# tjtiger86/dl-swin-gan

Measured on AMD Instinct MI355X. Metric: cine slices/sec (fwd+bwd) at 10-iter unroll, 1/2/4/8 GPU; PSNR vs ref, higher is better.
Workload: dtype fp32

## Files before the change

### dl-swin-gan_amd/csrc/conv3d.hip

```cpp
#include "dlcs_common.h"

#include <cstdlib>
#include <map>
#include <mutex>
#include <tuple>
#include <type_traits>

namespace {

enum ScratchSlot { kScrColsum, kScrH3r, kScrSplit2, kScrH3Tail, kScrWgH3, kScrTwp, kScrV6Tail, kScrBiasPart,
                   kScrSlots };
std::mutex g_scr_mu;
std::map<std::tuple<int, int, hipStream_t>, std::pair<void*, size_t>> g_scr;

void* scratch(int slot, hipStream_t st, size_t bytes) {
    int dev = 0;
    if (hipGetDevice(&dev) != hipSuccess) return nullptr;
    std::lock_guard<std::mutex> lk(g_scr_mu);
    auto& e = g_scr[{slot, dev, st}];
    if (e.second < bytes) {
        if (e.first) {
            if (hipStreamSynchronize(st) != hipSuccess) return nullptr;
            (void)hipFree(e.first);
        }
        e.first = nullptr;
        e.second = 0;
        if (hipMalloc(&e.first, bytes) != hipSuccess) return nullptr;
        e.second = bytes;
    }
    return e.first;
}

constexpr int kHaloT = 6, kHaloY = 10, kHaloX = 10;
constexpr int kHalo = kHaloT * kHaloY * kHaloX;
constexpr int CK = 32;

template <typename T> struct ConvPad;
template <> struct ConvPad<bf16> { static constexpr int v = 8; };
template <> struct ConvPad<float> { static constexpr int v = 4; };

DLCS_DEV long brow(int b, int t, int y, int x, int nT, int nY, int nX) {
    const long patch = (((long)b * nT + (t >> 2)) * nY + (y >> 2)) * nX + (x >> 2);
    return patch * 64 + ((t & 3) << 4) + ((y & 3) << 2) + (x & 3);
}

struct ConvArgs {
    const void* in; const void* w; const float* bias; void* out;
    const void* mask; const void* res;
    int B, D, H, W, Cin, cin_ld, cin_pad, Cout, cout_pad, cout_ld;
    int mask_ld, res_ld, relu_in, out_f32, res_f32, accumulate, relu_out;
    float res_scale;
};

template <typename T>
DLCS_DEV Frag8<T> relu8(Frag8<T> f) {
#pragma unroll
    for (int i = 0; i < 8; ++i) f.v[i] = (to_f(f.v[i]) > 0.0f) ? f.v[i] : from_f<T>(0.0f);
    return f;
}

template <typename T, int NT>
__global__ void __launch_bounds__(256) conv3d_k3_kernel(ConvArgs a) {
    constexpr int LD = CK + ConvPad<T>::v;
    constexpr int COP = NT * 32;
    extern __shared__ __attribute__((aligned(16))) char smem_raw[];
    T* Hs = reinterpret_cast<T*>(smem_raw);
    T* Ws = Hs + kHalo * LD;

    const int nT = a.D >> 2, nY = a.H >> 2, nX = a.W >> 2;
    const int nYt = (nY + 1) >> 1, nXt = (nX + 1) >> 1;
    int bid = blockIdx.x;
    const int txx = bid % nXt; bid /= nXt;
    const int tyy = bid % nYt; bid /= nYt;
    const int pt = bid % nT;
    const int b = bid / nT;
    const int t0 = pt * 4, y0 = tyy * 8, x0 = txx * 8;
    const T* in = reinterpret_cast<const T*>(a.in);
    const T* wt = reinterpret_cast<const T*>(a.w);
    const int lane = threadIdx.x & 63, wave = threadIdx.x >> 6, hh = lane >> 5;
    const int ncc = a.cin_pad / CK;
    const int nsteps = ncc * 27;

    auto stage_halo = [&](int cc) {
        for (int i = threadIdx.x; i < kHalo * (CK / 8); i += 256) {
            const int hv = i >> 2, c8 = (i & 3) * 8;
            const int ht = hv / (kHaloY * kHaloX), hy = (hv / kHaloX) % kHaloY, hx = hv % kHaloX;
            const int t = t0 - 1 + ht, y = y0 - 1 + hy, x = x0 - 1 + hx;
            const int c = cc * CK + c8;
            Frag8<T> f = zero8<T>();
            if (t >= 0 && t < a.D && y >= 0 && y < a.H && x >= 0 && x < a.W && c < a.Cin) {
                f = load8<T>(in + brow(b, t, y, x, nT, nY, nX) * a.cin_ld + c);
                if (a.relu_in) f = relu8<T>(f);
            }
// ... 1677 lines not shown
                         dlcs_stream_t stream) {
    DLCS_CHECK_ARG(in && gout && dw_packed && B > 0);
    if (D % 4 || H % 4 || W % 4 || cin_pad % 32 || cout_pad % 32 || cout_pad > 160 || cin_ld % 8 || g_ld % 8)
        return DLCS_ERR_UNSUPPORTED_SIZE;
    WgradArgs a{};
    a.in = in; a.g = gout; a.dw = dw_packed;
    a.B = (int)B; a.D = (int)D; a.H = (int)H; a.W = (int)W; a.Cin = (int)cin; a.cin_ld = (int)cin_ld;
    a.cin_pad = (int)cin_pad; a.Cout = (int)cout; a.g_ld = (int)g_ld; a.cout_pad = (int)cout_pad;
    a.relu_in = relu_in; a.vox_per_block = vox_per_block > 0 ? ((vox_per_block + 31) / 32) * 32 : 16384;
    hipStream_t st = (hipStream_t)stream;
    a.dbias = dbias;
    bool done = false;
    const int rc = dtype == DLCS_F32 ? wgrad_launch<float>(a, st, &done) : wgrad_launch<bf16>(a, st, &done);
    if (rc || !dbias || done) return rc;
    const long rows = B * D * H * W;
    return dlcs_colsum(dtype, gout, rows, cout, g_ld, dbias, stream);
}

int dlcs_conv3d_pack_weights(int dtype, const float* w, void* packed, int64_t cout, int64_t cin,
                             int64_t rows_pad, int64_t cols_pad, int mode, dlcs_stream_t stream) {
    DLCS_CHECK_ARG(w && packed && cout > 0 && cin > 0 && mode >= 0 && mode <= 3);
    const long n = 27L * rows_pad * cols_pad;
    hipStream_t st = (hipStream_t)stream;
    if (mode >= 2) {
#ifdef DLCS_DIAG_BUILD
        if (cout != 160 || cin != 160) return DLCS_ERR_UNSUPPORTED_SIZE;
        bf16* wa = (bf16*)packed;
        hipLaunchKernelGGL(pack_weights_x6_kernel, dim3(grid_for(27L * 160 * 160)), dim3(256), 0, st, w, wa,
                           wa + 27L * 160 * 320, mode - 2);
        return dlcs_launch_status();
#else
        return DLCS_ERR_UNSUPPORTED_SIZE;
#endif
    }
    if (dtype == DLCS_F32)
        hipLaunchKernelGGL(pack_weights_kernel<float>, dim3(grid_for(n)), dim3(256), 0, st, w, (float*)packed, (int)cout, (int)cin, (int)rows_pad, (int)cols_pad, mode);
    else
        hipLaunchKernelGGL(pack_weights_kernel<bf16>, dim3(grid_for(n)), dim3(256), 0, st, w, (bf16*)packed, (int)cout, (int)cin, (int)rows_pad, (int)cols_pad, mode);
    return dlcs_launch_status();
}

#ifdef DLCS_DIAG_BUILD
int dlcs_split3_bf16(const float* x, int64_t rows, int64_t ld, void* xa, void* xb, dlcs_stream_t stream) {
    DLCS_CHECK_ARG(x && xa && xb && rows > 0 && ld >= 160);
    if (ld % 4 || ((uintptr_t)x & 15) || ((uintptr_t)xa & 15) || ((uintptr_t)xb & 15)) return DLCS_ERR_UNSUPPORTED_SIZE;
    hipLaunchKernelGGL(split3_kernel, dim3(grid_for(rows * 20)), dim3(256), 0, (hipStream_t)stream, x, (long)rows,
                       (int)ld, (bf16*)xa, (bf16*)xb);
    return dlcs_launch_status();
}

int dlcs_conv3d_k3_x6(const void* xa, const void* xb, const void* wpacked, const float* bias, float* out,
                      int64_t cout_ld, int64_t B, int64_t D, int64_t H, int64_t W, const float* mask, int64_t mask_ld,
                      const float* residual, int64_t res_ld, float res_scale, int accumulate, int relu_out,
                      dlcs_stream_t stream) {
    DLCS_CHECK_ARG(xa && xb && wpacked && out && B > 0);
    auto al16 = [](const void* p) { return ((uintptr_t)p & 15) == 0; };
    if (D % 4 || H % 4 || W % 4 || cout_ld % 4 || !al16(xa) || !al16(xb) || !al16(wpacked) || !al16(out) ||
        (mask && (mask_ld % 4 || !al16(mask))) || (residual && (res_ld % 4 || !al16(residual))) || (bias && !al16(bias)) ||
        B * D * H * W * 320 >= (1L << 31))
        return DLCS_ERR_UNSUPPORTED_SIZE;
    ConvX6Args v{};
    v.xa = (const bf16*)xa; v.xb = (const bf16*)xb; v.w = (const bf16*)wpacked; v.bias = bias; v.out = out;
    v.mask = mask; v.res = residual; v.B = (int)B; v.D = (int)D; v.H = (int)H; v.W = (int)W;
    v.cout_ld = (int)cout_ld; v.mask_ld = (int)mask_ld; v.res_ld = (int)res_ld; v.accumulate = accumulate;
    v.relu_out = relu_out; v.res_scale = res_scale;
    return conv_x6_launch(v, (hipStream_t)stream);
}

int dlcs_conv3d_k3_wgrad_x6(const void* xa, const void* xb, const void* ga, const void* gb, float* dw_packed,
                            int64_t B, int64_t D, int64_t H, int64_t W, dlcs_stream_t stream) {
    DLCS_CHECK_ARG(xa && xb && ga && gb && dw_packed && B > 0);
    auto al16 = [](const void* p) { return ((uintptr_t)p & 15) == 0; };
    if (D % 4 || H % 4 || W % 4 || !al16(xa) || !al16(xb) || !al16(ga) || !al16(gb) ||
        B * D * H * W * 320 >= (1L << 40))
        return DLCS_ERR_UNSUPPORTED_SIZE;
    WgradX6Args v{};
    v.xa = (const bf16*)xa; v.xb = (const bf16*)xb; v.ga = (const bf16*)ga; v.gb = (const bf16*)gb;
    v.dw = dw_packed; v.B = (int)B; v.D = (int)D; v.H = (int)H; v.W = (int)W;
    return wgrad_x6_launch(v, (hipStream_t)stream);
}
#endif

size_t dlcs_split2_f16_bytes(int64_t rows) { return (size_t)rows * 640 + 256 + 640; }

int dlcs_split2_f16(const float* x, int64_t rows, int64_t ld, void* planes, int have_max, float* colsum,
                    dlcs_stream_t stream) {
    DLCS_CHECK_ARG(x && planes && rows > 0 && ld >= 160);
    if (ld % 4 || ((uintptr_t)x & 15) || ((uintptr_t)planes & 15)) return DLCS_ERR_UNSUPPORTED_SIZE;
    hipStream_t st = (hipStream_t)stream;
    unsigned* mx = (unsigned*)((char*)planes + (size_t)rows * 640);
    if (!have_max) {
        if (hipMemsetAsync(mx, 0, 4, st) != hipSuccess) return dlcs_launch_status();
        hipLaunchKernelGGL(absmax_kernel, dim3(std::min(h3_grid(rows * 10), 2048u)), dim3(256), 0, st, x, (long)rows,
                           (int)ld, mx);
    }
    const unsigned g = (unsigned)std::min<long>(kSplit2Blocks, std::max<long>(5, (rows * 20 + 255) / 256 / 5 * 5));
    if (colsum) {
        float* cpart = split2_colsum_workspace(st);
        if (!cpart) return (int)hipErrorOutOfMemory;
        hipLaunchKernelGGL(split2_f16_kernel<true>, dim3(g), dim3(256), 0, st, x, (long)rows, (int)ld,
                           (const unsigned*)mx, (f16*)planes, cpart);
        hipLaunchKernelGGL(colsum_parts_kernel, dim3(160), dim3(256), 0, st, (const float*)cpart, (int)g, colsum);
    } else {
        hipLaunchKernelGGL(split2_f16_kernel<false>, dim3(g), dim3(256), 0, st, x, (long)rows, (int)ld,
                           (const unsigned*)mx, (f16*)planes, nullptr);
    }
    return dlcs_launch_status();
}

size_t dlcs_conv3d_pack_weights_f16x3_bytes(void) { return (size_t)5 * 27 * 160 * 64 * 2 + 256; }

int dlcs_conv3d_pack_weights_f16x3(const float* w, int mode, void* packed, dlcs_stream_t stream) {
    DLCS_CHECK_ARG(w && packed && (mode == 0 || mode == 1));
    if (((uintptr_t)w & 15) || ((uintptr_t)packed & 15)) return DLCS_ERR_UNSUPPORTED_SIZE;
    hipStream_t st = (hipStream_t)stream;
    unsigned* mx = (unsigned*)((char*)packed + (size_t)5 * 27 * 160 * 64 * 2);
    if (hipMemsetAsync(mx, 0, 4, st) != hipSuccess) return dlcs_launch_status();
    hipLaunchKernelGGL(absmax_kernel, dim3(h3_grid(4320L * 10)), dim3(256), 0, st, w, 4320L, 160, mx);
    hipLaunchKernelGGL(pack_weights_f16x3_kernel, dim3(h3_grid(27L * 160 * 160)), dim3(256), 0, st, w,
                       (const unsigned*)mx, (f16*)packed, mode);
    return dlcs_launch_status();
}

static float* colsum_part_workspace(hipStream_t st, long nwg) {
    return static_cast<float*>(scratch(kScrColsum, st, (size_t)nwg * 160 * sizeof(float)));
}

int dlcs_conv3d_k3_f16x3(const void* xplanes, const void* wpacked, const float* bias, float* out, int64_t cout_ld,
                         int64_t B, int64_t D, int64_t H, int64_t W, const float* mask, int64_t mask_ld,
                         const float* residual, int64_t res_ld, float res_scale, int accumulate, int relu_out,
                         unsigned* out_max, void* out_planes, float* colsum, const void* mask_planes,
                         dlcs_stream_t stream) {
    DLCS_CHECK_ARG(xplanes && wpacked && B > 0 && (out || (out_planes && !accumulate)) && !(mask && mask_planes));
    if (!out) cout_ld = 160;
    auto al16 = [](const void* p) { return ((uintptr_t)p & 15) == 0; };
    const long rows = (long)B * D * H * W;
    if (D % 4 || H % 4 || W % 4 || cout_ld % 4 || !al16(xplanes) || !al16(wpacked) || !al16(out) ||
        (mask && (mask_ld % 4 || !al16(mask))) || (residual && (res_ld % 4 || !al16(residual))) || (bias && !al16(bias)) ||
        rows * 320 >= (1L << 31))
        return DLCS_ERR_UNSUPPORTED_SIZE;
    ConvH3Args v{};
    v.xp = (const f16*)xplanes; v.wp = (const f16*)wpacked;
    v.xmax = (const unsigned*)((const char*)xplanes + rows * 640);
    v.wmax = (const unsigned*)((const char*)wpacked + (size_t)5 * 27 * 160 * 64 * 2);
    v.bias = bias; v.out = out; v.mask = mask; v.res = residual;
    v.B = (int)B; v.D = (int)D; v.H = (int)H; v.W = (int)W;
    v.cout_ld = (int)cout_ld; v.mask_ld = (int)mask_ld; v.res_ld = (int)res_ld; v.accumulate = accumulate;
    v.relu_out = relu_out; v.res_scale = res_scale; v.omax = out_max;
    if (mask_planes && !al16(mask_planes)) return DLCS_ERR_UNSUPPORTED_SIZE;
    v.mplanes = mask_planes;
    if (out_planes) {
        if (cout_ld != 160 || !al16(out_planes)) return DLCS_ERR_UNSUPPORTED_SIZE;
        v.oplanes = (f16*)out_planes;
        v.opmax = (const unsigned*)((const char*)out_planes + rows * 640);
    }
#ifdef DLCS_DIAG_BUILD
    v.stamp = conv_stamps_on() ? 1 : 0;
    static const int h3_exp = [] { const char* e = dlcs_knob("DLCS_H3_EXP"); return e ? atoi(e) : 0; }();
    v.exp = h3_exp;
#endif
    hipStream_t st = (hipStream_t)stream;
    const long ntile = (long)B * (D / 4) * ((H / 4 + 1) / 2) * ((W / 4 + 1) / 2);
    if (colsum) {
        v.cpart = colsum_part_workspace(st, ntile);
        if (!v.cpart) return (int)hipErrorOutOfMemory;
    }
    const int rc = conv_f16x3_launch(v, st);
    if (rc || !colsum) return rc;
    hipLaunchKernelGGL(colsum_parts_kernel, dim3(160), dim3(256), 0, st, (const float*)v.cpart, (int)ntile, colsum);
    return dlcs_launch_status();
}

int dlcs_conv3d_k3_wgrad_f16x3(const void* xplanes, const void* gplanes, float* dw_packed, int64_t B, int64_t D,
                               int64_t H, int64_t W, dlcs_stream_t stream) {
    DLCS_CHECK_ARG(xplanes && gplanes && dw_packed && B > 0);
    auto al16 = [](const void* p) { return ((uintptr_t)p & 15) == 0; };
    const long rows = (long)B * D * H * W;
    if (D % 4 || H % 4 || W % 4 || !al16(xplanes) || !al16(gplanes) || rows * 320 >= (1L << 40))
        return DLCS_ERR_UNSUPPORTED_SIZE;
    WgradH3Args v{};
    v.xp = (const f16*)xplanes; v.gp = (const f16*)gplanes;
    v.xmax = (const unsigned*)((const char*)xplanes + rows * 640);
    v.gmax = (const unsigned*)((const char*)gplanes + rows * 640);
    v.dw = dw_packed; v.B = (int)B; v.D = (int)D; v.H = (int)H; v.W = (int)W;
    return wgrad_f16x3_launch(v, (hipStream_t)stream);
}

int dlcs_gemm_k160_f16x3(const void* aplanes, int64_t M, const void* bplanes, int64_t N, float* C, int64_t ldc,
                         const float* bias, int act, float alpha, const float* residual, int64_t ldr, float res_scale,
                         const float* residual2, int64_t ldr2, float res2_scale, int accumulate, unsigned* out_max,
                         void* out_planes, float* colsum, const void* res_planes, const void* res2_planes,
                         dlcs_stream_t stream) {
    DLCS_CHECK_ARG(aplanes && bplanes && M > 0 && N > 0 && (act == 0 || act == 3) &&
                   (C || (out_planes && !accumulate)) && !(residual && res_planes) && !(residual2 && res2_planes));
    if (!C) ldc = N;
    auto al16 = [](const void* p) { return ((uintptr_t)p & 15) == 0; };
    if (N % 160 || ldc % 4 || !al16(aplanes) || !al16(bplanes) || !al16(C) || (bias && !al16(bias)) ||
        (residual && (ldr % 4 || !al16(residual))) || (residual2 && (ldr2 % 4 || !al16(residual2))) ||
        M * 320 >= (1L << 40))
        return DLCS_ERR_UNSUPPORTED_SIZE;
    GemmH3Args g{};
    g.ap = (const f16*)aplanes; g.bp = (const f16*)bplanes;
    g.amax = (const unsigned*)((const char*)aplanes + M * 640);
    g.bmax = (const unsigned*)((const char*)bplanes + N * 640);
    g.c = C; g.ldc = ldc; g.bias = bias; g.act = act; g.alpha = alpha;
    g.res = residual; g.ldr = ldr; g.res_scale = res_scale;
    g.res2 = residual2; g.ldr2 = ldr2; g.res2_scale = res2_scale;
    g.accumulate = accumulate; g.M = (int)M; g.N = (int)N; g.omax = out_max;
    const long prows = M * (N / 160);
    if (res_planes) {
        if (!al16(res_planes)) return DLCS_ERR_UNSUPPORTED_SIZE;
        g.rp = (const f16*)res_planes;
        g.rpmax = (const unsigned*)((const char*)res_planes + prows * 640);
    }
    if (res2_planes) {
        if (!al16(res2_planes)) return DLCS_ERR_UNSUPPORTED_SIZE;
        g.rp2 = (const f16*)res2_planes;
        g.rp2max = (const unsigned*)((const char*)res2_planes + prows * 640);
    }
    if (out_planes) {
        if (ldc != N || !al16(out_planes)) return DLCS_ERR_UNSUPPORTED_SIZE;
        g.oplanes = (f16*)out_planes;
        g.opmax = (const unsigned*)((const char*)out_planes + M * (N / 160) * 640);
    }
    hipStream_t st = (hipStream_t)stream;
    const long nwg = cdiv(M, 64) * (N / 160);
    if (colsum) {
        if (g.row_map || nwg > (1L << 24)) return DLCS_ERR_UNSUPPORTED_SIZE;
        g.cpart = colsum_part_workspace(st, nwg);
        if (!g.cpart) return (int)hipErrorOutOfMemory;
    }
    const int rc = gemm_k160_launch(g, st);
    if (rc || !colsum) return rc;
    hipLaunchKernelGGL(colsum_parts_kernel, dim3(160), dim3(256), 0, st, (const float*)g.cpart, (int)nwg, colsum);
    return dlcs_launch_status();
}

int dlcs_linear_k160_f16x3(const void* xplanes, int64_t M, const void* wplanes, int64_t N, float* C, int64_t ldc,
                           const float* bias, int act, const float* aux, float* aux_out, int64_t ldaux, float alpha,
                           const float* residual, int64_t ldr, const int32_t* row_map, int accumulate,
                           dlcs_stream_t stream) {
    DLCS_CHECK_ARG(xplanes && wplanes && C && M > 0 && N > 0 && act >= 0 && act <= 3 && (act != 2 || aux));
    auto al16 = [](const void* p) { return ((uintptr_t)p & 15) == 0; };
    if (N % 160 || ldc % 4 || !al16(xplanes) || !al16(wplanes) || !al16(C) || (bias && !al16(bias)) ||
        (residual && (ldr % 4 || !al16(residual))) || ((aux || aux_out) && ldaux % 4) || (aux && !al16(aux)) ||
        (aux_out && !al16(aux_out)) || M * 320 >= (1L << 40))
        return DLCS_ERR_UNSUPPORTED_SIZE;
    GemmH3Args g{};
    g.ap = (const f16*)xplanes; g.bp = (const f16*)wplanes;
    g.amax = (const unsigned*)((const char*)xplanes + M * 640);
    g.bmax = (const unsigned*)((const char*)wplanes + N * 640);
    g.c = C; g.ldc = ldc; g.bias = bias; g.act = act; g.alpha = alpha;
    g.res = residual; g.ldr = ldr; g.res_scale = 1.0f;
    g.accumulate = accumulate; g.M = (int)M; g.N = (int)N;
    g.aux = aux; g.aux_out = aux_out; g.ldaux = ldaux; g.row_map = row_map;
    return gemm_k160_launch(g, (hipStream_t)stream);
}

size_t dlcs_h3r_pack_bytes(int64_t rows, int64_t K) {
    return (size_t)rows * K * 4 + (size_t)rows * 4 + (size_t)rows * kH3rKSplit * 4 + 256;
}

int dlcs_h3r_pack_multi(int n, const float* const* src, const int64_t* ld, const int* trans, const int64_t* rows,
                        const int64_t* K, void* const* dst, dlcs_stream_t stream) {
    DLCS_CHECK_ARG(n >= 0 && (n == 0 || (src && ld && trans && rows && K && dst)));
    for (int i0 = 0; i0 < n; i0 += kH3rPackMax) {
        H3rPackBatch bt{};
        const int cnt = std::min(n - i0, kH3rPackMax);
        int64_t maxrows = 0;
        int maxks = 1;
        for (int j = 0; j < cnt; ++j) {
            const int i = i0 + j;
            DLCS_CHECK_ARG(src[i] && dst[i] && rows[i] > 0 && K[i] > 0 && K[i] % 32 == 0 && ld[i] > 0 &&
                           ((uintptr_t)dst[i] & 15) == 0 && (trans[i] || (ld[i] % 4 == 0 && ((uintptr_t)src[i] & 15) == 0)));
            if (rows[i] > (1 << 20) || K[i] > 16384 || rows[i] * K[i] * 4 >= (1L << 31)) return DLCS_ERR_UNSUPPORTED_SIZE;
            H3rPackJob& jb = bt.j[j];
            jb.src = src[i]; jb.dst = (f16*)dst[i]; jb.inv = (float*)((char*)dst[i] + rows[i] * K[i] * 4);
            jb.part = jb.inv + rows[i];
            jb.rows = (int)rows[i]; jb.K = (int)K[i]; jb.ld = (int)ld[i]; jb.trans = trans[i];
            jb.nks = (int)std::max<int64_t>(1, std::min<int64_t>(kH3rKSplit, K[i] / 128));
            maxrows = std::max(maxrows, rows[i]);
            maxks = std::max(maxks, jb.nks);
        }
        const dim3 grid((unsigned)cdiv(maxrows, 64), (unsigned)cnt, (unsigned)maxks);
        hipLaunchKernelGGL(h3r_rowmax_kernel, grid, dim3(256), 0, (hipStream_t)stream, bt);
        hipLaunchKernelGGL(h3r_pack_kernel, grid, dim3(256), 0, (hipStream_t)stream, bt);
        const int st = dlcs_launch_status();
        if (st) return st;
    }
    return 0;
}

static float* h3r_ksplit_workspace(hipStream_t st, size_t floats) {
    return static_cast<float*>(scratch(kScrH3r, st, floats * sizeof(float)));
}

int dlcs_gemm_h3r(const float* A, int64_t M, int64_t K, int64_t lda, const void* bpacked, int64_t N, float* C,
                  int64_t ldc, const float* bias, int act, const float* aux, float* aux_out, int64_t ldaux, float alpha,
                  const float* residual, int64_t ldr, const int32_t* row_map, int accumulate, dlcs_stream_t stream) {
    DLCS_CHECK_ARG(A && bpacked && C && M > 0 && N > 0 && K > 0 && act >= 0 && act <= 7 &&
                   ((act != 2 && act != 5 && act != 6) || aux) && lda >= K);
    auto al16 = [](const void* p) { return ((uintptr_t)p & 15) == 0; };
    int nj = 0, nch = 0;
    if (N % 160 == 0 && K % 160 == 0) { nj = 5; nch = 5; }
    else if (N % 64 == 0 && K % 64 == 0) { nj = N % 128 == 0 ? 4 : 2; nch = K % 192 == 0 ? 6 : K % 128 == 0 ? 4 : 2; }
    if (!nj || lda % 4 || ldc % 4 || !al16(A) || !al16(bpacked) || !al16(C) || (bias && !al16(bias)) ||
        (residual && (ldr % 4 || !al16(residual))) || ((aux || aux_out) && ldaux % 4) || (aux && !al16(aux)) ||
// ... 45 lines not shown
    if (K % 4 || ld % 4 || ((uintptr_t)x & 15) || ((uintptr_t)q & 3) || K > (1 << 20))
        return DLCS_ERR_UNSUPPORTED_SIZE;
    hipLaunchKernelGGL(quant_f8r_kernel, dim3(cdiv(rows, 4)), dim3(256), 0, (hipStream_t)stream, x, (long)rows, (int)K,
                       (long)ld, (unsigned*)q, inv);
    return dlcs_launch_status();
}

int dlcs_gemm_f8r(const void* aq, const float* ainv, int64_t M, int64_t K, const void* bq, const float* binv,
                  int64_t N, float* C, int64_t ldc, const float* bias, int act, float* aux_out, int64_t ldaux,
                  float alpha, const float* residual, int64_t ldr, const int32_t* row_map, dlcs_stream_t stream) {
    DLCS_CHECK_ARG(aq && ainv && bq && binv && C && M > 0 && N > 0 && K > 0 && (act == 0 || act == 1 || act == 4));
    if (K % 64 || N % 64 || ((uintptr_t)aq & 15) || ((uintptr_t)bq & 15) || M * K >= (1L << 40))
        return DLCS_ERR_UNSUPPORTED_SIZE;
    GemmF8rArgs g{};
    g.a = (const unsigned char*)aq; g.ainv = ainv; g.M = (int)M;
    g.b = (const unsigned char*)bq; g.binv = binv; g.N = (int)N; g.K = (int)K;
    g.c = C; g.ldc = ldc; g.bias = bias; g.act = act; g.alpha = alpha;
    g.res = residual; g.ldr = ldr; g.row_map = row_map; g.aux_out = aux_out; g.ldaux = ldaux;
    hipLaunchKernelGGL(gemm_f8r_kernel, dim3(cdiv(M, 64), (unsigned)(N / 64)), dim3(256), 0, (hipStream_t)stream, g);
    return dlcs_launch_status();
}

size_t dlcs_conv3d_thin_pack_f16x3_bytes(int kind) {
    return (size_t)(kind == 0 ? kThinInHalfs : kThinOutHalfs) * 2 + 256;
}

int dlcs_conv3d_thin_pack_f16x3(const float* wpacked, int64_t cout, int64_t cout_pad, int64_t cin, int64_t cin_pad,
                                int kind, void* out, dlcs_stream_t stream) {
    DLCS_CHECK_ARG(wpacked && out && (kind == 0 || kind == 1) && cout <= cout_pad && cin <= cin_pad);
    if (kind == 0 ? !(cout == 160 && cout_pad == 160 && cin >= 1 && cin <= 4)
                  : !(cin == 160 && cin_pad == 160 && cout >= 1 && cout <= 4))
        return DLCS_ERR_UNSUPPORTED_SIZE;
    if ((uintptr_t)out & 15) return DLCS_ERR_UNSUPPORTED_SIZE;
    hipStream_t st = (hipStream_t)stream;
    const int halfs = kind == 0 ? kThinInHalfs : kThinOutHalfs;
    unsigned* mx = reinterpret_cast<unsigned*>(reinterpret_cast<char*>(out) + (size_t)halfs * 2 + 16);
    if (hipMemsetAsync(mx, 0, 4, st) != hipSuccess) return dlcs_launch_status();
    const long n = 27L * cout_pad * cin_pad;
    hipLaunchKernelGGL(absmax_flat_kernel, dim3((unsigned)std::min<long>(64, (n / 4 + 255) / 256)), dim3(256), 0, st,
                       wpacked, n, mx);
    hipLaunchKernelGGL(pack_thin_f16x3_grid_kernel, dim3((unsigned)((halfs / 2 + 255) / 256)), dim3(256), 0, st,
                       wpacked, (int)cout, (int)cout_pad, (int)cin, (int)cin_pad, kind, (const unsigned*)mx, (f16*)out);
    return dlcs_launch_status();
}

int dlcs_abs_row_sum_max(const float* w, int64_t rows, int64_t row_stride, int64_t n_outer, int64_t outer_stride,
                         int64_t inner, unsigned* out, dlcs_stream_t stream) {
    DLCS_CHECK_ARG(w && out && rows > 0 && rows < (1L << 31) && n_outer > 0 && inner > 0 && n_outer * inner < (1L << 31));
    hipStream_t st = (hipStream_t)stream;
    if (hipMemsetAsync(out, 0, 4, st) != hipSuccess) return dlcs_launch_status();
    if (n_outer * inner > 2048)
        hipLaunchKernelGGL(absrow_max_kernel<true>, dim3((unsigned)rows), dim3(256), 0, st, w, (int)rows,
                           (long)row_stride, (int)n_outer, (long)outer_stride, (int)inner, out);
    else
        hipLaunchKernelGGL(absrow_max_kernel<false>, dim3((unsigned)std::min<int64_t>((rows + 3) / 4, 256)), dim3(256), 0, st,
                           w, (int)rows,
                           (long)row_stride, (int)n_outer, (long)outer_stride, (int)inner, out);
    return dlcs_launch_status();
}

int dlcs_planes_bound(void* planes, int64_t rows, const unsigned* m0, const unsigned* n0, float c0,
                      const unsigned* m1, const unsigned* n1, float c1, const float* vec, int64_t nvec, float cvec,
                      dlcs_stream_t stream) {
    DLCS_CHECK_ARG(planes && rows > 0 && nvec >= 0 && nvec < (1L << 31) && (vec || nvec == 0));
    if ((uintptr_t)planes & 15) return DLCS_ERR_UNSUPPORTED_SIZE;
    hipLaunchKernelGGL(planes_bound_kernel, dim3(1), dim3(256), 0, (hipStream_t)stream,
                       (unsigned*)((char*)planes + (size_t)rows * 640), m0, n0, c0, m1, n1, c1, vec, (int)nvec, cvec);
    return dlcs_launch_status();
}

int dlcs_absmax_f32(const float* x, int64_t n, unsigned* out, dlcs_stream_t stream) {
    DLCS_CHECK_ARG(x && out && n >= 0);
    if ((uintptr_t)x & 15) return DLCS_ERR_UNSUPPORTED_SIZE;
    if (n == 0) return 0;
    hipLaunchKernelGGL(absmax_flat_kernel, dim3(std::min(h3_grid(n / 4 + 1), 1024u)), dim3(256), 0,
                       (hipStream_t)stream, x, (long)n, out);
    return dlcs_launch_status();
}

int dlcs_conv3d_thin_f16x3(const float* in, int64_t cin, int64_t cin_ld, const unsigned* in_max, const void* wthin,
                           const float* bias, float* out, int64_t cout, int64_t cout_ld, int64_t B, int64_t D,
                           int64_t H, int64_t W, const float* mask, int64_t mask_ld, const float* residual,
                           int64_t res_ld, float res_scale, int accumulate, int relu_out, unsigned* out_max,
                           void* out_planes, float* colsum, const void* mask_planes, dlcs_stream_t stream) {
    DLCS_CHECK_ARG(in && in_max && wthin && B > 0 && (out || out_planes) && !(mask && mask_planes));
    if (!out) cout_ld = 160;
    auto al16 = [](const void* p) { return ((uintptr_t)p & 15) == 0; };
    const long rows = (long)B * D * H * W;
    if (D % 4 || H % 4 || W % 4 || cin_ld % 4 || cout_ld % 4 || !al16(in) || !al16(out) || !al16(wthin) ||
        (bias && !al16(bias)) || rows * std::max(cin_ld, cout_ld) >= (1L << 31) || rows / 64 >= (1L << 24))
        return DLCS_ERR_UNSUPPORTED_SIZE;
    const bool thin_in = cin >= 1 && cin <= 4 && cout == 160;
    const bool thin_out = cin == 160 && cout >= 1 && cout <= 4;
    if (!thin_in && !thin_out) return DLCS_ERR_UNSUPPORTED_SIZE;
    if (thin_in && ((mask && (mask_ld % 4 || !al16(mask))) || (residual && (res_ld % 4 || !al16(residual)))))
        return DLCS_ERR_UNSUPPORTED_SIZE;
    if (thin_out && (mask || residual || out_max || cout_ld < 4)) return DLCS_ERR_UNSUPPORTED_SIZE;
    ConvF32Args v{};
    v.in = in; v.bias = bias; v.out = out; v.mask = mask; v.res = residual;
    v.B = (int)B; v.D = (int)D; v.H = (int)H; v.W = (int)W; v.cin_ld = (int)cin_ld; v.cin_pad = (int)cin;
    v.cout_ld = (int)cout_ld; v.mask_ld = (int)mask_ld; v.res_ld = (int)res_ld; v.accumulate = accumulate;
    v.relu_out = relu_out; v.res_scale = res_scale; v.cout = (int)cout; v.cout_pad = (int)cout; v.omax = out_max;
    v.mplanes = mask_planes;
    hipStream_t st = (hipStream_t)stream;
    if (!thin_in && (out_planes || colsum || mask_planes || !out)) return DLCS_ERR_UNSUPPORTED_SIZE;
    if (mask_planes && !al16(mask_planes)) return DLCS_ERR_UNSUPPORTED_SIZE;
    if (out_planes && (!al16(out_planes) || cout_ld != 160)) return DLCS_ERR_UNSUPPORTED_SIZE;
    const unsigned* opmax = out_planes ? (const unsigned*)((const char*)out_planes + rows * 640) : nullptr;
    const long ntile = (long)B * (D / 4) * ((H / 4 + 1) / 2) * ((W / 4 + 1) / 2);
    float* cpart = nullptr;
    if (colsum) {
        cpart = colsum_part_workspace(st, ntile);
        if (!cpart) return (int)hipErrorOutOfMemory;
    }
    const int rc = conv_thin_f16x3_launch(v, (const f16*)wthin, in_max, (int)cin, thin_in, st, (f16*)out_planes, opmax,
                                          cpart);
    if (rc || !colsum) return rc;
    hipLaunchKernelGGL(colsum_parts_kernel, dim3(160), dim3(256), 0, st, (const float*)cpart, (int)ntile, colsum);
    return dlcs_launch_status();
}

int dlcs_conv3d_thin_wgrad_f16x3(const float* in, int64_t cin, int64_t cin_ld, const unsigned* in_max,
                                 const float* g, int64_t cout, int64_t g_ld, const unsigned* g_max, float* dw_packed,
                                 int64_t cout_pad, int64_t cin_pad, float* colsum, int64_t B, int64_t D, int64_t H,
                                 int64_t W, dlcs_stream_t stream) {
    DLCS_CHECK_ARG(in && in_max && g && g_max && dw_packed && B > 0 && cout <= cout_pad && cin <= cin_pad);
    auto al16 = [](const void* p) { return ((uintptr_t)p & 15) == 0; };
    const bool thin_sfe = cout == 160 && cin >= 1 && cin <= 4;
    const bool thin_fin = cin == 160 && cout >= 1 && cout <= 4;
    const long npatch = B * (D / 4) * (H / 4) * (W / 4);
    if ((!thin_sfe && !thin_fin) || (colsum && !thin_sfe) || D % 4 || H % 4 || W % 4 || cin_ld % 4 || g_ld % 4 ||
        !al16(in) || !al16(g) || npatch >= (1L << 24))
        return DLCS_ERR_UNSUPPORTED_SIZE;
    ThinWgH3Args t{};
    t.big = thin_sfe ? g : in;
    t.thin = thin_sfe ? in : g;
    t.big_max = thin_sfe ? g_max : in_max;
    t.thin_max = thin_sfe ? in_max : g_max;
    t.dw = dw_packed; t.colsum = colsum;
    t.big_ld = (int)(thin_sfe ? g_ld : cin_ld); t.thin_ld = (int)(thin_sfe ? cin_ld : g_ld);
    t.sgn = thin_sfe ? 1 : -1; t.big_is_co = thin_sfe; t.thin_ch = (int)(thin_sfe ? cin : cout);
    t.cout_pad = (int)cout_pad; t.cin_pad = (int)cin_pad;
    t.B = (int)B; t.D = (int)D; t.H = (int)H; t.W = (int)W;
    const int nr = (int)std::min<long>(256, npatch);
    const int pp = (int)((npatch + nr - 1) / nr);
    hipLaunchKernelGGL(conv3d_wgrad_thin_f16x3_kernel, dim3(nr), dim3(512), 0, (hipStream_t)stream, t, nr, pp);
    return dlcs_launch_status();
}

int dlcs_conv3d_thin_out_planes_f16x3(const void* xplanes, const void* wthin, const float* bias, float* out,
                                      int64_t cout, int64_t cout_ld, int64_t B, int64_t D, int64_t H, int64_t W,
                                      int accumulate, int relu_out, dlcs_stream_t stream) {
    DLCS_CHECK_ARG(xplanes && wthin && out && B > 0 && cout >= 1 && cout <= 4 && cout_ld >= 4);
    auto al16 = [](const void* p) { return ((uintptr_t)p & 15) == 0; };
    if (D % 4 || H % 4 || W % 4 || cout_ld % 4 || !al16(xplanes) || !al16(wthin) || !al16(out))
        return DLCS_ERR_UNSUPPORTED_SIZE;
    ConvF32Args v{};
    v.bias = bias; v.out = out;
    v.B = (int)B; v.D = (int)D; v.H = (int)H; v.W = (int)W;
    v.cout_ld = (int)cout_ld; v.accumulate = accumulate; v.relu_out = relu_out; v.cout = (int)cout;
    v.cout_pad = (int)cout;
    return conv_thin_out_p_launch(v, (const f16*)xplanes, (const f16*)wthin, (hipStream_t)stream);
}

int dlcs_conv3d_thin_wgrad_planes_f16x3(const void* bigplanes, const float* thin, int64_t thin_ch, int64_t thin_ld,
                                        const unsigned* thin_max, int big_is_co, float* dw_packed, int64_t cout_pad,
                                        int64_t cin_pad, int64_t B, int64_t D, int64_t H, int64_t W,
                                        dlcs_stream_t stream) {
    DLCS_CHECK_ARG(bigplanes && thin && thin_max && dw_packed && B > 0 && thin_ch >= 1 && thin_ch <= 4 &&
                   thin_ld >= 4);
    auto al16 = [](const void* p) { return ((uintptr_t)p & 15) == 0; };
    if (D % 4 || H % 4 || W % 4 || thin_ld % 4 || !al16(bigplanes) || !al16(thin) ||
        (big_is_co ? (cout_pad < 160 || cin_pad < thin_ch) : (cin_pad < 160 || cout_pad < thin_ch)))
        return DLCS_ERR_UNSUPPORTED_SIZE;
    ThinWgPArgs t{};
    t.bp = (const f16*)bigplanes; t.thin = thin; t.dw = dw_packed; t.thin_max = thin_max;
    t.rows = (long)B * D * H * W;
    t.thin_ld = (int)thin_ld; t.sgn = big_is_co ? 1 : -1; t.big_is_co = big_is_co ? 1 : 0; t.thin_ch = (int)thin_ch;
    t.cout_pad = (int)cout_pad; t.cin_pad = (int)cin_pad;
    t.B = (int)B; t.D = (int)D; t.H = (int)H; t.W = (int)W;
    return wgrad_thin_p_launch(t, (hipStream_t)stream);
}

int dlcs_conv3d_unpack_wgrad(const float* dw_packed, float* grad, int64_t cout, int64_t cin, int64_t cout_pad,
                             int64_t cin_pad, int accumulate, dlcs_stream_t stream) {
    DLCS_CHECK_ARG(dw_packed && grad && cout > 0 && cin > 0);
    hipLaunchKernelGGL(unpack_wgrad_kernel, dim3(grid_for(cout * cin * 27)), dim3(256), 0, (hipStream_t)stream,
                       dw_packed, grad, (int)cout, (int)cin, (int)cout_pad, (int)cin_pad, accumulate);
    return dlcs_launch_status();
// ... 4 lines not shown
```

### dl-swin-gan_amd/csrc/conv3d_f16x3.inc

```
typedef _Float16 f16;
typedef _Float16 f16x8_t __attribute__((ext_vector_type(8)));
typedef unsigned u32x4_h3 __attribute__((ext_vector_type(4)));

DLCS_DEV void mfma16h(f32x4_t& acc, const f16x8_t& a, const f16x8_t& b) {
    acc = __builtin_amdgcn_mfma_f32_16x16x32_f16(a, b, acc, 0, 0, 0);
}

DLCS_DEV float f16x3_scale(unsigned maxbits) {
    const float m = __uint_as_float(maxbits);
    if (!(m > 0.0f) || !(m < 3.0e38f)) return 1.0f;
    int e;
    const float f = frexpf(m, &e);
    int k = 14 - (f == 0.5f ? e - 1 : e);
    k = k < -100 ? -100 : (k > 100 ? 100 : k);
    return ldexpf(1.0f, k);
}

typedef _Float16 f16x4_h3 __attribute__((ext_vector_type(4)));
DLCS_DEV f16 plane_lo(float u, f16 h) {
    f16 l = (f16)(u - (float)h);
    if (u != 0.0f && h == (f16)0.0f && l == (f16)0.0f) l = u > 0.0f ? (f16)5.9604645e-8f : (f16)-5.9604645e-8f;
    return l;
}
DLCS_DEV void put_planes8(f16* xp, long r, int c, const f32x4_t& v0, const f32x4_t& v1, float s) {
    f16x8_t h, l;
#pragma unroll
    for (int e = 0; e < 8; ++e) {
        const float u = (e < 4 ? v0[e] : v1[e - 4]) * s;
        h[e] = (f16)u;
        l[e] = plane_lo(u, h[e]);
    }
    f16* d = xp + r * 320 + (c >> 5) * 64 + (c & 31);
    *reinterpret_cast<f16x8_t*>(d) = h;
    *reinterpret_cast<f16x8_t*>(d + 32) = l;
}
DLCS_DEV void put_planes4(f16* xp, long r, int c, const f32x4_t& v, float s) {
    f16x4_h3 h, l;
#pragma unroll
    for (int e = 0; e < 4; ++e) {
        const float u = v[e] * s;
        h[e] = (f16)u;
        l[e] = plane_lo(u, h[e]);
    }
    f16* d = xp + r * 320 + (c >> 5) * 64 + (c & 31);
    *reinterpret_cast<f16x4_h3*>(d) = h;
    *reinterpret_cast<f16x4_h3*>(d + 32) = l;
}

DLCS_DEV f32x4_t get_planes4(const f16* xp, long r, int c, float rinv) {
    const f16* d = xp + r * 320 + (c >> 5) * 64 + (c & 31);
    const f16x4_h3 h = *reinterpret_cast<const f16x4_h3*>(d), l = *reinterpret_cast<const f16x4_h3*>(d + 32);
    f32x4_t v;
#pragma unroll
    for (int e = 0; e < 4; ++e) v[e] = ((float)h[e] + (float)l[e]) * rinv;
    return v;
}

template <bool ROWBLK>
__global__ void __launch_bounds__(256) absrow_max_kernel(const float* w, int R, long rs, int no, long os, int ni,
                                                         unsigned* out) {
    const int n = no * ni;
    float best = 0.0f;
    if (ROWBLK) {
        const float* row = w + (long)blockIdx.x * rs;
        float acc = 0.0f;
        for (int k = threadIdx.x; k < n; k += 256) acc += fabsf(row[(long)(k / ni) * os + k % ni]);
#pragma unroll
        for (int m = 32; m > 0; m >>= 1) acc += __shfl_xor(acc, m, 64);
        __shared__ float red[4];
        if ((threadIdx.x & 63) == 0) red[threadIdx.x >> 6] = acc;
        __syncthreads();
        best = (red[0] + red[1]) + (red[2] + red[3]);
    } else {
        const int lane = threadIdx.x & 63;
        for (int r = blockIdx.x * 4 + (int)(threadIdx.x >> 6); r < R; r += gridDim.x * 4) {
            const float* row = w + (long)r * rs;
            float acc = 0.0f;
            for (int k = lane; k < n; k += 64) acc += fabsf(row[(long)(k / ni) * os + k % ni]);
#pragma unroll
            for (int m = 32; m > 0; m >>= 1) acc += __shfl_xor(acc, m, 64);
            best = fmaxf(best, acc);
        }
        __shared__ float redm[4];
        if (lane == 0) redm[threadIdx.x >> 6] = best;
        __syncthreads();
        best = fmaxf(fmaxf(redm[0], redm[1]), fmaxf(redm[2], redm[3]));
    }
    if (threadIdx.x == 0 && best > 0.0f) atomicMax(out, __float_as_uint(best));
}

__global__ void __launch_bounds__(256) planes_bound_kernel(unsigned* trailer, const unsigned* m0, const unsigned* n0,
                                                           float c0, const unsigned* m1, const unsigned* n1, float c1,
                                                           const float* vec, int nvec, float cv) {
    float vm = 0.0f;
    for (int i = threadIdx.x; i < nvec; i += 256) vm = fmaxf(vm, fabsf(vec[i]));
    __shared__ float red[256];
    red[threadIdx.x] = vm;
    __syncthreads();
    for (int h = 128; h > 0; h >>= 1) {
        if ((int)threadIdx.x < h) red[threadIdx.x] = fmaxf(red[threadIdx.x], red[threadIdx.x + h]);
        __syncthreads();
    }
    if (threadIdx.x < 40)
        *reinterpret_cast<u32x4_h3*>(reinterpret_cast<char*>(trailer) + 256 + threadIdx.x * 16) = (u32x4_h3)0u;
    if (threadIdx.x == 0) {
        auto f = [](const unsigned* p) { return p ? __uint_as_float(*p) : 1.0f; };
        float b = cv * red[0];
        if (m0) b += c0 * f(m0) * f(n0);
        if (m1) b += c1 * f(m1) * f(n1);
        b *= 1.0f + 0.0009765625f;
        *trailer = b > 0.0f ? __float_as_uint(b) : 0u;
    }
}

DLCS_DEV void block_max_to(unsigned* omax, float v, float* red) {
    v = wave_max(v);
    const int w = threadIdx.x >> 6, nw = blockDim.x >> 6;
    __syncthreads();
    if ((threadIdx.x & 63) == 0) red[w] = v;
    __syncthreads();
    if (threadIdx.x == 0) {
        float m = red[0];
        for (int i = 1; i < nw; ++i) m = fmaxf(m, red[i]);
        if (m > 0.0f && m > __uint_as_float(__atomic_load_n(omax, __ATOMIC_RELAXED)))
            atomicMax(omax, __float_as_uint(m));
    }
}

DLCS_DEV int f16x3_halo_swz(int hy, int hx) { return 2 * (hy & 3) + ((hx >> 1) & 1); }
// ... 52 lines not shown
        }
        f16* dst = xp + r * 320 + (c8 >> 5) * 64 + (c8 & 31);
        *reinterpret_cast<f16x8_t*>(dst) = h;
        *reinterpret_cast<f16x8_t*>(dst + 32) = l;
    };
    const long rs = stride / 20;
    long r = gt / 20;
    for (; r + 3 * rs < rows; r += 4 * rs) {
        f32x4_t v[4][2];
#pragma unroll
        for (int u = 0; u < 4; ++u) {
            const float* src = x + (r + u * rs) * ld + c8;
            v[u][0] = *reinterpret_cast<const f32x4_t*>(src);
            v[u][1] = *reinterpret_cast<const f32x4_t*>(src + 4);
        }
#pragma unroll
        for (int u = 0; u < 4; ++u) put(r + u * rs, v[u][0], v[u][1]);
    }
    for (; r < rows; r += rs)
        put(r, *reinterpret_cast<const f32x4_t*>(x + r * ld + c8), *reinterpret_cast<const f32x4_t*>(x + r * ld + c8 + 4));
    if (CS) {
        __shared__ float part[256 * 8];
#pragma unroll
        for (int e = 0; e < 8; ++e) part[threadIdx.x * 8 + e] = cs[e];
        __syncthreads();
        if (threadIdx.x < 160) {
            const int c = threadIdx.x, g = c >> 3;
            const int t0 = (int)((g - (long)blockIdx.x * 256 % 20 + 20) % 20);
            float sum = 0.0f;
            for (int t = t0; t < 256; t += 20) sum += part[t * 8 + (c & 7)];
            cpart[blockIdx.x * 160 + c] = sum;
        }
    }
}

__global__ void __launch_bounds__(256) colsum_parts_kernel(const float* cpart, int nblk, float* colsum) {
    const int c = blockIdx.x;
    float v = 0.0f;
    for (int b = threadIdx.x; b < nblk; b += 256) v += cpart[b * 160 + c];
    __shared__ float red[256];
    red[threadIdx.x] = v;
    __syncthreads();
    for (int w = 128; w > 0; w >>= 1) {
        if ((int)threadIdx.x < w) red[threadIdx.x] += red[threadIdx.x + w];
        __syncthreads();
    }
    if (threadIdx.x == 0) colsum[c] += red[0];
}

static float* split2_colsum_workspace(hipStream_t st) {
    return static_cast<float*>(scratch(kScrSplit2, st, (size_t)kSplit2Blocks * 160 * sizeof(float)));
}

__global__ void pack_weights_f16x3_kernel(const float* w, const unsigned* maxbits, f16* wp, int mode) {
    const float s = f16x3_scale(*maxbits);
    const long n = 27L * 160 * 160;
    for (long i = blockIdx.x * (long)blockDim.x + threadIdx.x; i < n; i += (long)gridDim.x * blockDim.x) {
        const int c = (int)(i % 160);
        const int r = (int)((i / 160) % 160);
        const int tap = (int)(i / (160L * 160));
        const float u = s * (mode == 0 ? w[((long)r * 160 + c) * 27 + tap] : w[((long)c * 160 + r) * 27 + (26 - tap)]);
        const f16 hv = (f16)u;
        const long base = (((long)(c >> 5) * 27 + tap) * 160 + r) * 64 + (c & 31);
        wp[base] = hv;
        wp[base + 32] = (f16)(u - (float)hv);
    }
}

constexpr int kH3Halo = kHalo * 64;
constexpr int kH3Tap = 160 * 64;
constexpr int kH3Slot = 2 * kH3Tap;
constexpr int kH3Steps = 5 * 14;

struct ConvH3Args {
    const f16* xp; const f16* wp; const unsigned* xmax; const unsigned* wmax;
    const float* bias; float* out; const float* mask; const float* res;
    int B, D, H, W;
    int cout_ld, mask_ld, res_ld, accumulate, relu_out;
    float res_scale;
    unsigned* omax;
    float* part; int tail_base;
    f16* oplanes; const unsigned* opmax;
    float* cpart;
    const void* mplanes;
    int stamp;
    int exp;
};

#ifdef DLCS_DIAG_BUILD
__device__ unsigned long long g_h3_stamps[4096 * 73];
#define H3_STAMP(k) do { if (!TAIL && a.stamp && threadIdx.x == 0 && blockIdx.x < 4096) \
    g_h3_stamps[blockIdx.x * 73 + (k)] = __builtin_readcyclecounter(); } while (0)
#else
#define H3_STAMP(k) do { } while (0)
#endif

template <int EPI, int NPASS, bool PREF = true>
DLCS_DEV void conv_epilogue_h3(const ConvF32Args& a, const f32x4_t (&acc)[4][5], float* Es, int pw, int cw0,
                               int lane, int b, int pt, int pyq, int pxq, int nT, int nY, int nX,
                               f16* op, const unsigned* opmax, float* cpart) {
    const float ps = op ? f16x3_scale(*opmax) : 1.0f;
    static_assert(EPI == kEpiRes || EPI == kEpiMask, "fused forms only");
    constexpr int PC = 160 / NPASS, EL = PC + 4, NCH = PC / 8, PER = 256 * NCH / 512;
    static_assert(PC % 8 == 0 && 256 * NCH % 512 == 0 && PC <= 512, "whole 8-channel chunks per thread");
    const float* src = EPI == kEpiRes ? a.res : a.mask;
    const int sld = EPI == kEpiRes ? a.res_ld : a.mask_ld;
    const f16* mp = EPI == kEpiMask ? reinterpret_cast<const f16*>(a.mplanes) : nullptr;
    f32x4_t pre[PREF ? NPASS : 1][PER][2];
    long orows[PER];
    bool oks[PER];
#pragma unroll
    for (int k = 0; k < PER; ++k) {
        const int c = threadIdx.x + k * 512;
        const int vl = c / NCH;
        const int pwv = vl >> 6;
        const int py = pyq + (pwv >> 1), px = pxq + (pwv & 1);
        oks[k] = py < nY && px < nX;
        orows[k] = ((((long)b * nT + pt) * nY + min(py, nY - 1)) * nX + min(px, nX - 1)) * 64 + (vl & 63);
    }
    auto load_pre = [&](int pass, int slot) {
#pragma unroll
        for (int k = 0; k < PER; ++k) {
            const int c = threadIdx.x + k * 512;
            const int co = pass * PC + (c % NCH) * 8;
            if (mp) {
                const f16* q = mp + orows[k] * 320 + (co >> 5) * 64 + (co & 31);
                pre[slot][k][0] = *reinterpret_cast<const f32x4_t*>(q);
                pre[slot][k][1] = *reinterpret_cast<const f32x4_t*>(q + 32);
            } else {
                const float* sp = src + orows[k] * sld + co;
                pre[slot][k][0] = *reinterpret_cast<const f32x4_t*>(sp);
                pre[slot][k][1] = *reinterpret_cast<const f32x4_t*>(sp + 4);
            }
        }
    };
    if constexpr (PREF) {
#pragma unroll
        for (int pass = 0; pass < NPASS; ++pass) load_pre(pass, pass);
    }
    float vmax = 0.0f;
#pragma unroll
    for (int pass = 0; pass < NPASS; ++pass) {
        const int ps_ = PREF ? pass : 0;
        if constexpr (!PREF) load_pre(pass, 0);
#pragma unroll
        for (int j = 0; j < 5; ++j) {
            const int c0 = cw0 + j * 16 - pass * PC;
            if (c0 + 16 <= 0 || c0 >= PC) continue;
#pragma unroll
            for (int i = 0; i < 4; ++i)
#pragma unroll
                for (int r = 0; r < 4; ++r) {
                    const int vl = pw * 64 + i * 16 + (lane >> 4) * 4 + r;
                    const int cl = c0 + (lane & 15);
                    if (cl >= 0 && cl < PC) Es[vl * EL + cl] = acc[i][j][r];
                }
        }
        __syncthreads();
#pragma unroll
        for (int k = 0; k < PER; ++k) {
            const int c = threadIdx.x + k * 512;
            const int vl = c / NCH, ch = (c % NCH) * 8;
            const int co = pass * PC + ch;
            if (!oks[k]) {
                if (cpart) {
                    *reinterpret_cast<f32x4_t*>(Es + vl * EL + ch) = (f32x4_t)0.0f;
                    *reinterpret_cast<f32x4_t*>(Es + vl * EL + ch + 4) = (f32x4_t)0.0f;
                }
                continue;
            }
            f32x4_t v0 = *reinterpret_cast<const f32x4_t*>(Es + vl * EL + ch);
            f32x4_t v1 = *reinterpret_cast<const f32x4_t*>(Es + vl * EL + ch + 4);
            if (a.bias) {
                v0 += *reinterpret_cast<const f32x4_t*>(a.bias + co);
                v1 += *reinterpret_cast<const f32x4_t*>(a.bias + co + 4);
            }
            if (EPI == kEpiMask && mp) {
                const u32x4_h3 hb = __builtin_bit_cast(u32x4_h3, pre[ps_][k][0]);
                const u32x4_h3 lb = __builtin_bit_cast(u32x4_h3, pre[ps_][k][1]);
#pragma unroll
                for (int e = 0; e < 8; ++e) {
                    const unsigned nz = ((hb[e >> 1] | lb[e >> 1]) >> (16 * (e & 1))) & 0x7fffu;
                    if (e < 4) v0[e] = nz ? v0[e] : 0.0f;
                    else v1[e - 4] = nz ? v1[e - 4] : 0.0f;
                }
            } else if (EPI == kEpiMask) {
#pragma unroll
                for (int e = 0; e < 4; ++e) {
                    v0[e] = pre[ps_][k][0][e] > 0.0f ? v0[e] : 0.0f;
                    v1[e] = pre[ps_][k][1][e] > 0.0f ? v1[e] : 0.0f;
                }
            } else {
                v0 += a.res_scale * pre[ps_][k][0];
                v1 += a.res_scale * pre[ps_][k][1];
            }
            if (a.relu_out) {
#pragma unroll
                for (int e = 0; e < 4; ++e) { v0[e] = fmaxf(v0[e], 0.0f); v1[e] = fmaxf(v1[e], 0.0f); }
            }
            if (a.out) {
                float* o = a.out + orows[k] * a.cout_ld + co;
                *reinterpret_cast<f32x4_t*>(o) = v0;
                *reinterpret_cast<f32x4_t*>(o + 4) = v1;
            }
            if (op) put_planes8(op, orows[k], co, v0, v1, ps);
            if (cpart) {
                *reinterpret_cast<f32x4_t*>(Es + vl * EL + ch) = v0;
                *reinterpret_cast<f32x4_t*>(Es + vl * EL + ch + 4) = v1;
            }
            if (a.omax) {
#pragma unroll
                for (int e = 0; e < 4; ++e) vmax = fmaxf(vmax, fmaxf(fabsf(v0[e]), fabsf(v1[e])));
            }
        }
        if (cpart) {
            constexpr int G = 512 / PC;
            __syncthreads();
            float* red = Es + 256 * EL;
            const int t = threadIdx.x;
            if (t < G * PC) {
                const int cc = t % PC, g = t / PC;
                float cs = 0.0f;
                for (int r = g; r < 256; r += G) cs += Es[r * EL + cc];
                red[g * PC + cc] = cs;
            }
            __syncthreads();
            if (t < PC) {
                float cs = 0.0f;
#pragma unroll
                for (int g = 0; g < G; ++g) cs += red[g * PC + t];
                cpart[pass * PC + t] = cs;
            }
        }
        __syncthreads();
    }
    if (a.omax) {
        vmax = wave_max(vmax);
        if ((threadIdx.x & 63) == 0 && vmax > 0.0f && vmax > __uint_as_float(__atomic_load_n(a.omax, __ATOMIC_RELAXED)))
            atomicMax(a.omax, __float_as_uint(vmax));
    }
}

template <int EPI, int FOLD, bool TAIL = false>
__global__ void __launch_bounds__(512) conv3d_k3_f16x3_kernel(ConvH3Args a) {
    __shared__ __attribute__((aligned(16))) f16 smem_h3[kH3Halo + 2 * kH3Slot];
    f16* X = smem_h3;
    f16* Ws = X + kH3Halo;

    const int nT = a.D >> 2, nY = a.H >> 2, nX = a.W >> 2;
    const int nYt = (nY + 1) >> 1, nXt = (nX + 1) >> 1;
    const int nblk = a.B * nT * nYt * nXt;
    const int cc0 = TAIL ? (int)blockIdx.x % 5 : 0;
    const int cc1 = TAIL ? cc0 + 1 : 5;
    const int q8 = nblk >> 3, r8 = nblk & 7;
    const int lane = threadIdx.x & 63;
    const int wave = __builtin_amdgcn_readfirstlane(threadIdx.x >> 6);
    int vb = 0, b = 0, pt = 0, tyy = 0, txx = 0, t0 = 0, y0 = 0, x0 = 0;
    unsigned rsgn = 0;
    auto set_tile = [&](int v) {
        vb = v;
        const int xcd = vb & 7;
        int bid = xcd * q8 + min(xcd, r8) + (vb >> 3);
        txx = bid % nXt; bid /= nXt;
        tyy = bid % nYt; bid /= nYt;
        pt = bid % nT;
        b = bid / nT;
        t0 = pt * 4; y0 = tyy * 8; x0 = txx * 8;
        rsgn = ((unsigned)(vb * 8 + wave) * 0x9E3779B1u) >> 16;
    };
    set_tile(TAIL ? a.tail_base + (int)blockIdx.x / 5 : (int)blockIdx.x);
    const int pw = wave & 3, nh = wave >> 2;
    const int send = cc1 * 14;
    H3_STAMP(0);

    constexpr int HP = 10, HD = 3, HR = HP - HD;
    f16x8_t hr[HR];
    auto halo_off = [&](int k) {
        const int i = threadIdx.x + k * 512;
        int off = -1;
        if (i < kHalo * 8) {
            const int hv = i >> 3, c = i & 7;
            const int ht = hv / (kHaloY * kHaloX), hy = (hv / kHaloX) % kHaloY, hx = hv % kHaloX;
            const int t = t0 - 1 + ht, y = y0 - 1 + hy, x = x0 - 1 + hx;
            if (t >= 0 && t < a.D && y >= 0 && y < a.H && x >= 0 && x < a.W)
                off = (int)(brow(b, t, y, x, nT, nY, nX) * 320 + (c ^ f16x3_halo_swz(hy, hx)) * 8);
        }
        return off;
    };
    const unsigned xbase = lds_offset(X);
    auto dma_halo = [&](int cc) {
        const f16* zrow = reinterpret_cast<const f16*>(g_wg_zero_row);
#pragma unroll
        for (int k = 0; k < HD; ++k) {
            const int off = halo_off(k);
            glds16(off >= 0 ? a.xp + cc * 64 + off : zrow, xbase + (unsigned)((k * 512 + wave * 64) * 16));
        }
    };
    auto load_halo = [&](int cc) {
#pragma unroll
        for (int k = 0; k < HR; ++k) {
            const int off = halo_off(HD + k);
            hr[k] = (f16x8_t)(f16)0.0f;
            if (off >= 0) hr[k] = *reinterpret_cast<const f16x8_t*>(a.xp + cc * 64 + off);
        }
    };
    auto store_halo = [&]() {
#pragma unroll
        for (int k = 0; k < HR; ++k) {
            const int i = threadIdx.x + (HD + k) * 512;
            if (i < kHalo * 8) *reinterpret_cast<f16x8_t*>(X + i * 8) = hr[k];
        }
    };
    const unsigned wbase = lds_offset(Ws);
    unsigned woff[5];
#pragma unroll
    for (int k = 0; k < 5; ++k) {
        const int wi = k * 8 + wave, pp = wi % 20;
// ... 141 lines not shown
#pragma unroll
                for (int i = 0; i < 4; ++i)
#pragma unroll
                    for (int j = 0; j < 5; ++j) acc[i][j] = -acc[i][j];
            };
            const unsigned nm = flip ? 0x80008000u : 0u;
            auto nega = [&](f16x8_t (&af)[4]) {
                if constexpr (FOLD == 2 || FOLD == 3) {
                    const unsigned m = FOLD == 2 ? nm : rowm;
#pragma unroll
                    for (int i = 0; i < 4; ++i)
                        af[i] = __builtin_bit_cast(f16x8_t, __builtin_bit_cast(u32x4_h3, af[i]) ^ m);
                }
            };
            if (flip) negate_acc();
#pragma unroll
            for (int ti = 0; ti < nt; ++ti) {
                read_a(tap_a(ti, 0), ah);
                nega(ah);
                read_b(ti, bofh, bh);
                read_b(ti, bofl, bl);
                if (xexp & 4) {
                    read_a(tap_a(ti, 1), al);
#pragma unroll
                    for (int i = 0; i < 4; ++i)
                        acc[i][0][0] += (float)ah[i][0] + (float)al[i][1] + (float)bh[i][2] + (float)bl[i][3] + (float)bh[4][i] + (float)bl[4][i];
                    continue;
                }
                mma(ah, bh);
                if (ti == 0 && s + 1 < send && !(xexp & 8)) issue_w(s + 1);
                read_a(tap_a(ti, 1), al);
                nega(al);
                mma(ah, bl);
                mma(al, bh);
            }
            if (flip) negate_acc();
        }
        if (seam) {
            __syncthreads();
            store_halo();
        }
        if (!(xexp & 2)) asm volatile("s_waitcnt vmcnt(0)" ::: "memory");
        if (seam || !(xexp & 1)) __syncthreads();
        H3_STAMP(2 + s);
    };
    dma_halo(cc0);
    load_halo(cc0);
    issue_w(cc0 * 14);
    store_halo();
    asm volatile("s_waitcnt vmcnt(0)" ::: "memory");
    __syncthreads();
    H3_STAMP(1);

#pragma unroll
    for (int i = 0; i < 4; ++i)
#pragma unroll
        for (int j = 0; j < 5; ++j) acc[i][j] = (f32x4_t)0.0f;
    for (int cc = cc0; cc < cc1; ++cc) {
        for (int tp = 0; tp < 13; ++tp) step(cc * 14 + tp, cc, tp, std::integral_constant<int, 2>{});
        step(cc * 14 + 13, cc, 13, std::integral_constant<int, 1>{});
    }
    const float inv = 1.0f / (f16x3_scale(*a.xmax) * f16x3_scale(*a.wmax));
#pragma unroll
    for (int i = 0; i < 4; ++i)
#pragma unroll
        for (int j = 0; j < 5; ++j)
#pragma unroll
            for (int r = 0; r < 4; ++r)
                acc[i][j][r] *= (FOLD == 3 && ((rsgn >> (4 * (lane >> 4) + r)) & 1)) ? -inv : inv;
    if constexpr (TAIL) {
        float* pp = a.part + (long)blockIdx.x * 256 * 160;
#pragma unroll
        for (int i = 0; i < 4; ++i)
#pragma unroll
            for (int j = 0; j < 5; ++j)
#pragma unroll
                for (int r = 0; r < 4; ++r)
                    pp[(pw * 64 + i * 16 + (lane >> 4) * 4 + r) * 160 + nh * 80 + j * 16 + (lane & 15)] = acc[i][j][r];
        return;
    }
    ConvF32Args ea{};
    ea.bias = a.bias; ea.out = a.out; ea.mask = a.mask; ea.res = a.res;
    ea.cout_ld = a.cout_ld; ea.mask_ld = a.mask_ld; ea.res_ld = a.res_ld; ea.accumulate = a.accumulate;
    ea.relu_out = a.relu_out; ea.res_scale = a.res_scale; ea.omax = a.omax; ea.mplanes = a.mplanes;
    if constexpr (EPI == kEpiRes || EPI == kEpiMask)
        conv_epilogue_h3<EPI, 2>(ea, acc, reinterpret_cast<float*>(smem_h3), pw, nh * 80, lane, b, pt, tyy * 2, txx * 2,
                                 nT, nY, nX, a.oplanes, a.opmax, a.cpart ? a.cpart + (long)vb * 160 : nullptr);
    else
        conv_epilogue_f32<EPI>(ea, acc, reinterpret_cast<float*>(smem_h3), pw, nh * 80, lane, b, pt, tyy * 2, txx * 2,
                               nT, nY, nX);
    H3_STAMP(72);
}

__global__ void __launch_bounds__(256) conv_f16x3_tail_reduce_kernel(ConvH3Args a, int ntail) {
    __shared__ float red[4];
    const int nT = a.D >> 2, nY = a.H >> 2, nX = a.W >> 2;
    const int nYt = (nY + 1) >> 1, nXt = (nX + 1) >> 1;
    const int nblk = a.B * nT * nYt * nXt;
    const long i = (long)blockIdx.x * 256 + threadIdx.x;
    float vmax = 0.0f;
    if (i < (long)ntail * 256 * 40) {
        const int t = (int)(i / (256 * 40)), rem = (int)(i % (256 * 40));
        const int vl = rem / 40, c = (rem % 40) * 4;
        f32x4_t v = (f32x4_t)0.0f;
#pragma unroll
        for (int w = 0; w < 5; ++w) v += *reinterpret_cast<const f32x4_t*>(a.part + ((long)(t * 5 + w) * 256 + vl) * 160 + c);
        const int vb = a.tail_base + t;
        const int q8 = nblk >> 3, r8 = nblk & 7, xcd = vb & 7;
        int bid = xcd * q8 + min(xcd, r8) + (vb >> 3);
        const int txx = bid % nXt; bid /= nXt;
        const int tyy = bid % nYt; bid /= nYt;
        const int pt = bid % nT;
        const int b = bid / nT;
        const int pwv = vl >> 6;
        const int py = tyy * 2 + (pwv >> 1), px = txx * 2 + (pwv & 1);
        if (py < nY && px < nX) {
            const long orow = ((((long)b * nT + pt) * nY + py) * nX + px) * 64 + (vl & 63);
            if (a.bias) v += *reinterpret_cast<const f32x4_t*>(a.bias + c);
            if (a.mask) {
                const f32x4_t m = *reinterpret_cast<const f32x4_t*>(a.mask + orow * a.mask_ld + c);
#pragma unroll
                for (int e = 0; e < 4; ++e) v[e] = m[e] > 0.0f ? v[e] : 0.0f;
            } else if (a.mplanes) {
                const f16* q = reinterpret_cast<const f16*>(a.mplanes) + orow * 320 + (c >> 5) * 64 + (c & 31);
                const f16x4_h3 h = *reinterpret_cast<const f16x4_h3*>(q), l = *reinterpret_cast<const f16x4_h3*>(q + 32);
#pragma unroll
                for (int e = 0; e < 4; ++e) v[e] = (h[e] != (f16)0.0f || l[e] != (f16)0.0f) ? v[e] : 0.0f;
            }
            if (a.res) v += a.res_scale * *reinterpret_cast<const f32x4_t*>(a.res + orow * a.res_ld + c);
            if (a.relu_out) {
#pragma unroll
                for (int e = 0; e < 4; ++e) v[e] = fmaxf(v[e], 0.0f);
            }
            if (a.out) {
                float* o = a.out + orow * a.cout_ld + c;
                if (a.accumulate) v += *reinterpret_cast<const f32x4_t*>(o);
                *reinterpret_cast<f32x4_t*>(o) = v;
            }
            if (a.oplanes) put_planes4(a.oplanes, orow, c, v, f16x3_scale(*a.opmax));
            vmax = fmaxf(fmaxf(fabsf(v[0]), fabsf(v[1])), fmaxf(fabsf(v[2]), fabsf(v[3])));
        } else {
            v = (f32x4_t)0.0f;
        }
        if (a.cpart) *reinterpret_cast<f32x4_t*>(a.part + ((long)(t * 5) * 256 + vl) * 160 + c) = v;
    }
    if (a.omax) block_max_to(a.omax, vmax, red);
}

__global__ void __launch_bounds__(160) tail_colsum_kernel(ConvH3Args a, int nparts) {
    const int t = blockIdx.x, c = threadIdx.x;
    const float* p = a.part + (long)(t * nparts) * 256 * 160 + c;
    float cs = 0.0f;
    for (int r = 0; r < 256; ++r) cs += p[(long)r * 160];
    a.cpart[(long)(a.tail_base + t) * 160 + c] = cs;
}

static float* h3_tail_workspace(hipStream_t st) {
    return static_cast<float*>(scratch(kScrH3Tail, st, (size_t)51 * 5 * 256 * 160 * sizeof(float)));
}

static int conv_f16x3_launch(const ConvH3Args& v0, hipStream_t st) {
    ConvH3Args v = v0;
    const int nT = v.D / 4, nY = v.H / 4, nX = v.W / 4;
    unsigned nblk = (unsigned)((long)v.B * nT * ((nY + 1) / 2) * ((nX + 1) / 2));
    const char* te = dlcs_test_hook("DLCS_H3_TAIL");
    const bool tail_split = !(te && te[0] == '0');
    const unsigned ntail = nblk % 256, nmain = nblk - ntail;
    const bool split = tail_split && nmain > 0 && ntail > 0 && ntail * 5 <= 256;
    float* ws = nullptr;
    if (split) {
        ws = h3_tail_workspace(st);
        if (!ws) return (int)hipErrorOutOfMemory;
        nblk = nmain;
    }
    int epi;
    if (!v.res && !v.mask && !v.mplanes && !v.accumulate) epi = 0;
    else if (v.res && !v.mask && !v.mplanes && !v.accumulate) epi = kEpiRes;
    else if (!v.res && (v.mask || v.mplanes) && !v.accumulate) epi = kEpiMask;
    else epi = kEpiGeneric;
    if ((v.oplanes || v.cpart || v.mplanes) && epi != kEpiRes && epi != kEpiMask)
        return DLCS_ERR_UNSUPPORTED_SIZE;
    static const int fold_mode = [] {
        const char* e = dlcs_knob("DLCS_H3_FOLD");
        return !e ? 4 : e[0] == '0' ? 0 : e[0] == 'm' ? 2 : e[0] == 'a' ? 3 : e[0] == 'r' ? 4 : e[0] == 'R' ? 5 : 1;
    }();
    const bool masked = v.mask || v.mplanes;
    const int pf = fold_mode == 1 || (fold_mode == 2 && masked) ? 1 : (fold_mode == 3 && masked) ? 2
                 : (fold_mode == 5 || (fold_mode == 4 && masked)) ? 3 : 0;
    auto launch = [&](auto F) {
        constexpr int f = decltype(F)::value;
        const dim3 g(nblk);
        if (epi == 0) hipLaunchKernelGGL((conv3d_k3_f16x3_kernel<0, f>), g, dim3(512), 0, st, v);
        else if (epi == kEpiRes) hipLaunchKernelGGL((conv3d_k3_f16x3_kernel<kEpiRes, f>), g, dim3(512), 0, st, v);
        else if (epi == kEpiMask) hipLaunchKernelGGL((conv3d_k3_f16x3_kernel<kEpiMask, f>), g, dim3(512), 0, st, v);
        else hipLaunchKernelGGL((conv3d_k3_f16x3_kernel<kEpiGeneric, f>), g, dim3(512), 0, st, v);
    };
#ifdef DLCS_DIAG_BUILD
    if (pf == 1) launch(std::integral_constant<int, 1>{});
    else if (pf == 2) launch(std::integral_constant<int, 2>{});
    else
#endif
    if (pf == 3) launch(std::integral_constant<int, 3>{});
    else launch(std::integral_constant<int, 0>{});
    if (split) {
        ConvH3Args t = v;
        t.part = ws;
        t.tail_base = (int)nmain;
#ifdef DLCS_DIAG_BUILD
        if (pf == 1) hipLaunchKernelGGL((conv3d_k3_f16x3_kernel<0, 1, true>), dim3(ntail * 5), dim3(512), 0, st, t);
        else if (pf == 2) hipLaunchKernelGGL((conv3d_k3_f16x3_kernel<0, 2, true>), dim3(ntail * 5), dim3(512), 0, st, t);
        else
#endif
        if (pf == 3) hipLaunchKernelGGL((conv3d_k3_f16x3_kernel<0, 3, true>), dim3(ntail * 5), dim3(512), 0, st, t);
        else hipLaunchKernelGGL((conv3d_k3_f16x3_kernel<0, 0, true>), dim3(ntail * 5), dim3(512), 0, st, t);
        hipLaunchKernelGGL(conv_f16x3_tail_reduce_kernel, dim3((unsigned)cdiv((long)ntail * 256 * 40, 256)), dim3(256),
                           0, st, t, (int)ntail);
        if (v.cpart) hipLaunchKernelGGL(tail_colsum_kernel, dim3(ntail), dim3(160), 0, st, t, 5);
    }
    return dlcs_launch_status();
}

constexpr int kWhRows = 32 + 48;
constexpr int kWhPlane = kWhRows * 160;
constexpr int kWhBuf = 2 * kWhPlane;

struct WgradH3Args {
    const f16* gp; const f16* xp;
    const unsigned* gmax; const unsigned* xmax;
    float* dw;
    float* part;
    int B, D, H, W;
};

DLCS_DEV f16x8_t tr_read16h(const f16* p0, const f16* p1) {
    return __builtin_bit_cast(f16x8_t, tr_read16(reinterpret_cast<const bf16*>(p0), reinterpret_cast<const bf16*>(p1)));
}

DLCS_DEV long h3_zero_row_byte(long rows) { return rows * 640 + 256; }

__global__ void __launch_bounds__(768) conv3d_wgrad_f16x3_kernel(WgradH3Args a, int nrange, int ppr) {
    __shared__ __attribute__((aligned(16))) f16 smem_wh[3 * kWhBuf];
    const int b = blockIdx.x;
    int range, grp;
    {
        const int xcd = b & 7, slot = b >> 3;
        const int q = nrange >> 3;
        if ((nrange & 7) == 0) { range = (slot / 9) * 8 + xcd; grp = slot % 9; }
        else if ((nrange & 7) == 4) {
            if (slot < 9 * q) { range = (slot / 9) * 8 + xcd; grp = slot % 9; }
            else { range = 8 * q + (xcd & 3); grp = (slot - 9 * q) + (xcd < 4 ? 0 : 5); }
        } else { range = b / 9; grp = b % 9; }
    }
    if (range >= nrange || grp >= 9) return;
    const int kd = grp / 3 - 1, kh = grp % 3 - 1;
    const int nT = a.D >> 2, nY = a.H >> 2, nX = a.W >> 2;
    const int nYX = nY * nX;
    const int npatch = a.B * nT * nYX;
    const int p0 = range * ppr, p1 = min(npatch, p0 + ppr);
    if (p0 >= p1) return;
    const int lane = threadIdx.x & 63, wave = __builtin_amdgcn_readfirstlane(threadIdx.x >> 6);
    const int kwi = wave >> 2, coh = (wave >> 1) & 1, cih = wave & 1;
    const int bias_rows = (nYX + nX + 1) * 64;
    const long rows = (long)npatch * 64;

    unsigned pk[5];
#pragma unroll
    for (int k = 0; k < 5; ++k) {
        const int wi = k * 12 + wave;
        const int pl = wi >= 25 ? 1 : 0, wl = wi - pl * 25;
// ... 130 lines not shown
                xl = tr_read16h(Xl + bcol(j + 1), Xl + 6 * 160 + bcol(j + 1));
            }
        }
        if (!ahead) asm volatile("s_waitcnt vmcnt(0)" ::: "memory");
        else if (wave < 2) asm volatile("s_waitcnt vmcnt(5)" ::: "memory");
        else asm volatile("s_waitcnt vmcnt(4)" ::: "memory");
        __syncthreads();
        cur = cur == 2 ? 0 : cur + 1;
    };
    for (int u = 2 * p0; u < 2 * p1; ++u) {
        const int th = u & 1;
        unit(th, (u >> 1) + 1 < p1);
        if (th) next_patch();
    }
    const int tap = (kd + 1) * 9 + (kh + 1) * 3 + kwi;
    float* pp = a.part + ((long)range * 27 + tap) * 160 * 160;
    float* st = reinterpret_cast<float*>(smem_wh) + wave * (16 * 84);
#pragma unroll
    for (int i = 0; i < 5; ++i) {
#pragma unroll
        for (int j = 0; j < 5; ++j)
#pragma unroll
            for (int r = 0; r < 4; ++r) st[(gq * 4 + r) * 84 + j * 16 + (lane & 15)] = acc[i][j][r];
#pragma unroll
        for (int s = 0; s < 5; ++s) {
            const int e = s * 64 + lane, r = e / 20, c4 = (e % 20) * 4;
            const f32x4_t v = *reinterpret_cast<const f32x4_t*>(st + r * 84 + c4);
            *reinterpret_cast<f32x4_t*>(pp + (coh * 80 + 16 * i + r) * 160 + cih * 80 + c4) = v;
        }
    }
}

__global__ void __launch_bounds__(256) wgrad_f16x3_reduce_kernel(WgradH3Args a, int nrange) {
    const long i = (long)blockIdx.x * 256 + threadIdx.x;
    if (i >= 27L * 160 * 40) return;
    const float inv = 1.0f / (f16x3_scale(*a.gmax) * f16x3_scale(*a.xmax));
    const f32x4_t* src = reinterpret_cast<const f32x4_t*>(a.part);
    f32x4_t s = src[i];
    for (int r = 1; r < nrange; ++r) s += src[(long)r * 27 * 160 * 40 + i];
    f32x4_t* d = reinterpret_cast<f32x4_t*>(a.dw) + i;
    *d = *d + s * inv;
}

constexpr int kWgH3MaxRanges = 32;

static float* wgh3_workspace(hipStream_t st) {
    return static_cast<float*>(scratch(kScrWgH3, st, (size_t)kWgH3MaxRanges * 27 * 160 * 160 * sizeof(float)));
}

static int wgrad_f16x3_launch(const WgradH3Args& a0, hipStream_t st) {
    WgradH3Args a = a0;
    const long npatch = (long)a.B * (a.D / 4) * (a.H / 4) * (a.W / 4);
    const long bias_rows = ((long)(a.H / 4) * (a.W / 4) + a.W / 4 + 1) * 64;
    if ((2 * bias_rows + 128) * 40 >= (1L << 25) || (npatch * 64 + bias_rows) * 640 + 1024 >= (1L << 32))
        return DLCS_ERR_UNSUPPORTED_SIZE;
    static const int env_nr = [] { const char* e = dlcs_knob("DLCS_WGH3_RANGES"); return e ? atoi(e) : 0; }();
    int nr = env_nr > 0 ? std::min(env_nr, kWgH3MaxRanges) : 28;
    nr = (int)std::min<long>(nr, npatch);
    const long pp = (npatch + nr - 1) / nr;
    nr = (int)((npatch + pp - 1) / pp);
    a.part = wgh3_workspace(st);
    if (!a.part) return (int)hipErrorOutOfMemory;
    hipLaunchKernelGGL(conv3d_wgrad_f16x3_kernel, dim3((unsigned)(9 * nr)), dim3(768), 0, st, a, nr, (int)pp);
    hipLaunchKernelGGL(wgrad_f16x3_reduce_kernel, dim3((unsigned)cdiv(27L * 160 * 40, 256)), dim3(256), 0, st, a, nr);
    return dlcs_launch_status();
}

struct GemmH3Args {
    const f16* ap; const f16* bp; const unsigned* amax; const unsigned* bmax;
    float* c; long ldc;
    const float* bias; int act; float alpha;
    const float* res; long ldr; float res_scale;
    const float* res2; long ldr2; float res2_scale;
    int accumulate;
    int M, N;
    unsigned* omax;
    const float* aux; float* aux_out; long ldaux;
    const int* row_map;
    int xcd_nt;
    f16* oplanes; const unsigned* opmax;
    float* cpart;
    const f16* rp; const f16* rp2;
    const unsigned* rpmax; const unsigned* rp2max;
};
constexpr int kG3A = 64 * 64, kG3B = 160 * 64;

__global__ void __launch_bounds__(512, 2) gemm_k160_f16x3_kernel(GemmH3Args g) {
    __shared__ __attribute__((aligned(16))) f16 smem_g3[5 * kG3A + 2 * kG3B];
    const int lane = threadIdx.x & 63, wave = __builtin_amdgcn_readfirstlane(threadIdx.x >> 6);
    const int wm = wave & 3, wn = wave >> 2;
    int mt = blockIdx.x, nt = blockIdx.y;
    if (g.xcd_nt) {
        const int k = blockIdx.x >> 3;
        nt = (blockIdx.x & 7) * g.xcd_nt + k % g.xcd_nt;
        mt = k / g.xcd_nt;
    }
    const int m0 = mt * 64, n0 = nt * 160;
    const unsigned sbase = lds_offset(smem_g3);
    auto issue_a = [&]() {
        for (int wi = wave; wi < 40; wi += 8) {
            const int cc = wi >> 3, rb = wi & 7;
            const int r = rb * 8 + (lane >> 3), pc = lane & 7;
            const int lc = pc ^ ((r >> 1) & 7);
            const f16* src = g.ap + (long)min(m0 + r, g.M - 1) * 320 + cc * 64 + lc * 8;
            glds16(src, sbase + (unsigned)(cc * kG3A * 2 + rb * 1024));
        }
    };
    auto issue_b = [&](int cc, int slot) {
        for (int rb = wave; rb < 20; rb += 8) {
            const int r = rb * 8 + (lane >> 3), pc = lane & 7;
            const int lc = pc ^ ((r >> 1) & 7);
            const f16* src = g.bp + (long)min(n0 + r, g.N - 1) * 320 + cc * 64 + lc * 8;
            glds16(src, sbase + (unsigned)((5 * kG3A + slot * kG3B) * 2 + rb * 1024));
        }
    };
    issue_a();
    issue_b(0, 0);
    f32x4_t acc[5];
#pragma unroll
    for (int j = 0; j < 5; ++j) acc[j] = (f32x4_t)0.0f;
    const int vq = lane & 15, cq = lane >> 4, sw = (vq >> 1) & 7;
    const int oh = (cq ^ sw) << 3, ol = ((4 + cq) ^ sw) << 3;
    asm volatile("s_waitcnt vmcnt(0)" ::: "memory");
    __syncthreads();
    for (int cc = 0; cc < 5; ++cc) {
        if (cc + 1 < 5) issue_b(cc + 1, (cc + 1) & 1);
        const f16* As = smem_g3 + cc * kG3A + (wm * 16 + vq) * 64;
        const f16* Bs = smem_g3 + 5 * kG3A + (cc & 1) * kG3B + (wn * 80 + vq) * 64;
        const f16x8_t ah = *reinterpret_cast<const f16x8_t*>(As + oh);
        const f16x8_t al = *reinterpret_cast<const f16x8_t*>(As + ol);
#pragma unroll
        for (int j = 0; j < 5; ++j) {
            const f16x8_t bh = *reinterpret_cast<const f16x8_t*>(Bs + j * 16 * 64 + oh);
            const f16x8_t bl = *reinterpret_cast<const f16x8_t*>(Bs + j * 16 * 64 + ol);
            mfma16h(acc[j], ah, bh);
            mfma16h(acc[j], ah, bl);
            mfma16h(acc[j], al, bh);
        }
        asm volatile("s_waitcnt vmcnt(0)" ::: "memory");
        __syncthreads();
    }
    const float inv = 1.0f / (f16x3_scale(*g.amax) * f16x3_scale(*g.bmax));
    __syncthreads();
    float* Es = reinterpret_cast<float*>(smem_g3);
    constexpr int EL = 164;
    const float ps = g.oplanes ? f16x3_scale(*g.opmax) : 1.0f;
    const float rinv = g.rp ? 1.0f / f16x3_scale(*g.rpmax) : 1.0f;
    const float rinv2 = g.rp2 ? 1.0f / f16x3_scale(*g.rp2max) : 1.0f;
    float vmax = 0.0f;
#pragma unroll
    for (int j = 0; j < 5; ++j)
#pragma unroll
        for (int r = 0; r < 4; ++r)
            Es[(wm * 16 + 4 * cq + r) * EL + wn * 80 + j * 16 + vq] = acc[j][r] * inv;
    __syncthreads();
#pragma unroll
    for (int k = 0; k < 5; ++k) {
        const int c = threadIdx.x + k * 512;
        const int ml = c / 40, ch = (c % 40) * 4;
        const long m = m0 + ml, n = n0 + ch;
        if (m >= g.M || n >= g.N) {
            if (g.cpart) *reinterpret_cast<f32x4_t*>(Es + ml * EL + ch) = (f32x4_t)0.0f;
            continue;
        }
        long orow = m;
        if (g.row_map) {
            orow = g.row_map[m];
            if (orow < 0) continue;
        }
        f32x4_t v = *reinterpret_cast<const f32x4_t*>(Es + ml * EL + ch);
        if (g.bias) v += *reinterpret_cast<const f32x4_t*>(g.bias + n);
        if (g.act == 3) {
#pragma unroll
            for (int e = 0; e < 4; ++e) v[e] = fmaxf(v[e], 0.0f);
        } else if (g.act == 1) {
            if (g.aux_out) *reinterpret_cast<f32x4_t*>(g.aux_out + m * g.ldaux + n) = v;
#pragma unroll
            for (int e = 0; e < 4; ++e) v[e] = gelu_erf(v[e]);
        } else if (g.act == 2) {
            const f32x4_t av = *reinterpret_cast<const f32x4_t*>(g.aux + m * g.ldaux + n);
#pragma unroll
            for (int e = 0; e < 4; ++e) v[e] *= gelu_erf_grad(av[e]);
        }
        v *= g.alpha;
        if (g.res) v += g.res_scale * *reinterpret_cast<const f32x4_t*>(g.res + orow * g.ldr + n);
        if (g.res2) v += g.res2_scale * *reinterpret_cast<const f32x4_t*>(g.res2 + orow * g.ldr2 + n);
        if (g.rp) v += g.res_scale * get_planes4(g.rp, orow * (g.N / 160) + nt, ch, rinv);
        if (g.rp2) v += g.res2_scale * get_planes4(g.rp2, orow * (g.N / 160) + nt, ch, rinv2);
        if (g.c) {
            float* cp = g.c + orow * g.ldc + n;
            if (g.accumulate) v += *reinterpret_cast<const f32x4_t*>(cp);
            *reinterpret_cast<f32x4_t*>(cp) = v;
        }
        if (g.oplanes) put_planes4(g.oplanes, orow * (g.N / 160) + nt, ch, v, ps);
        if (g.cpart) *reinterpret_cast<f32x4_t*>(Es + ml * EL + ch) = v;
        vmax = fmaxf(vmax, fmaxf(fmaxf(fabsf(v[0]), fabsf(v[1])), fmaxf(fabsf(v[2]), fabsf(v[3]))));
    }
    if (g.cpart) {
        __syncthreads();
        if (threadIdx.x < 160) {
            float cs = 0.0f;
            for (int r = 0; r < 64; ++r) cs += Es[r * EL + threadIdx.x];
            g.cpart[((long)mt * (g.N / 160) + nt) * 160 + threadIdx.x] = cs;
        }
    }
    if (g.omax) block_max_to(g.omax, vmax, Es + 64 * EL);
}

static int gemm_k160_launch(const GemmH3Args& g0, hipStream_t st) {
    GemmH3Args g = g0;
    const int ntiles = g.N / 160;
    if (g.xcd_nt >= 0 && ntiles % 8 == 0) {
        g.xcd_nt = ntiles / 8;
        hipLaunchKernelGGL(gemm_k160_f16x3_kernel, dim3(cdiv(g.M, 64) * (unsigned)ntiles), dim3(512), 0, st, g);
    } else {
        g.xcd_nt = 0;
        hipLaunchKernelGGL(gemm_k160_f16x3_kernel, dim3(cdiv(g.M, 64), (unsigned)ntiles), dim3(512), 0, st, g);
    }
    return dlcs_launch_status();
}
```

### dl-swin-gan_amd/csrc/conv3d_f32.inc

```

constexpr int kWfC = 160;
constexpr int kWfRows = 32 + 48;
constexpr int kWfBuf = kWfRows * kWfC;
constexpr int kWfChunks = kWfRows * kWfC / 4;

__device__ float4 g_wf_zero_row[kWfC / 4];

DLCS_DEV void mfma4f(f32x4_t& acc, float a, float b) {
    acc = __builtin_amdgcn_mfma_f32_16x16x4f32(a, b, acc, 0, 0, 0);
}

__global__ void __launch_bounds__(768) conv3d_wgrad_f32_kernel(WgradArgs a, int nrange, long ppr, int xcd_map) {
    __shared__ __attribute__((aligned(16))) float smem[3 * kWfBuf];
    const int b = blockIdx.x;
    int range, grp;
    if (xcd_map) {
        const int xcd = b & 7, slot = b >> 3;
        range = (slot / 9) * 8 + xcd;
        grp = slot % 9;
    } else {
        range = b / 9;
        grp = b % 9;
    }
    if (range >= nrange) return;
// ... 40 lines not shown
            }
            glds16(src, dst + wi * 1024);
        }
    };

    f32x4_t acc[5][5];
#pragma unroll
    for (int i = 0; i < 5; ++i)
#pragma unroll
        for (int j = 0; j < 5; ++j) acc[i][j] = (f32x4_t)0.0f;

    const int q = lane >> 4, m = lane & 15;
    const int gp = q & 1, hp = (q + kwi) & 1;
    int aoff[5], boff[5];
#pragma unroll
    for (int i = 0; i < 5; ++i) aoff[i] = q * kWfC + (((coh * 5 + i) ^ gp) << 4) + m;
#pragma unroll
    for (int j = 0; j < 5; ++j) boff[j] = (32 + q + kwi) * kWfC + (((cih * 5 + j) ^ hp) << 4) + m;

    const long u0 = 2 * p0, u1 = 2 * p1;
    issue(u0, 0);
    if (u0 + 1 < u1) issue(u0 + 1, 1);
    asm volatile("s_waitcnt vmcnt(0)" ::: "memory");
    __syncthreads();
    int cur = 0;
    for (long u = u0; u < u1; ++u) {
        if (u + 2 < u1) issue(u + 2, cur == 0 ? 2 : cur - 1);
        const float* S = smem + cur * kWfBuf;
#pragma unroll
        for (int s = 0; s < 8; ++s) {
            const int gro = 4 * s * kWfC, hro = ((s >> 2) * 4 + (s & 3)) * 6 * kWfC;
            float af[5], bfv[5];
#pragma unroll
            for (int i = 0; i < 5; ++i) af[i] = S[aoff[i] + gro];
#pragma unroll
            for (int j = 0; j < 5; ++j) bfv[j] = S[boff[j] + hro];
#pragma unroll
            for (int j = 0; j < 5; ++j)
#pragma unroll
                for (int i = 0; i < 5; ++i) mfma4f(acc[i][j], af[i], bfv[j]);
        }
        if (u + 2 < u1) {
            if (wave < 2) asm volatile("s_waitcnt vmcnt(5)" ::: "memory");
            else asm volatile("s_waitcnt vmcnt(4)" ::: "memory");
        } else {
            asm volatile("s_waitcnt vmcnt(0)" ::: "memory");
        }
        __syncthreads();
        cur = cur == 2 ? 0 : cur + 1;
    }
    const int tap = (kd + 1) * 9 + (kh + 1) * 3 + kwi;
    float* dw = a.dw + (long)tap * kWfC * kWfC;
#pragma unroll
    for (int i = 0; i < 5; ++i)
#pragma unroll
        for (int j = 0; j < 5; ++j)
#pragma unroll
            for (int r = 0; r < 4; ++r) {
                const int co = coh * 80 + 16 * i + q * 4 + r, ci = cih * 80 + 16 * j + m;
                atomicAdd(dw + co * kWfC + ci, acc[i][j][r]);
            }
}

static int wgrad_f32_c160_launch(const WgradArgs& a, hipStream_t st) {
    const long npatch = (long)a.B * (a.D / 4) * (a.H / 4) * (a.W / 4);
    static const int env_nr = [] { const char* e = dlcs_knob("DLCS_WGF32_RANGES"); return e ? atoi(e) : 0; }();
    int nr = env_nr > 0 ? env_nr : 28;
    nr = (int)std::min<long>(nr, npatch);
    const long pp = (npatch + nr - 1) / nr;
    nr = (int)((npatch + pp - 1) / pp);
    const int xcd_map = (nr % 8 == 0) ? 1 : 0;
    hipLaunchKernelGGL(conv3d_wgrad_f32_kernel, dim3((unsigned)(9 * nr)), dim3(768), 0, st, a, nr, pp, xcd_map);
    return dlcs_launch_status();
}

struct ConvF32Args {
    const float* in; const float* w; const float* bias; float* out;
    const float* mask; const float* res;
    int B, D, H, W, cin_ld, cin_pad;
    int cout_ld, mask_ld, res_ld, accumulate, relu_out;
    float res_scale;
    int cout, cout_pad;
    unsigned* omax;
    const void* mplanes;
};

template <int EPI, int NPASS = 2>
DLCS_DEV void conv_epilogue_f32(const ConvF32Args& a, const f32x4_t (&acc)[4][5], float* Es, int pw, int cw0,
                                int lane, int b, int pt, int pyq, int pxq, int nT, int nY, int nX) {
    constexpr int PC = 160 / NPASS, EL = PC + 4, NCH = PC / 8, PER = 256 * NCH / 512;
    static_assert(256 * NCH % 512 == 0, "whole 8-channel chunks per thread");
    const bool has_res = (EPI & kEpiGeneric) ? a.res != nullptr : (EPI & kEpiRes);
    const bool has_mask = (EPI & kEpiGeneric) ? a.mask != nullptr : (EPI & kEpiMask);
    const bool accum = (EPI & kEpiGeneric) ? a.accumulate != 0 : (EPI & kEpiAcc);
    float vmax = 0.0f;
#pragma unroll
    for (int pass = 0; pass < NPASS; ++pass) {
#pragma unroll
        for (int j = 0; j < 5; ++j) {
            const int c0 = cw0 + j * 16 - pass * PC;
            if (c0 + 16 <= 0 || c0 >= PC) continue;
#pragma unroll
            for (int i = 0; i < 4; ++i)
#pragma unroll
                for (int r = 0; r < 4; ++r) {
                    const int vl = pw * 64 + i * 16 + (lane >> 4) * 4 + r;
                    const int cl = c0 + (lane & 15);
                    if (cl >= 0 && cl < PC) Es[vl * EL + cl] = acc[i][j][r];
                }
        }
        __syncthreads();
#pragma unroll
        for (int k = 0; k < PER; ++k) {
            const int c = threadIdx.x + k * 512;
            const int vl = c / NCH, ch = (c % NCH) * 8;
            const int pwv = vl >> 6;
            const int py = pyq + (pwv >> 1), px = pxq + (pwv & 1);
            if (py >= nY || px >= nX) continue;
            const long orow = ((((long)b * nT + pt) * nY + py) * nX + px) * 64 + (vl & 63);
            const int co = pass * PC + ch;
            f32x4_t v0 = *reinterpret_cast<const f32x4_t*>(Es + vl * EL + ch);
            f32x4_t v1 = *reinterpret_cast<const f32x4_t*>(Es + vl * EL + ch + 4);
            if (a.bias) {
                v0 += *reinterpret_cast<const f32x4_t*>(a.bias + co);
                v1 += *reinterpret_cast<const f32x4_t*>(a.bias + co + 4);
            }
            if (has_mask) {
                const float* mp = a.mask + orow * a.mask_ld + co;
                const f32x4_t m0 = *reinterpret_cast<const f32x4_t*>(mp);
                const f32x4_t m1 = *reinterpret_cast<const f32x4_t*>(mp + 4);
#pragma unroll
                for (int e = 0; e < 4; ++e) {
                    v0[e] = m0[e] > 0.0f ? v0[e] : 0.0f;
                    v1[e] = m1[e] > 0.0f ? v1[e] : 0.0f;
                }
            }
            if (has_res) {
                const float* rp = a.res + orow * a.res_ld + co;
                v0 += a.res_scale * *reinterpret_cast<const f32x4_t*>(rp);
                v1 += a.res_scale * *reinterpret_cast<const f32x4_t*>(rp + 4);
            }
            if (a.relu_out) {
#pragma unroll
                for (int e = 0; e < 4; ++e) { v0[e] = fmaxf(v0[e], 0.0f); v1[e] = fmaxf(v1[e], 0.0f); }
            }
            float* o = a.out + orow * a.cout_ld + co;
            if (accum) {
                v0 += *reinterpret_cast<const f32x4_t*>(o);
                v1 += *reinterpret_cast<const f32x4_t*>(o + 4);
            }
            *reinterpret_cast<f32x4_t*>(o) = v0;
            *reinterpret_cast<f32x4_t*>(o + 4) = v1;
            if (a.omax) {
#pragma unroll
                for (int e = 0; e < 4; ++e) vmax = fmaxf(vmax, fmaxf(fabsf(v0[e]), fabsf(v1[e])));
            }
        }
        __syncthreads();
    }
    if (a.omax) {
        vmax = wave_max(vmax);
        if ((threadIdx.x & 63) == 0 && vmax > 0.0f && vmax > __uint_as_float(__atomic_load_n(a.omax, __ATOMIC_RELAXED)))
            atomicMax(a.omax, __float_as_uint(vmax));
    }
}

constexpr int kF5Slot = 3 * 160 * 16;
// ... 496 lines not shown
```

### dl-swin-gan_amd/csrc/conv3d_thin_f16x3.inc

```
typedef _Float16 f16x4_t __attribute__((ext_vector_type(4)));

DLCS_DEV void mfma32h(f32x16& acc, const f16x8_t& a, const f16x8_t& b) {
    acc = __builtin_amdgcn_mfma_f32_32x32x16_f16(a, b, acc, 0, 0, 0);
}

struct XcdWalk {
    int t, end, step;
    DLCS_DEV XcdWalk(int ntiles) {
        const int per = (ntiles + 7) >> 3, x = blockIdx.x & 7;
        t = x * per + (blockIdx.x >> 3);
        end = min(ntiles, (x + 1) * per);
        step = gridDim.x >> 3;
    }
};

DLCS_DEV f32x4_t ldz4f(const float* p, bool ok) {
    return *reinterpret_cast<const f32x4_t*>(ok ? static_cast<const void*>(p) : static_cast<const void*>(g_wg_zero_row));
}

DLCS_DEV void split_f16(float x, float s, f16& h, f16& l) {
    const float u = x * s;
    h = (f16)u;
    l = (f16)(u - (float)h);
}
// ... 121 lines not shown
    auto decode = [&](int tile, int& b, int& pt, int& tyy, int& txx) {
        int bid = tile;
        txx = bid % nXt; bid /= nXt;
        tyy = bid % nYt; bid /= nYt;
        pt = bid % nT;
        b = bid / nT;
    };
    constexpr int HPER = (kHalo + 511) / 512;
    f32x4_t hreg[HPER];
    auto load_halo = [&](int tile) {
        int b, pt, tyy, txx;
        decode(tile, b, pt, tyy, txx);
#pragma unroll
        for (int kk = 0; kk < HPER; ++kk) {
            const int hv = threadIdx.x + 512 * kk;
            const int ht = hv / (kHaloY * kHaloX), hy = (hv / kHaloX) % kHaloY, hx = hv % kHaloX;
            const int t = pt * 4 - 1 + ht, y = tyy * 8 - 1 + hy, x = txx * 8 - 1 + hx;
            const bool ok = hv < kHalo && t >= 0 && t < a.D && y >= 0 && y < a.H && x >= 0 && x < a.W;
            hreg[kk] = ldz4f(a.in + brow(b, t, y, x, nT, nY, nX) * a.cin_ld, ok);
        }
    };
    const XcdWalk wk(ntiles);
    int tile = wk.t;
    if (tile < wk.end) load_halo(tile);
    for (; tile < wk.end; tile += wk.step) {
        int b, pt, tyy, txx;
        decode(tile, b, pt, tyy, txx);
#pragma unroll
        for (int kk = 0; kk < HPER; ++kk) {
            const int hv = threadIdx.x + 512 * kk;
            if (hv < kHalo) {
                f16x8_t hl;
#pragma unroll
                for (int e = 0; e < 4; ++e) {
                    f16 h, l;
                    split_f16(e < cin ? hreg[kk][e] : 0.0f, sx, h, l);
                    hl[e] = h;
                    hl[4 + e] = l;
                }
                *reinterpret_cast<f16x8_t*>(Hs + hv * 8) = hl;
            }
        }
        __syncthreads();
        if (tile + wk.step < wk.end) load_halo(tile + wk.step);
        f32x4_t acc[4][5];
#pragma unroll
        for (int i = 0; i < 4; ++i)
#pragma unroll
            for (int j = 0; j < 5; ++j) acc[i][j] = (f32x4_t)0.0f;
        const unsigned rsgn = ((unsigned)(tile * 8 + wave) * 0x9E3779B1u) >> 16;
        const unsigned rowm = ((rsgn >> m) & 1) ? 0x80008000u : 0u;
#pragma unroll
        for (int ks = 0; ks < 4; ++ks) {
            f16x8_t ah[4], al[4];
#pragma unroll
            for (int i = 0; i < 4; ++i) {
                const f16x8_t ra = *reinterpret_cast<const f16x8_t*>(Hs + aoff[ks][0] + i * kHaloY * kHaloX * 8);
                const f16x8_t rb = *reinterpret_cast<const f16x8_t*>(Hs + aoff[ks][1] + i * kHaloY * kHaloX * 8);
                ah[i] = __builtin_shufflevector(ra, rb, 0, 1, 2, 3, 8, 9, 10, 11);
                al[i] = __builtin_shufflevector(ra, rb, 4, 5, 6, 7, 12, 13, 14, 15);
                ah[i] = __builtin_bit_cast(f16x8_t, __builtin_bit_cast(u32x4_h3, ah[i]) ^ rowm);
                al[i] = __builtin_bit_cast(f16x8_t, __builtin_bit_cast(u32x4_h3, al[i]) ^ rowm);
            }
#pragma unroll
            for (int j = 0; j < 5; ++j) {
                const f16* wb = Wt + ks * 4 * 160 * 8 + boff + j * 16 * 8;
                const f16x8_t bh = *reinterpret_cast<const f16x8_t*>(wb);
                const f16x8_t bl = *reinterpret_cast<const f16x8_t*>(wb + kThinInHalfs / 2);
#pragma unroll
                for (int i = 0; i < 4; ++i) {
                    mfma16h(acc[i][j], al[i], bh);
                    mfma16h(acc[i][j], ah[i], bl);
                    mfma16h(acc[i][j], ah[i], bh);
                }
            }
        }
#pragma unroll
        for (int i = 0; i < 4; ++i)
#pragma unroll
            for (int j = 0; j < 5; ++j)
#pragma unroll
                for (int r = 0; r < 4; ++r) acc[i][j][r] *= ((rsgn >> (4 * (lane >> 4) + r)) & 1) ? -inv : inv;
        if constexpr (EPI == kEpiMask)
            conv_epilogue_h3<kEpiMask, 5, false>(a, acc, Es, pw, nh * 80, lane, b, pt, tyy * 2, txx * 2, nT, nY, nX, op, opmax,
                                          cpart ? cpart + (long)tile * 160 : nullptr);
        else
            conv_epilogue_f32<EPI, 5>(a, acc, Es, pw, nh * 80, lane, b, pt, tyy * 2, txx * 2, nT, nY, nX);
    }
}

template <bool GW>
__global__ void __launch_bounds__(256, GW ? 2 : 1) conv3d_thin_out_f16x3_kernel(ConvF32Args a, const f16* wimg,
                                                                                const unsigned* xmax, int ntiles) {
    constexpr int WCH = 9 * 2 * 4 * 16 * 8;
    __shared__ __attribute__((aligned(16))) f16 smem_to3[kHalo * 64 + (GW ? 8 : WCH)];
    f16* Hs = smem_to3;
    f16* Wk = smem_to3 + kHalo * 64;
    float* Q = reinterpret_cast<float*>(smem_to3);
    const float sx = f16x3_scale(*xmax);
    const float inv = 1.0f / (sx * *reinterpret_cast<const float*>(wimg + kThinOutHalfs));
    const int nT = a.D >> 2, nY = a.H >> 2, nX = a.W >> 2;
    const int nYt = (nY + 1) >> 1, nXt = (nX + 1) >> 1;
    const int lane = threadIdx.x & 63, wave = __builtin_amdgcn_readfirstlane(threadIdx.x >> 6);
    const int m = lane & 15, kg = lane >> 4;
    int hb[5];
#pragma unroll
    for (int i = 0; i < 5; ++i) {
        const int r = 16 * (5 * wave + i) + m;
        const int xp = r % 10, y = (r / 10) % 8, t = r / 80;
        hb[i] = (t * kHaloY + y) * kHaloX + xp;
    }
    constexpr int NQ = kHalo * 8;
    constexpr int HPER = (NQ + 255) / 256;
    f32x4_t hr[HPER];
    auto load_halo = [&](int b, int pt, int tyy, int txx, int cc) {
#pragma unroll
        for (int k = 0; k < HPER; ++k) {
            const int i = threadIdx.x + k * 256;
            const int hv = i >> 3, q = i & 7;
            const int ht = hv / (kHaloY * kHaloX), hy = (hv / kHaloX) % kHaloY, hx = hv % kHaloX;
            const int t = pt * 4 - 1 + ht, y = tyy * 8 - 1 + hy, x = txx * 8 - 1 + hx;
            const bool ok = i < NQ && t >= 0 && t < a.D && y >= 0 && y < a.H && x >= 0 && x < a.W;
            hr[k] = ldz4f(a.in + brow(b, ok ? t : 0, ok ? y : 0, ok ? x : 0, nT, nY, nX) * a.cin_ld + cc * 32 + q * 4, ok);
        }
    };
    auto store_halo = [&]() {
#pragma unroll
        for (int k = 0; k < HPER; ++k) {
            const int i = threadIdx.x + k * 256;
            if (i < NQ) {
                const int hv = i >> 3, q = i & 7;
                const int swz = ((hv >> 1) & 3) << 1;
                f16x4_t h, l;
#pragma unroll
                for (int e = 0; e < 4; ++e) {
                    f16 hh, ll;
                    split_f16(hr[k][e], sx, hh, ll);
                    h[e] = hh;
                    l[e] = ll;
                }
                f16* row = Hs + hv * 64 + (q & 1) * 4;
                *reinterpret_cast<f16x4_t*>(row + (((q >> 1) ^ swz) << 3)) = h;
                *reinterpret_cast<f16x4_t*>(row + (((4 + (q >> 1)) ^ swz) << 3)) = l;
            }
        }
    };
    auto store_w = [&](int cc) {
        const uint4* src = reinterpret_cast<const uint4*>(wimg + cc * WCH);
        for (int it = threadIdx.x; it < WCH / 8; it += 256) reinterpret_cast<uint4*>(Wk)[it] = src[it];
    };
    const XcdWalk wk(ntiles);
    for (int tile = wk.t; tile < wk.end; tile += wk.step) {
        int bid = tile;
        const int txx = bid % nXt; bid /= nXt;
        const int tyy = bid % nYt; bid /= nYt;
        const int pt = bid % nT;
        const int b = bid / nT;
        f32x4_t acc[5];
#pragma unroll
        for (int i = 0; i < 5; ++i) acc[i] = (f32x4_t)0.0f;
        load_halo(b, pt, tyy, txx, 0);
        for (int cc = 0; cc < 5; ++cc) {
            __syncthreads();
            store_halo();
            if (!GW) store_w(cc);
            __syncthreads();
            if (cc + 1 < 5) load_halo(b, pt, tyy, txx, cc + 1);
// ... 279 lines not shown
                *reinterpret_cast<f16x8_t*>(ThinC + 8192 + n * 64 + c * 8) = lv;
            }
        }
    };

    f32x16 acc[5];
#pragma unroll
    for (int i = 0; i < 5; ++i) acc[i] = (f32x16)0.0f;
    const int r = lane & 31, h = lane >> 5;
    const int nt = wave & 3, kh2 = wave >> 2;
    const int nrow = 32 * nt + r;
    load(p0);
    store(0);
    if (p0 + 1 < p1) load(p0 + 1);
    __syncthreads();
    for (int patch = p0; patch < p1; ++patch) {
        const int cur = (patch - p0) & 1;
        const f16* BigT = smem_tw + cur * kTwgBuf;
        const f16* ThinC = BigT + kTwgBig;
#pragma unroll
        for (int kk = 0; kk < 2; ++kk) {
            const int c = 2 * (2 * kh2 + kk) + h;
            const f16* bp = ThinC + nrow * 64 + ((c ^ ((nrow >> 1) & 7)) << 3);
            const f16x8_t bh = *reinterpret_cast<const f16x8_t*>(bp);
            const f16x8_t bl = *reinterpret_cast<const f16x8_t*>(bp + 8192);
#pragma unroll
            for (int mt = 0; mt < 5; ++mt) {
                const int brw = 32 * mt + r;
                const f16* ap = BigT + brw * 64 + ((c ^ ((brw >> 1) & 7)) << 3);
                const f16x8_t ah = *reinterpret_cast<const f16x8_t*>(ap);
                const f16x8_t al = *reinterpret_cast<const f16x8_t*>(ap + 10240);
                mfma32h(acc[mt], al, bh);
                mfma32h(acc[mt], ah, bl);
                mfma32h(acc[mt], ah, bh);
            }
        }
        if (patch + 1 < p1) {
            store(cur ^ 1);
            if (patch + 2 < p1) load(patch + 2);
        }
        __syncthreads();
    }
    float* X = reinterpret_cast<float*>(smem_tw);
    if (kh2 == 1) {
#pragma unroll
        for (int mt = 0; mt < 5; ++mt)
#pragma unroll
            for (int q = 0; q < 16; ++q) X[((nt * 5 + mt) * 16 + q) * 64 + lane] = acc[mt][q];
    }
    __syncthreads();
    if (kh2 == 0) {
        const int n = 32 * nt + r, tap = n >> 2, sc = n & 3;
        if (tap < 27 && sc < a.thin_ch) {
#pragma unroll
            for (int mt = 0; mt < 5; ++mt)
#pragma unroll
                for (int q = 0; q < 16; ++q) {
                    const int bch = 32 * mt + (q & 3) + 8 * (q >> 2) + 4 * h;
                    const int co = a.big_is_co ? bch : sc, ci = a.big_is_co ? sc : bch;
                    const float v = acc[mt][q] + X[((nt * 5 + mt) * 16 + q) * 64 + lane];
                    atomicAdd(a.dw + ((long)tap * a.cout_pad + co) * a.cin_pad + ci, v * inv);
                }
        }
    }
    if (a.colsum && big_task) {
#pragma unroll
        for (int e = 0; e < 4; ++e) atomicAdd(a.colsum + 4 * cq + e, csum[e]);
    }
}

static bool thin_out_v1() {
    static const bool v = [] { const char* e = dlcs_knob("DLCS_THIN_OUT_V2"); return !(e && e[0] == '1'); }();
    return v;
}

static int conv_thin_f16x3_launch(const ConvF32Args& v, const f16* wimg, const unsigned* xmax, int cin, bool thin_in,
                                  hipStream_t st, f16* op = nullptr, const unsigned* opmax = nullptr,
                                  float* cpart = nullptr) {
    const int nT = v.D / 4, nY = v.H / 4, nX = v.W / 4;
    const int ntiles = (int)((long)v.B * nT * ((nY + 1) / 2) * ((nX + 1) / 2));
    const dim3 g(256);
    if (thin_in) {
        int epi;
        if (!v.res && !v.mask && !v.mplanes && !v.accumulate) epi = 0;
        else if (!v.res && (v.mask || v.mplanes) && !v.accumulate) epi = kEpiMask;
        else epi = kEpiGeneric;
        if ((op || cpart || v.mplanes) && epi != kEpiMask) return DLCS_ERR_UNSUPPORTED_SIZE;
        if (epi == 0)
            hipLaunchKernelGGL(conv3d_thin_in_f16x3_kernel<0>, g, dim3(512), 0, st, v, wimg, xmax, cin, ntiles, op, opmax,
                               cpart);
        else if (epi == kEpiMask)
            hipLaunchKernelGGL(conv3d_thin_in_f16x3_kernel<kEpiMask>, g, dim3(512), 0, st, v, wimg, xmax, cin, ntiles, op,
                               opmax, cpart);
        else
            hipLaunchKernelGGL(conv3d_thin_in_f16x3_kernel<kEpiGeneric>, g, dim3(512), 0, st, v, wimg, xmax, cin, ntiles,
                               op, opmax, cpart);
    } else if (thin_out_v1()) {
        static const bool gw = [] { const char* e = dlcs_knob("DLCS_THIN_OUT_GW"); return !(e && e[0] == '0'); }();
        if (gw) hipLaunchKernelGGL(conv3d_thin_out_f16x3_kernel<true>, dim3(512), dim3(256), 0, st, v, wimg, xmax, ntiles);
        else hipLaunchKernelGGL(conv3d_thin_out_f16x3_kernel<false>, g, dim3(256), 0, st, v, wimg, xmax, ntiles);
    } else {
        hipLaunchKernelGGL(conv3d_thin_out_f16x3_v2_kernel, g, dim3(256), 0, st, v, wimg, xmax, ntiles);
    }
    return dlcs_launch_status();
}
```

### dl-swin-gan_amd/dl_cs/_lib.py

```python
import ctypes
import os

import torch

_HERE = os.path.dirname(os.path.abspath(__file__))
LIB_PATH = os.environ.get("DLCS_HIP_LIB", os.path.join(_HERE, "libdlcs_hip.so"))

F32, BF16 = 0, 1
_LIB = None

_P = ctypes.c_void_p
_I64 = ctypes.c_int64
_INT = ctypes.c_int
_F = ctypes.c_float
_SZ = ctypes.c_size_t

SIGNATURES = {
    "dlcs_version": [],
    "dlcs_status_string": [_INT],
    "dlcs_scratch_bytes": [],
    "dlcs_release_scratch": [],
    "dlcs_sense_workspace_bytes": [_I64, _I64, _I64, _I64, _I64],
    "dlcs_sense_fwd": [_P, _P, _P, _I64, _P, _I64, _I64, _I64, _I64, _I64, _I64, _P, _SZ, _P],
    "dlcs_sense_adj": [_P, _P, _P, _I64, _P, _P, _P, _F, _I64, _I64, _I64, _I64, _I64, _I64, _P, _SZ, _P],
    "dlcs_sense_normal": [_P, _P, _P, _I64, _P, _P, _F, _F, _I64, _I64, _I64, _I64, _I64, _I64, _P, _SZ, _P],
    "dlcs_sense_cg_workspace_bytes": [_I64] * 6,
    "dlcs_sense_cg": [_P, _P, _P, _P, _I64, _F, _INT, _I64, _I64, _I64, _I64, _I64, _I64, _P, _SZ, _P],
    "dlcs_sense_rowtab_bytes": [_I64] * 4,
    "dlcs_sense_rowtab": [_P, _I64, _I64, _I64, _I64, _I64, _P, _SZ, _P],
    "dlcs_sense_rows_workspace_bytes": [_I64] * 5,
    "dlcs_sense_adj_rows": [_P, _P, _P, _I64, _P, _I64, _P, _P, _P, _F, _I64, _I64, _I64, _I64, _I64, _I64, _P,
                            _SZ, _P],
    "dlcs_sense_normal_rows": [_P, _P, _P, _I64, _P, _I64, _P, _P, _F, _F, _I64, _I64, _I64, _I64, _I64, _I64, _P,
                               _SZ, _P],
    "dlcs_sense_cg_rows": [_P, _P, _P, _P, _I64, _P, _I64, _F, _INT, _I64, _I64, _I64, _I64, _I64, _I64, _P, _SZ, _P],
    "dlcs_fft2": [_P, _P, _I64, _I64, _I64, _INT, _P, _SZ, _P],
    "dlcs_fft_plan": [_I64, _P, _P],
    "dlcs_window_index": [_I64] * 10 + [_P, _P, _P, _P],
    "dlcs_gather_rows": [_INT, _INT, _P, _P, _P, _I64, _I64, _I64, _I64, _P],
    "dlcs_layernorm_fwd": [_INT, _P, _P, _P, _P, _F, _P, _P, _P, _I64, _I64, _P],
    "dlcs_layernorm_bwd_workspace_bytes": [_I64, _I64],
    "dlcs_layernorm_bwd": [_P, _P, _P, _P, _P, _P, _P, _P, _P, _P, _I64, _I64, _P, _SZ, _P],
    "dlcs_colsum": [_INT, _P, _I64, _I64, _I64, _P, _P],
    "dlcs_gemm": [_INT, _I64, _I64, _I64, _P, _I64, _INT, _P, _I64, _INT, _P, _I64, _INT,
                  _P, _INT, _P, _P, _I64, _F, _P, _I64, _INT, _F, _P, _I64, _INT, _F, _P, _INT, _INT, _P],
    "dlcs_gemm_dw_workspace_bytes": [_INT, _P, _P, _I64],
    "dlcs_gemm_dw_grouped": [_INT, _P, _P, _P, _P, _P, _P, _P, _P, _P, _I64, _P, _SZ, _P],
    "dlcs_gemm_dw_grouped_f32": [_INT, _P, _P, _P, _P, _P, _P, _P, _P, _P, _I64, _P, _SZ, _P],
    "dlcs_window_attn_fwd": [_INT, _P, _P, _P, _P, _P, _P, _I64, _I64, _I64, _I64, _I64,
                             _I64, _I64, _I64, _F, _P],
    "dlcs_window_attn_bwd": [_INT, _P, _P, _P, _P, _P, _P, _P, _I64, _P, _P, _I64, _I64, _I64, _I64,
                             _I64, _I64, _I64, _F, _P],
    "dlcs_conv3d_k3": [_INT, _P, _I64, _I64, _P, _I64, _P, _P, _INT, _I64, _I64, _I64, _I64, _I64, _I64,
                       _I64, _INT, _P, _I64, _P, _INT, _I64, _F, _INT, _INT, _P],
    "dlcs_conv3d_k3_wgrad": [_INT, _P, _I64, _I64, _I64, _INT, _P, _I64, _I64, _I64, _P, _P, _I64, _I64, _I64,
                             _I64, _I64, _P],
    "dlcs_conv3d_pack_weights": [_INT, _P, _P, _I64, _I64, _I64, _I64, _INT, _P],
    "dlcs_conv3d_unpack_wgrad": [_P, _P, _I64, _I64, _I64, _I64, _INT, _P],
    "dlcs_split2_f16_bytes": [_I64],
    "dlcs_split2_f16": [_P, _I64, _I64, _P, _INT, _P, _P],
    "dlcs_conv3d_pack_weights_f16x3_bytes": [],
    "dlcs_conv3d_pack_weights_f16x3": [_P, _INT, _P, _P],
    "dlcs_gemm_k160_f16x3": [_P, _I64, _P, _I64, _P, _I64, _P, _INT, _F, _P, _I64, _F, _P, _I64, _F, _INT, _P, _P, _P,
                             _P, _P, _P],
    "dlcs_planes_bound": [_P, _I64, _P, _P, _F, _P, _P, _F, _P, _I64, _F, _P],
    "dlcs_abs_row_sum_max": [_P, _I64, _I64, _I64, _I64, _I64, _P, _P],
    "dlcs_h3r_pack_bytes": [_I64, _I64],
    "dlcs_h3r_pack_multi": [_INT, _P, _P, _P, _P, _P, _P, _P],
    "dlcs_gemm_h3r": [_P, _I64, _I64, _I64, _P, _I64, _P, _I64, _P, _INT, _P, _P, _I64, _F, _P, _I64, _P, _INT, _P],
    "dlcs_f8r_quant": [_P, _I64, _I64, _I64, _P, _P, _P],
    "dlcs_gemm_f8r": [_P, _P, _I64, _I64, _P, _P, _I64, _P, _I64, _P, _INT, _P, _I64, _F, _P, _I64, _P, _P],
    "dlcs_linear_k160_f16x3": [_P, _I64, _P, _I64, _P, _I64, _P, _INT, _P, _P, _I64, _F, _P, _I64, _P, _INT, _P],
    "dlcs_gemm_f32_splitk_det": [_P, _I64, _P, _I64, _I64, _I64, _I64, _P, _P, _SZ, _P],
    "dlcs_gemm_f32_splitk_det_workspace_bytes": [_I64, _I64],
    "dlcs_conv3d_k3_wgrad_f16x3": [_P, _P, _P, _I64, _I64, _I64, _I64, _P],
    "dlcs_conv3d_k3_f16x3": [_P, _P, _P, _P, _I64, _I64, _I64, _I64, _I64, _P, _I64, _P, _I64, _F, _INT, _INT, _P, _P, _P,
                             _P, _P],
    "dlcs_conv3d_thin_pack_f16x3_bytes": [_INT],
    "dlcs_conv3d_thin_pack_f16x3": [_P, _I64, _I64, _I64, _I64, _INT, _P, _P],
    "dlcs_absmax_f32": [_P, _I64, _P, _P],
    "dlcs_conv3d_thin_f16x3": [_P, _I64, _I64, _P, _P, _P, _P, _I64, _I64, _I64, _I64, _I64, _I64, _P, _I64, _P,
                               _I64, _F, _INT, _INT, _P, _P, _P, _P, _P],
    "dlcs_conv3d_thin_out_planes_f16x3": [_P, _P, _P, _P, _I64, _I64, _I64, _I64, _I64, _I64, _INT, _INT, _P],
    "dlcs_conv3d_thin_wgrad_planes_f16x3": [_P, _P, _I64, _I64, _P, _INT, _P, _I64, _I64, _I64, _I64, _I64, _I64,
                                            _P],
    "dlcs_conv3d_thin_wgrad_f16x3": [_P, _I64, _I64, _P, _P, _I64, _I64, _P, _P, _I64, _I64, _P, _I64, _I64, _I64,
                                     _I64, _P],
    "dlcs_swin_pre": [_INT, _P, _P, _I64, _I64, _I64, _I64, _I64, _I64, _I64, _P],
    "dlcs_swin_pre_bwd": [_INT, _P, _P, _I64, _I64, _I64, _I64, _I64, _I64, _I64, _P],
    "dlcs_swin_post": [_INT, _P, _P, _I64, _I64, _I64, _I64, _I64, _I64, _I64, _P],
    "dlcs_swin_post_bwd": [_INT, _P, _P, _I64, _I64, _I64, _I64, _I64, _I64, _I64, _P],
    "dlcs_axpby": [_INT, _INT, _P, _P, _I64, _F, _F, _P],
    "dlcs_relu_grad": [_INT, _P, _INT, _P, _I64, _P],
    "dlcs_permute": [_INT, _INT, _P, _P, _I64, _P, _P, _INT, _P],
    "dlcs_fill_bias": [_P, _P, _I64, _I64, _I64, _P],
    "dlcs_block_layout": [_INT, _INT, _P, _P, _I64, _I64, _I64, _I64, _I64, _I64, _INT, _P],
    "dlcs_cast_multi_bf16": [_I64, _P, _P, _P, _P],
    "dlcs_kt_window_average": [_P, _P, _I64, _I64, _I64, _I64, _INT, _P],
    "dlcs_kth_largest_abs": [_P, _I64, _I64, _P, _P],
    "dlcs_cplx_mask_scale": [_P, _P, _P, _I64, _I64, _I64, _P, _INT, _P],
    "dlcs_crop_flip": [_P, _P, _I64, _I64, _I64, _I64, _I64, _I64, _I64, _I64, _INT, _INT, _INT, _P],
    "dlcs_mhsa_fwd": [_INT, _P, _P, _P, _I64, _I64, _I64, _I64, _F, _P],
    "dlcs_mhsa_bwd_workspace_bytes": [_I64, _I64, _I64],
    "dlcs_mhsa_bwd": [_INT, _P, _P, _P, _P, _P, _I64, _I64, _I64, _I64, _F, _P, _SZ, _P],
    "dlcs_conv3d_thin_im2col": [_P, _I64, _I64, _P, _I64, _INT, _I64, _I64, _I64, _I64, _P],
    "dlcs_conv3d_thin_col2im": [_P, _I64, _I64, _P, _I64, _P, _INT, _INT, _I64, _I64, _I64, _I64, _P],
    "dlcs_dit_vec": [_INT, _P, _P, _P, _I64, _P],
    "dlcs_timestep_embedding": [_P, _I64, _I64, _F, _P, _P],
    "dlcs_scale_rows": [_P, _P, _P, _P, _P, _I64, _I64, _P],
    "dlcs_gated_linear_grad": [_P, _P, _P, _P, _P, _P, _P, _P, _I64, _I64, _P],
    "dlcs_rows_add": [_P, _P, _P, _I64, _I64, _P],
}
DIAG_SIGNATURES = {
    "dlcs_conv3d_k3_x6": [_P, _P, _P, _P, _P, _I64, _I64, _I64, _I64, _I64, _P, _I64, _P, _I64, _F, _INT,
                          _INT, _P],
    "dlcs_split3_bf16": [_P, _I64, _I64, _P, _P, _P],
    "dlcs_conv3d_k3_wgrad_x6": [_P, _P, _P, _P, _P, _I64, _I64, _I64, _I64, _P],
    "dlcs_gemm_nt_x6": [_P, _I64, _P, _I64, _I64, _I64, _I64, _P, _P, _SZ, _P],
    "dlcs_gemm_nt_x6_workspace_bytes": [_I64, _I64, _I64],
    "dlcs_debug_conv_stamps": [_P, _I64],
    "dlcs_debug_h3_stamps": [_P, _I64],
}
_RESTYPE = {"dlcs_status_string": ctypes.c_char_p, "dlcs_scratch_bytes": _SZ, "dlcs_sense_workspace_bytes": _SZ,
            "dlcs_sense_cg_workspace_bytes": _SZ, "dlcs_sense_rowtab_bytes": _SZ,
            "dlcs_sense_rows_workspace_bytes": _SZ, "dlcs_split2_f16_bytes": _SZ,
            "dlcs_conv3d_pack_weights_f16x3_bytes": _SZ, "dlcs_conv3d_thin_pack_f16x3_bytes": _SZ,
            "dlcs_gemm_dw_workspace_bytes": _SZ, "dlcs_layernorm_bwd_workspace_bytes": _SZ,
            "dlcs_gemm_f32_splitk_det_workspace_bytes": _SZ, "dlcs_gemm_nt_x6_workspace_bytes": _SZ,
            "dlcs_h3r_pack_bytes": _SZ, "dlcs_mhsa_bwd_workspace_bytes": _SZ}


class DlcsError(RuntimeError):
    pass


def lib():
    global _LIB
    if _LIB is None:
        if not os.path.exists(LIB_PATH):
            raise DlcsError(f"libdlcs_hip.so not found at {LIB_PATH}; build it with "
                            "`make -C dl-swin-gan_amd/csrc` (or __graft_entry__.build())")
        L = ctypes.CDLL(LIB_PATH)
        for name, args in SIGNATURES.items():
            fn = getattr(L, name)
            fn.argtypes = args
            fn.restype = _RESTYPE.get(name, _INT)
        for name, args in DIAG_SIGNATURES.items():
            if hasattr(L, name):
                fn = getattr(L, name)
                fn.argtypes = args
                fn.restype = _RESTYPE.get(name, _INT)
        _LIB = L
    return _LIB


def exported_symbols():
    return sorted(SIGNATURES.keys())


def scratch_bytes():
    return int(lib().dlcs_scratch_bytes())


def release_scratch():
    check(lib().dlcs_release_scratch(), "dlcs_release_scratch")


def has_symbol(name):
    return hasattr(lib(), name)


def check(status, name):
    if status != 0:
        msg = lib().dlcs_status_string(int(status))
        raise DlcsError(f"{name} failed with status {status}: {msg.decode() if msg else '?'}")


def call(name, *args):
    check(getattr(lib(), name)(*args), name)


_RAW_STREAM = getattr(torch._C, "_cuda_getCurrentRawStream", None)
_GET_DEVICE = getattr(torch._C, "_cuda_getDevice", None)


def stream():
    if _RAW_STREAM is not None and _GET_DEVICE is not None:
        return ctypes.c_void_p(_RAW_STREAM(_GET_DEVICE()))
    return ctypes.c_void_p(torch.cuda.current_stream().cuda_stream)


def ptr(t):
    return None if t is None else ctypes.c_void_p(t.data_ptr())


def require_gpu(*tensors):
    for t in tensors:
        if t is not None and not t.is_cuda:
            raise DlcsError("dl_cs HIP ops need GPU tensors (no CPU fallback in the product path)")


def dtype_code(dt):
    if dt == torch.float32:
        return F32
    if dt == torch.bfloat16:
        return BF16
    raise DlcsError(f"unsupported dtype {dt}")
```

### dl-swin-gan_amd/dl_cs/models/_ops.py

```python
import ctypes

import torch

from .. import _lib
from .. import diag as _diag

F32, BF16 = _lib.F32, _lib.BF16
_I64P = ctypes.POINTER(ctypes.c_int64)


def code(t_or_dtype):
    dt = t_or_dtype.dtype if torch.is_tensor(t_or_dtype) else t_or_dtype
    return _lib.dtype_code(dt)


p = _lib.ptr
S = _lib.stream
call = _lib.call


def empty(shape, dtype, device):
    return torch.empty(shape, dtype=dtype, device=device)


# ... 262 lines not shown

def attn_bwd(qkv, out, dout, lse, table, labels, dtable, nwin, N, heads, hd, window0, scale,
             mask=None, mask_nw=0):
    dqkv = empty(qkv.shape, torch.float32, qkv.device)
    call("dlcs_window_attn_bwd", code(qkv), p(qkv), p(out), p(dout), p(lse), p(table), p(labels),
         p(mask), int(mask_nw), p(dqkv), p(dtable), nwin, N, heads, hd, window0[0], window0[1],
         window0[2], float(scale), S())
    return dqkv


def pad32(n):
    return (n + 31) // 32 * 32


def conv_pack(w, dtype, mode):
    cout, cin = w.shape[0], w.shape[1]
    rows, cols = (pad32(cout), pad32(cin)) if mode == 0 else (pad32(cin), pad32(cout))
    out = empty((27, rows, cols), dtype, w.device)
    call("dlcs_conv3d_pack_weights", code(out), p(w.contiguous()), p(out), cout, cin, rows, cols, mode, S())
    return out


def conv3d(x, cin, packed, cout, out_ld, grid, bias=None, out=None, out_dtype=None, relu_in=0,
           mask=None, res=None, res_scale=1.0, accumulate=0, relu_out=0):
    B, D, H, W = grid
    rows = B * D * H * W
    if out is None:
        out = empty((rows, out_ld), out_dtype or x.dtype, x.device)
    call("dlcs_conv3d_k3", code(x), p(x), cin, x.shape[-1], p(packed), packed.shape[2], p(bias),
         p(out), code(out), cout, packed.shape[1], out.shape[-1], B, D, H, W, int(relu_in),
         p(mask), mask.shape[-1] if mask is not None else 0, p(res),
         code(res) if res is not None else F32, res.shape[-1] if res is not None else 0,
         float(res_scale), int(accumulate), int(relu_out), S())
    return out


def split3(x, out=None):
    rows = x.shape[0]
    if out is None:
        out = (empty((rows, 320), torch.bfloat16, x.device), empty((rows, 160), torch.bfloat16, x.device))
    call("dlcs_split3_bf16", p(x), rows, x.shape[-1], p(out[0]), p(out[1]), S())
    return out


def conv_pack_x6(w, mode):
    packed = empty((27 * 160 * 480,), torch.bfloat16, w.device)
    call("dlcs_conv3d_pack_weights", F32, p(w.contiguous()), p(packed), 160, 160, 0, 0, 2 + mode, S())
    return packed


def conv3d_x6(planes, packed, grid, bias=None, out=None, mask=None, res=None, res_scale=1.0, accumulate=0,
              relu_out=0):
    B, D, H, W = grid
    xa, xb = planes
    if out is None:
        out = empty((xa.shape[0], 160), torch.float32, xa.device)
    call("dlcs_conv3d_k3_x6", p(xa), p(xb), p(packed), p(bias), p(out), out.shape[-1], B, D, H, W, p(mask),
         mask.shape[-1] if mask is not None else 0, p(res), res.shape[-1] if res is not None else 0,
         float(res_scale), int(accumulate), int(relu_out), S())
    return out


def conv3d_wgrad_x6(x_planes, g_planes, grid, dw_packed):
    B, D, H, W = grid
    call("dlcs_conv3d_k3_wgrad_x6", p(x_planes[0]), p(x_planes[1]), p(g_planes[0]), p(g_planes[1]), p(dw_packed),
         B, D, H, W, S())
    return dw_packed


def split2(x, out=None, have_max=False, colsum=None):
    rows = x.shape[0]
    if out is None:
        out = empty((int(_lib.lib().dlcs_split2_f16_bytes(rows)),), torch.uint8, x.device)
    call("dlcs_split2_f16", p(x), rows, x.shape[-1], p(out), int(bool(have_max)), p(colsum), S())
    return out


def planes_alloc(rows, device):
    out = empty((int(_lib.lib().dlcs_split2_f16_bytes(rows)),), torch.uint8, device)
    out[rows * 640:rows * 640 + 4].zero_()
    return out


def planes_max(planes, rows):
    return ctypes.c_void_p(planes.data_ptr() + rows * 640)


def conv_pack_f16x3(w, mode):
    packed = empty((int(_lib.lib().dlcs_conv3d_pack_weights_f16x3_bytes()),), torch.uint8, w.device)
    call("dlcs_conv3d_pack_weights_f16x3", p(w.contiguous()), int(mode), p(packed), S())
    return packed


def conv3d_f16x3(planes, packed, grid, bias=None, out=None, mask=None, res=None, res_scale=1.0, accumulate=0,
                 relu_out=0, out_max=None, out_planes=None, colsum=None, planes_only=False, mask_planes=None):
    B, D, H, W = grid
    rows = B * D * H * W
    if out is None and not planes_only:
        out = empty((rows, 160), torch.float32, planes.device)
    call("dlcs_conv3d_k3_f16x3", p(planes), p(packed), p(bias), p(out), out.shape[-1] if out is not None else 160,
         B, D, H, W, p(mask), mask.shape[-1] if mask is not None else 0, p(res), res.shape[-1] if res is not None else 0,
         float(res_scale), int(accumulate), int(relu_out), out_max, p(out_planes), p(colsum), p(mask_planes), S())
    return out


def gemm_k160_f16x3(a_planes, M, b_planes, N, C, bias=None, act=0, alpha=1.0, res=None, res_scale=1.0,
                    res2=None, res2_scale=1.0, accumulate=0, out_max=None, out_planes=None, colsum=None,
                    res_planes=None, res2_planes=None):
    call("dlcs_gemm_k160_f16x3", p(a_planes), M, p(b_planes), N, p(C), C.shape[-1] if C is not None else N,
         p(bias), int(act), float(alpha), p(res), res.shape[-1] if res is not None else 0, float(res_scale),
         p(res2), res2.shape[-1] if res2 is not None else 0, float(res2_scale), int(accumulate), out_max,
         p(out_planes), p(colsum), p(res_planes), p(res2_planes), S())
    return C


def _w(m):
    if m is None or isinstance(m, ctypes.c_void_p):
        return m
    return p(m)


def planes_bound(planes, rows, m0=None, n0=None, c0=1.0, m1=None, n1=None, c1=1.0, vec=None, cvec=1.0):
    call("dlcs_planes_bound", p(planes), rows, _w(m0), _w(n0), float(c0), _w(m1), _w(n1), float(c1), p(vec),
         vec.numel() if vec is not None else 0, float(cvec), S())
    return planes


def abs_row_sum_max(w, rows, row_stride, inner, n_outer=1, outer_stride=0, out=None):
    if out is None:
        out = empty((1,), torch.int32, w.device)
    call("dlcs_abs_row_sum_max", p(w), rows, row_stride, n_outer, outer_stride, inner, p(out), S())
    return out


def linear_k160_f16x3(x_planes, M, w_planes, N, out, bias=None, act=0, aux=None, aux_out=None, alpha=1.0,
                      res=None, row_map=None, accumulate=0):
    ldaux = (aux if aux is not None else aux_out).shape[-1] if (aux is not None or aux_out is not None) else 0
    call("dlcs_linear_k160_f16x3", p(x_planes), M, p(w_planes), N, p(out), out.shape[-1], p(bias), int(act),
         p(aux), p(aux_out), ldaux, float(alpha), p(res), res.shape[-1] if res is not None else 0, p(row_map),
         int(accumulate), S())
    return out


def conv3d_wgrad_f16x3(x_planes, g_planes, grid, dw_packed):
    B, D, H, W = grid
    call("dlcs_conv3d_k3_wgrad_f16x3", p(x_planes), p(g_planes), p(dw_packed), B, D, H, W, S())
    return dw_packed


def absmax(x, out=None):
    if out is None:
        out = zeros((1,), torch.int32, x.device)
    call("dlcs_absmax_f32", p(x), x.numel(), p(out), S())
    return out


def _word(m):
    return m if isinstance(m, ctypes.c_void_p) else p(m)


def thin_pack_f16x3(packed, cout, cin, kind):
    out = empty((int(_lib.lib().dlcs_conv3d_thin_pack_f16x3_bytes(kind)),), torch.uint8, packed.device)
    call("dlcs_conv3d_thin_pack_f16x3", p(packed), cout, packed.shape[1], cin, packed.shape[2], int(kind), p(out), S())
    return out


def conv3d_thin_f16x3(x, cin, x_max, wthin, cout, out_ld, grid, bias=None, out=None, mask=None, res=None,
                      res_scale=1.0, accumulate=0, relu_out=0, out_max=None, out_planes=None, colsum=None,
                      planes_only=False, mask_planes=None):
    B, D, H, W = grid
    rows = B * D * H * W
    if out is None and not planes_only:
        out = empty((rows, out_ld), torch.float32, x.device)
    call("dlcs_conv3d_thin_f16x3", p(x), cin, x.shape[-1], _word(x_max), p(wthin), p(bias), p(out), cout,
         out.shape[-1] if out is not None else 160, B, D, H, W, p(mask), mask.shape[-1] if mask is not None else 0,
         p(res), res.shape[-1] if res is not None else 0, float(res_scale), int(accumulate), int(relu_out),
         _word(out_max) if out_max is not None else None, p(out_planes), p(colsum), p(mask_planes), S())
    return out


def conv3d_thin_wgrad_f16x3(x, cin, x_max, g, cout, g_max, grid, dw_packed, colsum=None):
    B, D, H, W = grid
    call("dlcs_conv3d_thin_wgrad_f16x3", p(x), cin, x.shape[-1], _word(x_max), p(g), cout, g.shape[-1],
         _word(g_max), p(dw_packed), dw_packed.shape[1], dw_packed.shape[2], p(colsum), B, D, H, W, S())
    return dw_packed


def conv3d_thin_out_planes(planes, wthin, cout, out_ld, grid, bias=None, out=None, accumulate=0, relu_out=0):
    B, D, H, W = grid
    rows = B * D * H * W
    if out is None:
        out = empty((rows, out_ld), torch.float32, planes.device)
    call("dlcs_conv3d_thin_out_planes_f16x3", p(planes), p(wthin), p(bias), p(out), cout, out.shape[-1], B, D, H, W,
         int(accumulate), int(relu_out), S())
    return out


def conv3d_thin_wgrad_planes(big_planes, thin, thin_ch, thin_max, big_is_co, grid, dw_packed):
    B, D, H, W = grid
    call("dlcs_conv3d_thin_wgrad_planes_f16x3", p(big_planes), p(thin), thin_ch, thin.shape[-1], _word(thin_max),
         int(big_is_co), p(dw_packed), dw_packed.shape[1], dw_packed.shape[2], B, D, H, W, S())
    return dw_packed


def conv3d_wgrad(x, cin, relu_in, g, cout, grid, dw_packed, vox_per_block=16384, dbias=None):
    B, D, H, W = grid
    call("dlcs_conv3d_k3_wgrad", code(x), p(x), cin, x.shape[-1], dw_packed.shape[2], int(relu_in),
         p(g), cout, g.shape[-1], dw_packed.shape[1], p(dw_packed), p(dbias), B, D, H, W, vox_per_block, S())
    return dw_packed


def conv_unpack_grad(dw_packed, grad, cout, cin, accumulate=1):
    call("dlcs_conv3d_unpack_wgrad", p(dw_packed), p(grad), cout, cin, dw_packed.shape[1],
         dw_packed.shape[2], int(accumulate), S())
    return grad


def swin_pre(x, dtype, pad, ldc):
    B, E, T, Y, X = x.shape
    u = empty((B * (T + 2 * pad) * Y * X, ldc), dtype, x.device)
    call("dlcs_swin_pre", code(dtype), p(x), p(u), B, E, T, Y, X, pad, ldc, S())
    return u


def swin_pre_bwd(gu, shape, pad):
    B, E, T, Y, X = shape
    gx = empty(shape, torch.complex64, gu.device)
    call("dlcs_swin_pre_bwd", code(gu), p(gu), p(gx), B, E, T, Y, X, pad, gu.shape[-1], S())
    return gx


def swin_post(o, shape, pad):
    B, E, T, Y, X = shape
    out = empty(shape, torch.complex64, o.device)
    call("dlcs_swin_post", code(o), p(o), p(out), B, E, T, Y, X, pad, o.shape[-1], S())
    return out


def swin_post_bwd(gout, dtype, pad, ldc):
    B, E, T, Y, X = gout.shape
    go = empty((B * (T + 2 * pad) * Y * X, ldc), dtype, gout.device)
    call("dlcs_swin_post_bwd", code(dtype), p(gout), p(go), B, E, T, Y, X, pad, ldc, S())
    return go


def relu_grad(g, a):
    assert g.numel() == a.numel()
    call("dlcs_relu_grad", code(g), p(g), code(a), p(a), g.numel(), S())
    return g
```

### dl-swin-gan_amd/dl_cs/models/engine.py

```python
import ctypes
import math
import weakref


import torch

from .. import diag as _diag
from . import _ops as K
from ._window import get_window_size as get_window_size_tuple


class BlockWeights:

    NAMES = ("norm1.weight", "norm1.bias", "attn.relative_position_bias_table", "attn.qkv.weight",
             "attn.qkv.bias", "attn.proj.weight", "attn.proj.bias", "norm2.weight", "norm2.bias",
             "mlp.fc1.weight", "mlp.fc1.bias", "mlp.fc2.weight", "mlp.fc2.bias")

    LINEARS = ("attn.qkv.weight", "attn.proj.weight", "mlp.fc1.weight", "mlp.fc2.weight")

    def __init__(self, params, dtype, cast=None, hr=None):
        self.p = params
        w = cast if cast is not None else [K.cast(params[n], dtype) for n in self.LINEARS]
        self.wqkv, self.wproj, self.wfc1, self.wfc2 = w
        self.hr = None
# ... 250 lines not shown
        if depth and h3r_ok(dtype, *[bp[0][n] for n in BlockWeights.LINEARS]):
            flat = K.h3r_pack([(b[n], t) for b in bp for t in (False, True) for n in BlockWeights.LINEARS])
            hrs = [flat[8 * i:8 * i + 8] for i in range(depth)]
        if dtype == torch.bfloat16:
            flat = K.cast_multi_bf16([b[n] for b in bp for n in BlockWeights.LINEARS])
            casts = [flat[4 * i:4 * i + 4] for i in range(depth)]
        self.blocks = [BlockWeights(bp[i], dtype, casts[i], hrs[i]) for i in range(depth)]


class NetWeights:

    def __init__(self, params, dtype, depth, nstages=1):
        self.p = params
        self.dtype = dtype
        C = params["SFE.layers.2.conv.bias"].shape[0]
        self.split = _use_split(dtype, C)
        self.x6 = self.h3_patch = self.split
        self.sfe = K.conv_pack(params["SFE.layers.2.conv.weight"], dtype, 0)
        self.fin = K.conv_pack(params["final_layer.layers.2.conv.weight"], dtype, 0)
        dfe = params["dfe_tail.weight"]
        self.dfe = K.conv_pack_f16x3(dfe, 0) if self.split else K.conv_pack(dfe, dtype, 0)
        self.dfe_norm = _conv_norm(dfe, C) if self.split else None
        self.thin_h3 = self.split and not THIN_F32
        if self.thin_h3:
            cin = params["SFE.layers.2.conv.weight"].shape[1]
            self.sfe_h3 = K.thin_pack_f16x3(self.sfe, C, cin, 0)
            self.fin_h3 = K.thin_pack_f16x3(self.fin, cin, C, 1)
        self.stages = [StageWeights(params, f"rs{k}.", dtype, depth, self.split) for k in range(nstages)]


def _stage_swin_forward(W, st, inp, geos, ntok, heads, drops):
    dtype, P = W.dtype, W.p
    C = st.emb.shape[0]
    if dtype == torch.float32 and st.emb_h3r is not None:
        tok = K.linear_h3r(inp.view(ntok, 64 * C), st.emb_h3r, C, bias=P[st.pre + "patch_embed.proj.bias"])
    else:
        tok = K.fill_bias(K.empty((ntok, C), torch.float32, inp.device), P[st.pre + "patch_embed.proj.bias"],
                          ntok, C, C)
        if dtype == torch.float32 and W.split and EMBED_X6:
            K.gemm_nt_x6(inp, st.emb, tok, ntok, C, 64 * C, 64 * C, 64 * C)
        elif dtype == torch.float32:
            K.gemm_f32_splitk_det(inp, st.emb, tok, ntok, C, 64 * C, 64 * C, 64 * C)
        else:
            K.gemm(inp, st.emb, tok, ntok, C, 64 * C, 64 * C, 64 * C, C, accumulate=1, splitk=1)
    bsaved = []
    for i, bw in enumerate(st.blocks):
        ds = drops[i] if drops is not None else (1.0, 1.0)
        tok, sv = block_forward(bw, geos[i], tok, dtype, heads, drop_scale=ds)
        bsaved.append(sv)
    return K.cast(tok, dtype), bsaved


def swinnet_forward(W, x, heads=8, window=(7, 8, 8), pad=4, drop_scales=None):
    dtype = W.dtype
    P = W.p
    B, E, T, Y, X = x.shape
    Tp = T + 2 * pad
    if Tp % 4 or Y % 4 or X % 4:
        raise NotImplementedError("dl_cs HIP path: T+2*pad, Y and X must be multiples of 4")
    grid = (B, Tp, Y, X)
    C = P["SFE.layers.2.conv.bias"].shape[0]
    cin = 2 * E
    dev = x.device
    rows = B * Tp * Y * X
    flops = _conv_flops(grid, C, C)
    u = K.swin_pre(x.contiguous(), dtype, pad, PAD_CIN)
    mx = K.zeros((2 * len(W.stages) + 2,), torch.int32, dev) if W.split else None
    word = (lambda i: ctypes.c_void_p(mx.data_ptr() + 4 * i)) if W.split else None
    if W.thin_h3:
        umax = K.absmax(u)
        s = K.conv3d_thin_f16x3(u, cin, umax, W.sfe_h3, C, C, grid, bias=P["SFE.layers.2.conv.bias"],
                                out_max=word(0) if W.split else None)
    else:
        umax = None
        s = K.conv3d(u, cin, W.sfe, C, C, grid, bias=P["SFE.layers.2.conv.bias"])
        if W.split:
            K.absmax(s, out=mx[0:1])
    nT, nY, nX = Tp // 4, Y // 4, X // 4
    ntok = B * nT * nY * nX
    depth = len(W.stages[0].blocks)
    geos = [SwinGeometry(B, nT, nY, nX, window, i % 2 == 1, dev) for i in range(depth)]
    nst = len(W.stages)
    stages = []
    inp, pout = s, None
    inp_max = word(0) if W.split else None
    fwd_po = (W.split and not K160_F32 and W.thin_h3 and THIN_PLANES and CAPTURE is None and
              DGRAD_CAPTURE is None and FWD_PLANES_ONLY)
    for k, st in enumerate(W.stages):
        last = k == nst - 1
        tok_t, bsaved = _stage_swin_forward(W, st, inp, geos, ntok, heads,
                                            drop_scales[k] if drop_scales is not None else None)
        a = None if fwd_po else K.empty((rows, C), dtype, dev)
        ss = dict(inp=inp, tok_t=tok_t, bsaved=bsaved, a=a)
        tb = P[st.pre + "swin_tail.bias"]
        if W.split:
            pa = K.planes_alloc(rows, dev)
            amax, omax = word(1 + 2 * k), word(2 + 2 * k)
            if K160_F32:
                K.gemm(tok_t, st.unemb, a, ntok, 64 * C, C, C, C, 64 * C, bias=st.unemb_bias, act=3)
                K.split2(a, out=pa)
                K.absmax(a, out=mx[1 + 2 * k:2 + 2 * k])
            else:
                tp = K.split2(tok_t)
                K.planes_bound(pa, rows, m0=K.planes_max(tp, ntok), n0=st.unemb_norm, vec=st.unemb_bias)
                K.gemm_k160_f16x3(tp, ntok, st.unemb_h3, 64 * C, a.view(ntok, 64 * C) if a is not None else None,
                                  bias=st.unemb_bias, act=3, out_max=amax, out_planes=pa)
            ss["planes"] = pa
            if last:
                pb = K.planes_alloc(rows, dev)
                K.planes_bound(pb, rows, m0=amax, n0=st.tail_norm, m1=inp_max, vec=tb)
                out = _timed("conv_fwd", flops, K.conv3d_f16x3, ss["planes"], st.tail, grid, bias=tb, res=inp,
                             relu_out=1, out_max=omax, out_planes=pb, planes_only=fwd_po)
                pout = pb
            else:
                out = _timed("conv_fwd", flops, K.conv3d_f16x3, ss["planes"], st.tail, grid, bias=tb, res=inp,
                             out_max=omax)
            inp_max = omax
        else:
            K.gemm(tok_t, st.unemb, a, ntok, 64 * C, C, C, C, 64 * C, bias=st.unemb_bias, act=3)
            out = _timed_conv(a, C, st.tail, C, C, grid, bias=tb, res=inp, relu_out=int(last))
        ss["out"] = out
        stages.append(ss)
        inp = out
    b = inp
    ph = None
    if W.split:
        hmax = mx[-1:]
        if W.thin_h3 and THIN_PLANES:
            ph = K.planes_alloc(rows, dev)
            K.planes_bound(ph, rows, m0=inp_max, n0=W.dfe_norm, m1=word(0), c1=2.0, vec=P["dfe_tail.bias"])
        h = _timed("conv_fwd", flops, K.conv3d_f16x3, pout, W.dfe, grid, bias=P["dfe_tail.bias"], res=s,
                   res_scale=2.0, relu_out=1, out_max=K.p(hmax), out_planes=ph, planes_only=fwd_po)
        if ph is not None:
            o = K.conv3d_thin_out_planes(ph, W.fin_h3, cin, PAD_CIN, grid, bias=P["final_layer.layers.2.conv.bias"])
        elif W.thin_h3:
            o = K.conv3d_thin_f16x3(h, C, hmax, W.fin_h3, cin, PAD_CIN, grid,
                                    bias=P["final_layer.layers.2.conv.bias"])
        else:
            o = K.conv3d(h, C, W.fin, cin, PAD_CIN, grid, bias=P["final_layer.layers.2.conv.bias"],
                         out_dtype=torch.float32)
    else:
        hmax = None
        h = _timed_conv(b, C, W.dfe, C, C, grid, bias=P["dfe_tail.bias"], res=s, res_scale=2.0, relu_out=1)
        o = K.conv3d(h, C, W.fin, cin, PAD_CIN, grid, bias=P["final_layer.layers.2.conv.bias"],
                     out_dtype=torch.float32)
    out = K.swin_post(o, (B, E, T, Y, X), pad)
    saved = dict(u=u, s=s, b=b, pout=pout, h=h, ph=ph, stages=stages, geos=geos, shape=(B, E, T, Y, X), grid=grid,
                 pad=pad, heads=heads, cin=cin, C=C, ntok=ntok, umax=umax, hmax=hmax)
    if CAPTURE is not None:
        CAPTURE.append(dict(relu_inputs=[ss["a"] for ss in stages] + [b, h], grid=grid, C=C))
    return out, saved


def swinnet_backward(W, sv, gout, grads):
    dtype = W.dtype
    P = W.p
    grid, pad, C, cin, ntok = sv["grid"], sv["pad"], sv["C"], sv["cin"], sv["ntok"]
    dev = gout.device
    rows = grid[0] * grid[1] * grid[2] * grid[3]
    flops = _conv_flops(grid, C, C)
    go = K.swin_post_bwd(gout.contiguous(), dtype, pad, PAD_CIN)
    gout_planes = W.split and not K160_F32 and DGRAD_CAPTURE is None

    def conv_grads(x_in, cin_, g, cout, wname, bname):
        dwp = torch.zeros((27, K.pad32(cout), K.pad32(cin_)), dtype=torch.float32, device=dev)
        if cin_ == C and cout == C:
            _timed("conv_wgrad", flops, K.conv3d_wgrad, x_in, cin_, 0, g, cout, grid, dwp, dbias=grads[bname])
        else:
            K.conv3d_wgrad(x_in, cin_, 0, g, cout, grid, dwp, dbias=grads[bname])
        K.conv_unpack_grad(dwp, grads[wname], cout, cin_)

    def split_wgrad(x_planes, g_planes, wname):
        dwp = torch.zeros((27, C, C), dtype=torch.float32, device=dev)
        _timed("conv_wgrad", flops, K.conv3d_wgrad_f16x3, x_planes, g_planes, grid, dwp)
        K.conv_unpack_grad(dwp, grads[wname], C, C)

    wf = K.conv_pack(P["final_layer.layers.2.conv.weight"], dtype, 1)
    if W.split:
        pg = K.planes_alloc(rows, dev)
        if W.thin_h3:
            gomax = K.absmax(go)
            if gout_planes:
                ghm = K.zeros((1,), torch.int32, dev)
                K.planes_bound(pg, rows, m0=gomax, n0=_conv_norm(P["final_layer.layers.2.conv.weight"], C, dgrad=True))
                K.conv3d_thin_f16x3(go, cin, gomax, K.thin_pack_f16x3(wf, C, cin, 0), C, C, grid, mask=sv["h"],
                                    mask_planes=sv["ph"] if sv["h"] is None else None, out_max=K.p(ghm),
                                    out_planes=pg, planes_only=True, colsum=grads["dfe_tail.bias"])
                g_h = None
            else:
                g_h = K.conv3d_thin_f16x3(go, cin, gomax, K.thin_pack_f16x3(wf, C, cin, 0), C, C, grid, mask=sv["h"],
                                          out_max=K.planes_max(pg, rows))
            dwp = torch.zeros((27, K.pad32(cin), C), dtype=torch.float32, device=dev)
            if sv["ph"] is not None:
                K.conv3d_thin_wgrad_planes(sv["ph"], go, cin, gomax, 0, grid, dwp)
            else:
                K.conv3d_thin_wgrad_f16x3(sv["h"], C, sv["hmax"], go, cin, gomax, grid, dwp)
            K.conv_unpack_grad(dwp, grads["final_layer.layers.2.conv.weight"], cin, C)
            K.colsum(go, grads["final_layer.layers.2.conv.bias"], rows=rows, C=cin, ld=go.shape[-1])
        else:
            g_h = K.conv3d(go, cin, wf, C, C, grid, relu_in=0, mask=sv["h"])
            conv_grads(sv["h"], C, go, cin, "final_layer.layers.2.conv.weight", "final_layer.layers.2.conv.bias")
        if g_h is None:
            gp = gh_pl = pg
            ghmax = ghm
        else:
            gh_pl = None
            gp = K.split2(g_h, out=pg, have_max=W.thin_h3, colsum=grads["dfe_tail.bias"])
            ghmax = gp[rows * 640:rows * 640 + 4].view(torch.int32).clone()
        pg = K.planes_alloc(rows, dev)
        if gout_planes:
            gom = K.zeros((1,), torch.int32, dev)
            K.planes_bound(pg, rows, m0=ghmax, n0=_conv_norm(P["dfe_tail.weight"], C, dgrad=True))
            _timed("conv_dgrad", flops, K.conv3d_f16x3, gp, K.conv_pack_f16x3(P["dfe_tail.weight"], 1), grid,
                   mask=sv["b"], mask_planes=sv["pout"] if sv["b"] is None else None, out_max=K.p(gom),
                   out_planes=pg, planes_only=True,
                   colsum=grads[W.stages[-1].pre + "swin_tail.bias"])
            g_out = None
        else:
            g_out = _timed("conv_dgrad", flops, K.conv3d_f16x3, gp, K.conv_pack_f16x3(P["dfe_tail.weight"], 1), grid,
                           mask=sv["b"], out_max=K.planes_max(pg, rows))
        split_wgrad(sv["pout"], gp, "dfe_tail.weight")
        del gp
        if DGRAD_CAPTURE is not None:
            DGRAD_CAPTURE.append(("dfe_tail", g_h, sv["b"], P["dfe_tail.weight"], g_out))
    else:
        g_h = K.conv3d(go, cin, wf, C, C, grid, relu_in=0, mask=sv["h"])
        conv_grads(sv["h"], C, go, cin, "final_layer.layers.2.conv.weight", "final_layer.layers.2.conv.bias")
        w2 = K.conv_pack(P["dfe_tail.weight"], dtype, 1)
        g_out = _timed("conv_dgrad", flops, K.conv3d, g_h, C, w2, C, C, grid, mask=sv["b"])
        conv_grads(sv["b"], C, g_h, C, "dfe_tail.weight", "dfe_tail.bias")
    gsmax = None
    pgs = None
    gout_pl = None
    for k in reversed(range(len(W.stages))):
        st, ss = W.stages[k], sv["stages"][k]
        pre = st.pre
        if W.split:
            if g_out is None:
                gp = gout_pl = pg
                gomax = gom
            else:
                gout_pl = None
                gp = K.split2(g_out, out=pg, have_max=True, colsum=grads[pre + "swin_tail.bias"])
                gomax = gp[rows * 640:rows * 640 + 4].view(torch.int32).clone()
            g_a = _timed("conv_dgrad", flops, K.conv3d_f16x3, gp, K.conv_pack_f16x3(P[pre + "swin_tail.weight"], 1),
                         grid, mask=ss["a"], mask_planes=ss["planes"] if ss["a"] is None else None)
            split_wgrad(ss["planes"], gp, pre + "swin_tail.weight")
            del gp
            if DGRAD_CAPTURE is not None:
                DGRAD_CAPTURE.append((pre + "swin_tail", g_out, ss["a"], P[pre + "swin_tail.weight"], g_a))
        else:
            w1 = K.conv_pack(P[pre + "swin_tail.weight"], dtype, 1)
            g_a = _timed("conv_dgrad", flops, K.conv3d, g_out, C, w1, C, C, grid, mask=ss["a"])
            conv_grads(ss["a"], C, g_out, C, pre + "swin_tail.weight", pre + "swin_tail.bias")
        d_tok = (K.empty if st.unemb_dx is not None else K.zeros)((ntok, C), torch.float32, dev)
        if st.unemb_dx is not None:
            K.linear_h3r(g_a.view(ntok, 64 * C), st.unemb_dx, C, out=d_tok)
        elif st.unembT is not None:
            K.gemm_nt_x6(g_a, st.unembT, d_tok, ntok, C, 64 * C, 64 * C, 64 * C)
        else:
            K.gemm(g_a, st.unemb, d_tok, ntok, C, 64 * C, 64 * C, C, C, b_trans=1, accumulate=1, splitk=16)
        if DGRAD_CAPTURE is not None:
            DGRAD_CAPTURE.append((pre + "unembed_dx", g_a, None, st.unemb, d_tok))
        g_a_tok = g_a.view(ntok, 64 * C)
        if K.dw_grouped_ok(ntok, [(g_a_tok, ss["tok_t"])]):
            K.gemm_dw_grouped(ntok, [(g_a_tok, ss["tok_t"], grads[pre + "unemb_packed"],
                                      grads[pre + "patch_unembed.proj.bias"], C)])
        else:
            K.gemm(g_a, ss["tok_t"], grads[pre + "unemb_packed"], 64 * C, C, ntok, 64 * C, C, C, a_trans=1,
                   b_trans=1, accumulate=1, splitk=max(1, min(16, ntok // 256)))
            K.colsum(g_a, grads[pre + "patch_unembed.proj.bias"], rows=rows, C=C, ld=C)
        del g_a, g_a_tok
        for i in reversed(range(len(st.blocks))):
            bg = {n: grads[f"{pre}blocks.{i}.{n}"] for n in BlockWeights.NAMES}
            d_tok = block_backward(st.blocks[i], sv["geos"][i], ss["bsaved"][i], d_tok, bg, dtype, sv["heads"])
        d_tok_t = K.cast(d_tok, dtype)
        first = k == 0
        planes_only = W.split and not K160_F32 and first and W.thin_h3 and THIN_PLANES
        g_in = None if planes_only else K.empty((rows, C), dtype, dev)
        if W.split and K160_F32:
            pg = K.planes_alloc(rows, dev)
            if first:
                K.gemm(d_tok_t, st.emb, g_in, ntok, 64 * C, C, C, 64 * C, 64 * C, b_trans=1,
                       res=g_h, ldr=64 * C, res_scale=2.0, res2=g_out, ldr2=64 * C)
                gsmax = K.absmax(g_in)
            else:
                K.gemm(d_tok_t, st.emb, g_in, ntok, 64 * C, C, C, 64 * C, 64 * C, b_trans=1, res=g_out, ldr=64 * C)
                K.absmax(g_in, out=pg[rows * 640:rows * 640 + 4].view(torch.int32))
        elif W.split:
            if first:
                dtp = K.split2(d_tok_t)
                if planes_only:
                    pgs = K.planes_alloc(rows, dev)
                    gsmax = None
                    K.planes_bound(pgs, rows, m0=K.planes_max(dtp, ntok), n0=st.embT_norm, m1=ghmax, c1=2.0,
                                   vec=gomax.view(torch.float32))
                    K.gemm_k160_f16x3(dtp, ntok, st.embT_h3, 64 * C, None,
                                      res=g_h.view(ntok, 64 * C) if g_h is not None else None, res_planes=gh_pl,
                                      res_scale=2.0, res2=g_out.view(ntok, 64 * C) if g_out is not None else None,
                                      res2_planes=gout_pl, out_planes=pgs, colsum=grads["SFE.layers.2.conv.bias"])
                else:
                    gsmax = K.zeros((1,), torch.int32, dev)
                    K.gemm_k160_f16x3(dtp, ntok, st.embT_h3, 64 * C, g_in.view(ntok, 64 * C),
                                      res=g_h.view(ntok, 64 * C) if g_h is not None else None, res_planes=gh_pl,
                                      res_scale=2.0, res2=g_out.view(ntok, 64 * C) if g_out is not None else None,
                                      res2_planes=gout_pl, out_max=K.p(gsmax))
            else:
                pg = K.planes_alloc(rows, dev)
                K.gemm_k160_f16x3(K.split2(d_tok_t), ntok, st.embT_h3, 64 * C, g_in.view(ntok, 64 * C),
                                  res=g_out.view(ntok, 64 * C) if g_out is not None else None, res_planes=gout_pl,
                                  out_max=K.planes_max(pg, rows))
        elif first:
            K.gemm(d_tok_t, st.emb, g_in, ntok, 64 * C, C, C, 64 * C, 64 * C, b_trans=1,
                   res=g_h, ldr=64 * C, res_scale=2.0, res2=g_out, ldr2=64 * C)
        else:
            K.gemm(d_tok_t, st.emb, g_in, ntok, 64 * C, C, C, 64 * C, 64 * C, b_trans=1, res=g_out, ldr=64 * C)
        in_tok = ss["inp"].view(ntok, 64 * C)
        if K.dw_grouped_ok(ntok, [(d_tok_t, in_tok)]):
            K.gemm_dw_grouped(ntok, [(d_tok_t, in_tok, grads[pre + "emb_packed"], grads[pre + "patch_embed.proj.bias"],
                                      0)])
        else:
            K.gemm(d_tok_t, ss["inp"], grads[pre + "emb_packed"], C, 64 * C, ntok, C, 64 * C, 64 * C, a_trans=1,
                   b_trans=1, accumulate=1, splitk=max(1, min(16, ntok // 256)))
            K.colsum(d_tok, grads[pre + "patch_embed.proj.bias"])
        g_out = g_in
    g_s_t = g_out
    wsfe = K.conv_pack(P["SFE.layers.2.conv.weight"], dtype, 1)
    if pgs is not None:
        if g_s_t is not None:
# ... 25 lines not shown
```

### include/dlcs.h

```cpp
#ifndef DLCS_H
#define DLCS_H

#include <stddef.h>
#include <stdint.h>

#ifdef __cplusplus
extern "C" {
#endif

#define DLCS_VERSION 1

enum dlcs_dtype { DLCS_F32 = 0, DLCS_BF16 = 1 };

enum dlcs_status {
    DLCS_OK = 0,
    DLCS_ERR_INVALID_ARG = 100001,
    DLCS_ERR_UNSUPPORTED_SIZE = 100002,
    DLCS_ERR_WORKSPACE = 100003
};

typedef void* dlcs_stream_t;

int dlcs_version(void);
const char* dlcs_status_string(int status);
// ... 35 lines not shown
                        void* workspace, size_t workspace_bytes, dlcs_stream_t stream);
int dlcs_sense_cg_rows(void* x, const void* b, const void* maps, const float* weights, int64_t weights_coils,
                       const void* table, int64_t jcap, float lamda, int num_iter,
                       int64_t B, int64_t E, int64_t C, int64_t T, int64_t Y, int64_t X,
                       void* workspace, size_t workspace_bytes, dlcs_stream_t stream);

int dlcs_fft2(const void* in, void* out, int64_t nplanes, int64_t Y, int64_t X, int inverse,
              void* workspace, size_t workspace_bytes, dlcs_stream_t stream);

int dlcs_fft_plan(int64_t n, int* kind, int* padded_len);


int dlcs_window_index(int64_t B, int64_t D, int64_t H, int64_t W, int64_t wd, int64_t wh, int64_t ww,
                      int64_t sd, int64_t sh, int64_t sw, int32_t* part_src, int32_t* rev_dst,
                      int32_t* labels, dlcs_stream_t stream);

int dlcs_gather_rows(int src_dtype, int dst_dtype, const void* src, const int32_t* idx, void* dst,
                     int64_t nrows, int64_t C, int64_t ld_src, int64_t ld_dst, dlcs_stream_t stream);

int dlcs_layernorm_fwd(int out_dtype, const float* x, const int32_t* src_map, const float* gamma,
                       const float* beta, float eps, void* out, float* mean, float* rstd,
                       int64_t rows, int64_t C, dlcs_stream_t stream);
size_t dlcs_layernorm_bwd_workspace_bytes(int64_t rows, int64_t C);
int dlcs_layernorm_bwd(const float* dy, const float* x, const int32_t* src_map, const float* gamma,
                       const float* mean, const float* rstd, const float* dx_in, float* dx, float* dgamma, float* dbeta,
                       int64_t rows, int64_t C, void* workspace, size_t workspace_bytes,
                       dlcs_stream_t stream);

int dlcs_colsum(int dtype, const void* x, int64_t rows, int64_t C, int64_t ld, float* out, dlcs_stream_t stream);

int dlcs_gemm(int dtype, int64_t M, int64_t N, int64_t K,
              const void* A, int64_t lda, int a_trans,
              const void* B, int64_t ldb, int b_trans,
              void* C, int64_t ldc, int c_dtype,
              const float* bias, int act, const void* aux, void* aux_out, int64_t ldaux, float alpha,
              const void* residual, int64_t ldr, int r_dtype, float res_scale,
              const void* residual2, int64_t ldr2, int r2_dtype, float res2_scale,
              const int32_t* row_map, int accumulate, int splitk, dlcs_stream_t stream);

size_t dlcs_gemm_dw_workspace_bytes(int ngroups, const int64_t* M, const int64_t* N, int64_t T);
int dlcs_gemm_dw_grouped(int ngroups, const void* const* A, const int64_t* lda, const void* const* B,
                         const int64_t* ldb, const int64_t* M, const int64_t* N, float* const* dW,
                         float* const* db, const int64_t* db_period, int64_t T, void* workspace,
                         size_t workspace_bytes, dlcs_stream_t stream);
int dlcs_gemm_dw_grouped_f32(int ngroups, const void* const* A, const int64_t* lda, const void* const* B,
                             const int64_t* ldb, const int64_t* M, const int64_t* N, float* const* dW,
                             float* const* db, const int64_t* db_period, int64_t T, void* workspace,
                             size_t workspace_bytes, dlcs_stream_t stream);

int dlcs_window_attn_fwd(int dtype, const void* qkv, void* out, float* lse, const float* table,
                         const int32_t* labels, const float* mask, int64_t mask_nw, int64_t nwin,
                         int64_t N, int64_t heads, int64_t head_dim,
                         int64_t wd0, int64_t wh0, int64_t ww0, float scale, dlcs_stream_t stream);
int dlcs_window_attn_bwd(int dtype, const void* qkv, const void* out, const void* dout, const float* lse,
                         const float* table, const int32_t* labels, const float* mask, int64_t mask_nw,
                         float* dqkv, float* dtable,
                         int64_t nwin, int64_t N, int64_t heads, int64_t head_dim,
                         int64_t wd0, int64_t wh0, int64_t ww0, float scale, dlcs_stream_t stream);

int dlcs_conv3d_k3(int dtype, const void* in, int64_t cin, int64_t cin_ld, const void* wpacked,
                   int64_t cin_pad, const float* bias, void* out, int out_dtype, int64_t cout,
                   int64_t cout_pad, int64_t cout_ld, int64_t B, int64_t D, int64_t H, int64_t W,
                   int relu_in, const void* mask, int64_t mask_ld, const void* residual, int res_dtype,
                   int64_t res_ld, float res_scale, int accumulate, int relu_out, dlcs_stream_t stream);
int dlcs_conv3d_k3_wgrad(int dtype, const void* in, int64_t cin, int64_t cin_ld, int64_t cin_pad, int relu_in,
                         const void* gout, int64_t cout, int64_t g_ld, int64_t cout_pad, float* dw_packed,
                         float* dbias, int64_t B, int64_t D, int64_t H, int64_t W, int64_t vox_per_block,
                         dlcs_stream_t stream);
int dlcs_conv3d_pack_weights(int dtype, const float* w, void* packed, int64_t cout, int64_t cin,
                             int64_t rows_pad, int64_t cols_pad, int mode, dlcs_stream_t stream);
#ifdef DLCS_DIAG_BUILD
int dlcs_conv3d_k3_x6(const void* xa, const void* xb, const void* wpacked, const float* bias, float* out,
                      int64_t cout_ld, int64_t B, int64_t D, int64_t H, int64_t W, const float* mask, int64_t mask_ld,
                      const float* residual, int64_t res_ld, float res_scale, int accumulate, int relu_out,
                      dlcs_stream_t stream);
int dlcs_conv3d_k3_wgrad_x6(const void* xa, const void* xb, const void* ga, const void* gb, float* dw_packed,
                            int64_t B, int64_t D, int64_t H, int64_t W, dlcs_stream_t stream);
int dlcs_split3_bf16(const float* x, int64_t rows, int64_t ld, void* xa, void* xb, dlcs_stream_t stream);
int dlcs_debug_conv_stamps(void* host, int64_t n);
int dlcs_debug_h3_stamps(void* host, int64_t n);
#endif

size_t dlcs_split2_f16_bytes(int64_t rows);
int dlcs_split2_f16(const float* x, int64_t rows, int64_t ld, void* planes, int have_max, float* colsum,
                    dlcs_stream_t stream);
size_t dlcs_conv3d_pack_weights_f16x3_bytes(void);
int dlcs_conv3d_pack_weights_f16x3(const float* w, int mode, void* packed, dlcs_stream_t stream);
int dlcs_conv3d_k3_f16x3(const void* xplanes, const void* wpacked, const float* bias, float* out, int64_t cout_ld,
                         int64_t B, int64_t D, int64_t H, int64_t W, const float* mask, int64_t mask_ld,
                         const float* residual, int64_t res_ld, float res_scale, int accumulate, int relu_out,
                         unsigned* out_max, void* out_planes, float* colsum, const void* mask_planes,
                         dlcs_stream_t stream);
int dlcs_gemm_k160_f16x3(const void* aplanes, int64_t M, const void* bplanes, int64_t N, float* C, int64_t ldc,
                         const float* bias, int act, float alpha, const float* residual, int64_t ldr, float res_scale,
                         const float* residual2, int64_t ldr2, float res2_scale, int accumulate, unsigned* out_max,
                         void* out_planes, float* colsum, const void* res_planes, const void* res2_planes,
                         dlcs_stream_t stream);
int dlcs_planes_bound(void* planes, int64_t rows, const unsigned* m0, const unsigned* n0, float c0,
                      const unsigned* m1, const unsigned* n1, float c1, const float* vec, int64_t nvec, float cvec,
                      dlcs_stream_t stream);
int dlcs_abs_row_sum_max(const float* w, int64_t rows, int64_t row_stride, int64_t n_outer, int64_t outer_stride,
                         int64_t inner, unsigned* out, dlcs_stream_t stream);

int dlcs_linear_k160_f16x3(const void* xplanes, int64_t M, const void* wplanes, int64_t N, float* C, int64_t ldc,
                           const float* bias, int act, const float* aux, float* aux_out, int64_t ldaux, float alpha,
                           const float* residual, int64_t ldr, const int32_t* row_map, int accumulate,
                           dlcs_stream_t stream);

size_t dlcs_h3r_pack_bytes(int64_t rows, int64_t K);
int dlcs_h3r_pack_multi(int n, const float* const* src, const int64_t* ld, const int* trans, const int64_t* rows,
                        const int64_t* K, void* const* dst, dlcs_stream_t stream);
int dlcs_gemm_h3r(const float* A, int64_t M, int64_t K, int64_t lda, const void* bpacked, int64_t N, float* C,
                  int64_t ldc, const float* bias, int act, const float* aux, float* aux_out, int64_t ldaux, float alpha,
                  const float* residual, int64_t ldr, const int32_t* row_map, int accumulate, dlcs_stream_t stream);

int dlcs_f8r_quant(const float* x, int64_t rows, int64_t K, int64_t ld, void* q, float* inv, dlcs_stream_t stream);
int dlcs_gemm_f8r(const void* aq, const float* ainv, int64_t M, int64_t K, const void* bq, const float* binv,
                  int64_t N, float* C, int64_t ldc, const float* bias, int act, float* aux_out, int64_t ldaux,
                  float alpha, const float* residual, int64_t ldr, const int32_t* row_map, dlcs_stream_t stream);

size_t dlcs_gemm_f32_splitk_det_workspace_bytes(int64_t M, int64_t N);
int dlcs_gemm_f32_splitk_det(const float* A, int64_t lda, const float* B, int64_t ldb, int64_t M, int64_t N,
                             int64_t K, float* C, void* workspace, size_t workspace_bytes, dlcs_stream_t stream);
#ifdef DLCS_DIAG_BUILD
size_t dlcs_gemm_nt_x6_workspace_bytes(int64_t M, int64_t N, int64_t K);
int dlcs_gemm_nt_x6(const float* A, int64_t lda, const float* B, int64_t ldb, int64_t M, int64_t N, int64_t K,
                    float* C, void* workspace, size_t workspace_bytes, dlcs_stream_t stream);
#endif
int dlcs_conv3d_k3_wgrad_f16x3(const void* xplanes, const void* gplanes, float* dw_packed, int64_t B, int64_t D,
                               int64_t H, int64_t W, dlcs_stream_t stream);
int dlcs_absmax_f32(const float* x, int64_t n, unsigned* out, dlcs_stream_t stream);
size_t dlcs_conv3d_thin_pack_f16x3_bytes(int kind);
int dlcs_conv3d_thin_pack_f16x3(const float* wpacked, int64_t cout, int64_t cout_pad, int64_t cin, int64_t cin_pad,
                                int kind, void* out, dlcs_stream_t stream);
int dlcs_conv3d_thin_f16x3(const float* in, int64_t cin, int64_t cin_ld, const unsigned* in_max, const void* wthin,
                           const float* bias, float* out, int64_t cout, int64_t cout_ld, int64_t B, int64_t D,
                           int64_t H, int64_t W, const float* mask, int64_t mask_ld, const float* residual,
                           int64_t res_ld, float res_scale, int accumulate, int relu_out, unsigned* out_max,
                           void* out_planes, float* colsum, const void* mask_planes, dlcs_stream_t stream);
int dlcs_conv3d_thin_wgrad_f16x3(const float* in, int64_t cin, int64_t cin_ld, const unsigned* in_max,
                                 const float* g, int64_t cout, int64_t g_ld, const unsigned* g_max, float* dw_packed,
                                 int64_t cout_pad, int64_t cin_pad, float* colsum, int64_t B, int64_t D, int64_t H,
                                 int64_t W, dlcs_stream_t stream);
int dlcs_conv3d_thin_out_planes_f16x3(const void* xplanes, const void* wthin, const float* bias, float* out,
                                      int64_t cout, int64_t cout_ld, int64_t B, int64_t D, int64_t H, int64_t W,
                                      int accumulate, int relu_out, dlcs_stream_t stream);
int dlcs_conv3d_thin_wgrad_planes_f16x3(const void* bigplanes, const float* thin, int64_t thin_ch, int64_t thin_ld,
                                        const unsigned* thin_max, int big_is_co, float* dw_packed, int64_t cout_pad,
                                        int64_t cin_pad, int64_t B, int64_t D, int64_t H, int64_t W,
                                        dlcs_stream_t stream);
int dlcs_conv3d_unpack_wgrad(const float* dw_packed, float* grad, int64_t cout, int64_t cin, int64_t cout_pad,
                             int64_t cin_pad, int accumulate, dlcs_stream_t stream);

int dlcs_swin_pre(int dtype, const void* x, void* u, int64_t B, int64_t E, int64_t T, int64_t Y, int64_t X,
                  int64_t pad, int64_t ldc, dlcs_stream_t stream);
int dlcs_swin_pre_bwd(int dtype, const void* gu, void* gx, int64_t B, int64_t E, int64_t T, int64_t Y, int64_t X,
                      int64_t pad, int64_t ldc, dlcs_stream_t stream);
int dlcs_swin_post(int dtype, const void* o, void* out, int64_t B, int64_t E, int64_t T, int64_t Y, int64_t X,
                   int64_t pad, int64_t ldc, dlcs_stream_t stream);
int dlcs_swin_post_bwd(int dtype, const void* gout, void* go, int64_t B, int64_t E, int64_t T, int64_t Y, int64_t X,
                       int64_t pad, int64_t ldc, dlcs_stream_t stream);

int dlcs_relu_grad(int g_dtype, void* g, int a_dtype, const void* a, int64_t n, dlcs_stream_t stream);
int dlcs_axpby(int x_dtype, int y_dtype, const void* x, void* y, int64_t n, float a, float b, dlcs_stream_t stream);
int dlcs_permute(int src_dtype, int dst_dtype, const void* src, void* dst, int64_t ndim,
                 const int64_t* dst_shape, const int64_t* src_strides, int accumulate, dlcs_stream_t stream);
int dlcs_fill_bias(float* out, const float* bias, int64_t rows, int64_t C, int64_t period, dlcs_stream_t stream);
int dlcs_block_layout(int src_dtype, int dst_dtype, const void* src, void* dst, int64_t B, int64_t C, int64_t D,
                      int64_t H, int64_t W, int64_t ld, int inverse, dlcs_stream_t stream);

#define DLCS_CAST_MULTI_MAX 64
int dlcs_cast_multi_bf16(int64_t count, const float* const* src, void* const* dst, const int64_t* n,
                         dlcs_stream_t stream);

int dlcs_kt_window_average(const void* k, void* out, int64_t P, int64_t T, int64_t YX, int64_t window,
                           int full, dlcs_stream_t stream);
int dlcs_kth_largest_abs(const void* x, int64_t n, int64_t k, float* out, dlcs_stream_t stream);
int dlcs_cplx_mask_scale(const void* x, const float* mask, void* y, int64_t P, int64_t TYX, int64_t mask_planes,
                         const float* scale, int divide, dlcs_stream_t stream);
int dlcs_crop_flip(const void* in, void* out, int64_t P, int64_t T, int64_t Y, int64_t X, int64_t y0, int64_t ny,
                   int64_t x0, int64_t nx, int flip_t, int flip_y, int flip_x, dlcs_stream_t stream);

int dlcs_mhsa_fwd(int dtype, const void* qkv, void* out, float* lse, int64_t nseq, int64_t N, int64_t heads,
                  int64_t head_dim, float scale, dlcs_stream_t stream);
size_t dlcs_mhsa_bwd_workspace_bytes(int64_t nseq, int64_t N, int64_t heads);
int dlcs_mhsa_bwd(int dtype, const void* qkv, const void* out, const void* dout, const float* lse, float* dqkv,
                  int64_t nseq, int64_t N, int64_t heads, int64_t head_dim, float scale, void* workspace,
                  size_t workspace_bytes, dlcs_stream_t stream);

int dlcs_conv3d_thin_im2col(const float* src, int64_t ld_src, int64_t C, float* dst, int64_t ld_dst, int sign,
                            int64_t B, int64_t D, int64_t H, int64_t W, dlcs_stream_t stream);
int dlcs_conv3d_thin_col2im(const float* P, int64_t ld_p, int64_t C, float* out, int64_t ld_out, const float* bias,
                            int sign, int accumulate, int64_t B, int64_t D, int64_t H, int64_t W,
                            dlcs_stream_t stream);

int dlcs_dit_vec(int op, const float* a, const float* b, float* y, int64_t n, dlcs_stream_t stream);
int dlcs_timestep_embedding(const float* t, int64_t B, int64_t dim, float max_period, float* out,
                            dlcs_stream_t stream);
int dlcs_scale_rows(const float* W, const float* b, const float* gate, float* Wo, float* bo, int64_t N, int64_t K,
                    dlcs_stream_t stream);
int dlcs_gated_linear_grad(const float* W, const float* b, const float* G, const float* colsum, const float* gate,
                           float* dW, float* db, float* dgate, int64_t N, int64_t K, dlcs_stream_t stream);
int dlcs_rows_add(float* dst, const int32_t* idx, const float* src, int64_t nrows, int64_t C, dlcs_stream_t stream);

#ifdef __cplusplus
}
#endif
#endif
```

Before: 4.568.

## Store ReLU masks as packed bits in forward for backward masking

Forward conv and GEMM epilogues now also emit a one-bit-per-channel ReLU mask (20 bytes per row), staged through shared memory and written coalesced. Backward dgrad epilogues read these bits instead of loading both f16 planes (640 bytes per row) to recover the mask. This cuts epilogue memory traffic in the backward pass. The cost is extra forward stores, some extra shared-memory use, and a conversion kernel kept as a fallback when only planes are supplied.

Result: no change. 4.565 (-0.1%).

```diff
diff --git a/dl-swin-gan_amd/csrc/conv3d.hip b/dl-swin-gan_amd/csrc/conv3d.hip
--- a/dl-swin-gan_amd/csrc/conv3d.hip
+++ b/dl-swin-gan_amd/csrc/conv3d.hip
@@ -9,6 +9,7 @@
 namespace {
 
 enum ScratchSlot { kScrColsum, kScrH3r, kScrSplit2, kScrH3Tail, kScrWgH3, kScrTwp, kScrV6Tail, kScrBiasPart,
+                   kScrMaskBits,
                    kScrSlots };
 std::mutex g_scr_mu;
 std::map<std::tuple<int, int, hipStream_t>, std::pair<void*, size_t>> g_scr;
@@ -1852,6 +1853,7 @@
 #endif
 
 size_t dlcs_split2_f16_bytes(int64_t rows) { return (size_t)rows * 640 + 256 + 640; }
+size_t dlcs_relu_bits_bytes(int64_t rows) { return (size_t)rows * 20; }
 
 int dlcs_split2_f16(const float* x, int64_t rows, int64_t ld, void* planes, int have_max, float* colsum,
                     dlcs_stream_t stream) {
@@ -1892,6 +1894,14 @@
     return dlcs_launch_status();
 }
 
+static const unsigned char* mask_bits_of_planes(const void* mask_planes, long rows, hipStream_t st) {
+    unsigned char* bits = static_cast<unsigned char*>(scratch(kScrMaskBits, st, (size_t)rows * 20));
+    if (!bits) return nullptr;
+    hipLaunchKernelGGL(relu_bits_from_planes_kernel, dim3((unsigned)cdiv(rows * 20, 256)), dim3(256), 0, st,
+                       (const f16*)mask_planes, rows, bits);
+    return bits;
+}
+
 static float* colsum_part_workspace(hipStream_t st, long nwg) {
     return static_cast<float*>(scratch(kScrColsum, st, (size_t)nwg * 160 * sizeof(float)));
 }
@@ -1900,8 +1910,9 @@
                          int64_t B, int64_t D, int64_t H, int64_t W, const float* mask, int64_t mask_ld,
                          const float* residual, int64_t res_ld, float res_scale, int accumulate, int relu_out,
                          unsigned* out_max, void* out_planes, float* colsum, const void* mask_planes,
-                         dlcs_stream_t stream) {
-    DLCS_CHECK_ARG(xplanes && wpacked && B > 0 && (out || (out_planes && !accumulate)) && !(mask && mask_planes));
+                         void* out_bits, const void* mask_bits, dlcs_stream_t stream) {
+    DLCS_CHECK_ARG(xplanes && wpacked && B > 0 && (out || (out_planes && !accumulate)) &&
+                   (mask != nullptr) + (mask_planes != nullptr) + (mask_bits != nullptr) <= 1);
     if (!out) cout_ld = 160;
     auto al16 = [](const void* p) { return ((uintptr_t)p & 15) == 0; };
     const long rows = (long)B * D * H * W;
@@ -1918,7 +1929,9 @@
     v.cout_ld = (int)cout_ld; v.mask_ld = (int)mask_ld; v.res_ld = (int)res_ld; v.accumulate = accumulate;
     v.relu_out = relu_out; v.res_scale = res_scale; v.omax = out_max;
     if (mask_planes && !al16(mask_planes)) return DLCS_ERR_UNSUPPORTED_SIZE;
-    v.mplanes = mask_planes;
+    if (out_bits && !al16(out_bits)) return DLCS_ERR_UNSUPPORTED_SIZE;
+    v.mbits = (const unsigned char*)mask_bits;
+    v.obits = (unsigned char*)out_bits;
     if (out_planes) {
         if (cout_ld != 160 || !al16(out_planes)) return DLCS_ERR_UNSUPPORTED_SIZE;
         v.oplanes = (f16*)out_planes;
@@ -1930,6 +1943,7 @@
     v.exp = h3_exp;
 #endif
     hipStream_t st = (hipStream_t)stream;
+    if (mask_planes && !(v.mbits = mask_bits_of_planes(mask_planes, rows, st))) return (int)hipErrorOutOfMemory;
     const long ntile = (long)B * (D / 4) * ((H / 4 + 1) / 2) * ((W / 4 + 1) / 2);
     if (colsum) {
         v.cpart = colsum_part_workspace(st, ntile);
@@ -1960,7 +1974,7 @@
                          const float* bias, int act, float alpha, const float* residual, int64_t ldr, float res_scale,
                          const float* residual2, int64_t ldr2, float res2_scale, int accumulate, unsigned* out_max,
                          void* out_planes, float* colsum, const void* res_planes, const void* res2_planes,
-                         dlcs_stream_t stream) {
+                         void* out_bits, dlcs_stream_t stream) {
     DLCS_CHECK_ARG(aplanes && bplanes && M > 0 && N > 0 && (act == 0 || act == 3) &&
                    (C || (out_planes && !accumulate)) && !(residual && res_planes) && !(residual2 && res2_planes));
     if (!C) ldc = N;
@@ -1993,6 +2007,8 @@
         g.oplanes = (f16*)out_planes;
         g.opmax = (const unsigned*)((const char*)out_planes + M * (N / 160) * 640);
     }
+    if (out_bits && ldc != N) return DLCS_ERR_UNSUPPORTED_SIZE;
+    g.obits = (unsigned char*)out_bits;
     hipStream_t st = (hipStream_t)stream;
     const long nwg = cdiv(M, 64) * (N / 160);
     if (colsum) {
@@ -2204,8 +2220,10 @@
                            const float* bias, float* out, int64_t cout, int64_t cout_ld, int64_t B, int64_t D,
                            int64_t H, int64_t W, const float* mask, int64_t mask_ld, const float* residual,
                            int64_t res_ld, float res_scale, int accumulate, int relu_out, unsigned* out_max,
-                           void* out_planes, float* colsum, const void* mask_planes, dlcs_stream_t stream) {
-    DLCS_CHECK_ARG(in && in_max && wthin && B > 0 && (out || out_planes) && !(mask && mask_planes));
+                           void* out_planes, float* colsum, const void* mask_planes, const void* mask_bits,
+                           dlcs_stream_t stream) {
+    DLCS_CHECK_ARG(in && in_max && wthin && B > 0 && (out || out_planes) &&
+                   (mask != nullptr) + (mask_planes != nullptr) + (mask_bits != nullptr) <= 1);
     if (!out) cout_ld = 160;
     auto al16 = [](const void* p) { return ((uintptr_t)p & 15) == 0; };
     const long rows = (long)B * D * H * W;
@@ -2223,10 +2241,11 @@
     v.B = (int)B; v.D = (int)D; v.H = (int)H; v.W = (int)W; v.cin_ld = (int)cin_ld; v.cin_pad = (int)cin;
     v.cout_ld = (int)cout_ld; v.mask_ld = (int)mask_ld; v.res_ld = (int)res_ld; v.accumulate = accumulate;
     v.relu_out = relu_out; v.res_scale = res_scale; v.cout = (int)cout; v.cout_pad = (int)cout; v.omax = out_max;
-    v.mplanes = mask_planes;
+    v.mbits = (const unsigned char*)mask_bits;
     hipStream_t st = (hipStream_t)stream;
-    if (!thin_in && (out_planes || colsum || mask_planes || !out)) return DLCS_ERR_UNSUPPORTED_SIZE;
+    if (!thin_in && (out_planes || colsum || mask_planes || mask_bits || !out)) return DLCS_ERR_UNSUPPORTED_SIZE;
     if (mask_planes && !al16(mask_planes)) return DLCS_ERR_UNSUPPORTED_SIZE;
+    if (mask_planes && !(v.mbits = mask_bits_of_planes(mask_planes, rows, st))) return (int)hipErrorOutOfMemory;
     if (out_planes && (!al16(out_planes) || cout_ld != 160)) return DLCS_ERR_UNSUPPORTED_SIZE;
     const unsigned* opmax = out_planes ? (const unsigned*)((const char*)out_planes + rows * 640) : nullptr;
     const long ntile = (long)B * (D / 4) * ((H / 4 + 1) / 2) * ((W / 4 + 1) / 2);
diff --git a/dl-swin-gan_amd/csrc/conv3d_f16x3.inc b/dl-swin-gan_amd/csrc/conv3d_f16x3.inc
--- a/dl-swin-gan_amd/csrc/conv3d_f16x3.inc
+++ b/dl-swin-gan_amd/csrc/conv3d_f16x3.inc
@@ -45,6 +45,23 @@
     f16* d = xp + r * 320 + (c >> 5) * 64 + (c & 31);
     *reinterpret_cast<f16x4_h3*>(d) = h;
     *reinterpret_cast<f16x4_h3*>(d + 32) = l;
+}
+
+DLCS_DEV unsigned relu_bits4(const f32x4_t& v) {
+    return (v[0] > 0.0f ? 1u : 0u) | (v[1] > 0.0f ? 2u : 0u) | (v[2] > 0.0f ? 4u : 0u) | (v[3] > 0.0f ? 8u : 0u);
+}
+DLCS_DEV unsigned relu_bits8(const f32x4_t& v0, const f32x4_t& v1) { return relu_bits4(v0) | (relu_bits4(v1) << 4); }
+__global__ void __launch_bounds__(256) relu_bits_from_planes_kernel(const f16* xp, long rows, unsigned char* bits) {
+    const long i = (long)blockIdx.x * 256 + threadIdx.x;
+    if (i >= rows * 20) return;
+    const long r = i / 20;
+    const int c = (int)(i % 20) * 8;
+    const f16* q = xp + r * 320 + (c >> 5) * 64 + (c & 31);
+    const u32x4_h3 h = *reinterpret_cast<const u32x4_h3*>(q), l = *reinterpret_cast<const u32x4_h3*>(q + 32);
+    unsigned m = 0;
+#pragma unroll
+    for (int e = 0; e < 8; ++e) m |= ((((h[e >> 1] | l[e >> 1]) >> (16 * (e & 1))) & 0x7fffu) ? 1u : 0u) << e;
+    bits[i] = (unsigned char)m;
 }
 
 DLCS_DEV f32x4_t get_planes4(const f16* xp, long r, int c, float rinv) {
@@ -263,7 +280,8 @@
     float* part; int tail_base;
     f16* oplanes; const unsigned* opmax;
     float* cpart;
-    const void* mplanes;
+    const unsigned char* mbits;
+    unsigned char* obits;
     int stamp;
     int exp;
 };
@@ -276,7 +294,7 @@
 #define H3_STAMP(k) do { } while (0)
 #endif
 
-template <int EPI, int NPASS, bool PREF = true>
+template <int EPI, int NPASS, bool PREF = true, bool OBITS = true>
 DLCS_DEV void conv_epilogue_h3(const ConvF32Args& a, const f32x4_t (&acc)[4][5], float* Es, int pw, int cw0,
                                int lane, int b, int pt, int pyq, int pxq, int nT, int nY, int nX,
                                f16* op, const unsigned* opmax, float* cpart) {
@@ -286,7 +304,8 @@
     static_assert(PC % 8 == 0 && 256 * NCH % 512 == 0 && PC <= 512, "whole 8-channel chunks per thread");
     const float* src = EPI == kEpiRes ? a.res : a.mask;
     const int sld = EPI == kEpiRes ? a.res_ld : a.mask_ld;
-    const f16* mp = EPI == kEpiMask ? reinterpret_cast<const f16*>(a.mplanes) : nullptr;
+    const unsigned char* mb = EPI == kEpiMask ? a.mbits : nullptr;
+    static_assert(PREF || NPASS <= 8, "one word per pass in an item's 8-word slot");
     f32x4_t pre[PREF ? NPASS : 1][PER][2];
     long orows[PER];
     bool oks[PER];
@@ -304,10 +323,10 @@
         for (int k = 0; k < PER; ++k) {
             const int c = threadIdx.x + k * 512;
             const int co = pass * PC + (c % NCH) * 8;
-            if (mp) {
-                const f16* q = mp + orows[k] * 320 + (co >> 5) * 64 + (co & 31);
-                pre[slot][k][0] = *reinterpret_cast<const f32x4_t*>(q);
-                pre[slot][k][1] = *reinterpret_cast<const f32x4_t*>(q + 32);
+            if (mb) {
+                const float w = __uint_as_float((unsigned)mb[orows[k] * 20 + (co >> 3)]);
+                if constexpr (PREF) pre[slot][k][0][0] = w;
+                else pre[0][k][pass >> 2][pass & 3] = w;
             } else {
                 const float* sp = src + orows[k] * sld + co;
                 pre[slot][k][0] = *reinterpret_cast<const f32x4_t*>(sp);
@@ -315,15 +334,16 @@
             }
         }
     };
-    if constexpr (PREF) {
+    if (PREF || mb) {
 #pragma unroll
         for (int pass = 0; pass < NPASS; ++pass) load_pre(pass, pass);
     }
     float vmax = 0.0f;
+    unsigned char* Bs = reinterpret_cast<unsigned char*>(Es + 256 * EL + 512);
 #pragma unroll
     for (int pass = 0; pass < NPASS; ++pass) {
         const int ps_ = PREF ? pass : 0;
-        if constexpr (!PREF) load_pre(pass, 0);
+        if (!PREF && !mb) load_pre(pass, 0);
 #pragma unroll
         for (int j = 0; j < 5; ++j) {
             const int c0 = cw0 + j * 16 - pass * PC;
@@ -356,14 +376,12 @@
                 v0 += *reinterpret_cast<const f32x4_t*>(a.bias + co);
                 v1 += *reinterpret_cast<const f32x4_t*>(a.bias + co + 4);
             }
-            if (EPI == kEpiMask && mp) {
-                const u32x4_h3 hb = __builtin_bit_cast(u32x4_h3, pre[ps_][k][0]);
-                const u32x4_h3 lb = __builtin_bit_cast(u32x4_h3, pre[ps_][k][1]);
-#pragma unroll
-                for (int e = 0; e < 8; ++e) {
-                    const unsigned nz = ((hb[e >> 1] | lb[e >> 1]) >> (16 * (e & 1))) & 0x7fffu;
-                    if (e < 4) v0[e] = nz ? v0[e] : 0.0f;
-                    else v1[e - 4] = nz ? v1[e - 4] : 0.0f;
+            if (EPI == kEpiMask && mb) {
+                const unsigned m = __float_as_uint(PREF ? pre[ps_][k][0][0] : pre[0][k][pass >> 2][pass & 3]);
+#pragma unroll
+                for (int e = 0; e < 4; ++e) {
+                    v0[e] = ((m >> e) & 1u) ? v0[e] : 0.0f;
+                    v1[e] = ((m >> (4 + e)) & 1u) ? v1[e] : 0.0f;
                 }
             } else if (EPI == kEpiMask) {
 #pragma unroll
@@ -385,6 +403,7 @@
                 *reinterpret_cast<f32x4_t*>(o + 4) = v1;
             }
             if (op) put_planes8(op, orows[k], co, v0, v1, ps);
+            if (OBITS && a.obits) Bs[vl * 20 + (co >> 3)] = (unsigned char)relu_bits8(v0, v1);
             if (cpart) {
                 *reinterpret_cast<f32x4_t*>(Es + vl * EL + ch) = v0;
                 *reinterpret_cast<f32x4_t*>(Es + vl * EL + ch + 4) = v1;
@@ -414,6 +433,15 @@
             }
         }
         __syncthreads();
+    }
+    if (OBITS && a.obits && threadIdx.x < 320) {
+        const int p = threadIdx.x / 80, q = threadIdx.x % 80;
+        const int py = pyq + (p >> 1), px = pxq + (p & 1);
+        if (py < nY && px < nX) {
+            const long row0 = ((((long)b * nT + pt) * nY + py) * nX + px) * 64;
+            *reinterpret_cast<u32x4_h3*>(a.obits + row0 * 20 + q * 16) =
+                *reinterpret_cast<const u32x4_h3*>(Bs + p * 1280 + q * 16);
+        }
     }
     if (a.omax) {
         vmax = wave_max(vmax);
@@ -721,7 +749,8 @@
     ConvF32Args ea{};
     ea.bias = a.bias; ea.out = a.out; ea.mask = a.mask; ea.res = a.res;
     ea.cout_ld = a.cout_ld; ea.mask_ld = a.mask_ld; ea.res_ld = a.res_ld; ea.accumulate = a.accumulate;
-    ea.relu_out = a.relu_out; ea.res_scale = a.res_scale; ea.omax = a.omax; ea.mplanes = a.mplanes;
+    ea.relu_out = a.relu_out; ea.res_scale = a.res_scale; ea.omax = a.omax;
+    ea.mbits = a.mbits; ea.obits = a.obits;
     if constexpr (EPI == kEpiRes || EPI == kEpiMask)
         conv_epilogue_h3<EPI, 2>(ea, acc, reinterpret_cast<float*>(smem_h3), pw, nh * 80, lane, b, pt, tyy * 2, txx * 2,
                                  nT, nY, nX, a.oplanes, a.opmax, a.cpart ? a.cpart + (long)vb * 160 : nullptr);
@@ -738,6 +767,9 @@
     const int nblk = a.B * nT * nYt * nXt;
     const long i = (long)blockIdx.x * 256 + threadIdx.x;
     float vmax = 0.0f;
+    unsigned nib = 0;
+    long brow_ = -1;
+    int bc = 0;
     if (i < (long)ntail * 256 * 40) {
         const int t = (int)(i / (256 * 40)), rem = (int)(i % (256 * 40));
         const int vl = rem / 40, c = (rem % 40) * 4;
@@ -760,11 +792,10 @@
                 const f32x4_t m = *reinterpret_cast<const f32x4_t*>(a.mask + orow * a.mask_ld + c);
 #pragma unroll
                 for (int e = 0; e < 4; ++e) v[e] = m[e] > 0.0f ? v[e] : 0.0f;
-            } else if (a.mplanes) {
-                const f16* q = reinterpret_cast<const f16*>(a.mplanes) + orow * 320 + (c >> 5) * 64 + (c & 31);
-                const f16x4_h3 h = *reinterpret_cast<const f16x4_h3*>(q), l = *reinterpret_cast<const f16x4_h3*>(q + 32);
-#pragma unroll
-                for (int e = 0; e < 4; ++e) v[e] = (h[e] != (f16)0.0f || l[e] != (f16)0.0f) ? v[e] : 0.0f;
+            } else if (a.mbits) {
+                const unsigned m = (unsigned)a.mbits[orow * 20 + (c >> 3)] >> (c & 4);
+#pragma unroll
+                for (int e = 0; e < 4; ++e) v[e] = ((m >> e) & 1u) ? v[e] : 0.0f;
             }
             if (a.res) v += a.res_scale * *reinterpret_cast<const f32x4_t*>(a.res + orow * a.res_ld + c);
             if (a.relu_out) {
@@ -777,11 +808,18 @@
                 *reinterpret_cast<f32x4_t*>(o) = v;
             }
             if (a.oplanes) put_planes4(a.oplanes, orow, c, v, f16x3_scale(*a.opmax));
+            nib = relu_bits4(v);
+            brow_ = orow;
+            bc = c;
             vmax = fmaxf(fmaxf(fabsf(v[0]), fabsf(v[1])), fmaxf(fabsf(v[2]), fabsf(v[3])));
         } else {
             v = (f32x4_t)0.0f;
         }
         if (a.cpart) *reinterpret_cast<f32x4_t*>(a.part + ((long)(t * 5) * 256 + vl) * 160 + c) = v;
+    }
+    if (a.obits) {
+        const unsigned hi = __shfl_xor(nib, 1, 64);
+        if (brow_ >= 0 && !(bc & 4)) a.obits[brow_ * 20 + (bc >> 3)] = (unsigned char)(nib | (hi << 4));
     }
     if (a.omax) block_max_to(a.omax, vmax, red);
 }
@@ -813,17 +851,17 @@
         nblk = nmain;
     }
     int epi;
-    if (!v.res && !v.mask && !v.mplanes && !v.accumulate) epi = 0;
-    else if (v.res && !v.mask && !v.mplanes && !v.accumulate) epi = kEpiRes;
-    else if (!v.res && (v.mask || v.mplanes) && !v.accumulate) epi = kEpiMask;
+    const bool masked = v.mask || v.mbits;
+    if (!v.res && !masked && !v.accumulate) epi = 0;
+    else if (v.res && !masked && !v.accumulate) epi = kEpiRes;
+    else if (!v.res && masked && !v.accumulate) epi = kEpiMask;
     else epi = kEpiGeneric;
-    if ((v.oplanes || v.cpart || v.mplanes) && epi != kEpiRes && epi != kEpiMask)
+    if ((v.oplanes || v.cpart || v.mbits || v.obits) && epi != kEpiRes && epi != kEpiMask)
         return DLCS_ERR_UNSUPPORTED_SIZE;
     static const int fold_mode = [] {
         const char* e = dlcs_knob("DLCS_H3_FOLD");
         return !e ? 4 : e[0] == '0' ? 0 : e[0] == 'm' ? 2 : e[0] == 'a' ? 3 : e[0] == 'r' ? 4 : e[0] == 'R' ? 5 : 1;
     }();
-    const bool masked = v.mask || v.mplanes;
     const int pf = fold_mode == 1 || (fold_mode == 2 && masked) ? 1 : (fold_mode == 3 && masked) ? 2
                  : (fold_mode == 5 || (fold_mode == 4 && masked)) ? 3 : 0;
     auto launch = [&](auto F) {
@@ -1120,6 +1158,7 @@
     float* cpart;
     const f16* rp; const f16* rp2;
     const unsigned* rpmax; const unsigned* rp2max;
+    unsigned char* obits;
 };
 constexpr int kG3A = 64 * 64, kG3B = 160 * 64;
 
@@ -1231,6 +1270,10 @@
             *reinterpret_cast<f32x4_t*>(cp) = v;
         }
         if (g.oplanes) put_planes4(g.oplanes, orow * (g.N / 160) + nt, ch, v, ps);
+        if (g.obits) {
+            const unsigned nb = relu_bits4(v), hi = __shfl_xor(nb, 1, 64);
+            if (!(ch & 4)) g.obits[(orow * (g.N / 160) + nt) * 20 + (ch >> 3)] = (unsigned char)(nb | (hi << 4));
+        }
         if (g.cpart) *reinterpret_cast<f32x4_t*>(Es + ml * EL + ch) = v;
         vmax = fmaxf(vmax, fmaxf(fmaxf(fabsf(v[0]), fabsf(v[1])), fmaxf(fabsf(v[2]), fabsf(v[3]))));
     }
diff --git a/dl-swin-gan_amd/csrc/conv3d_f32.inc b/dl-swin-gan_amd/csrc/conv3d_f32.inc
--- a/dl-swin-gan_amd/csrc/conv3d_f32.inc
+++ b/dl-swin-gan_amd/csrc/conv3d_f32.inc
@@ -146,7 +146,8 @@
     float res_scale;
     int cout, cout_pad;
     unsigned* omax;
-    const void* mplanes;
+    const unsigned char* mbits;
+    unsigned char* obits;
 };
 
 template <int EPI, int NPASS = 2>
diff --git a/dl-swin-gan_amd/csrc/conv3d_thin_f16x3.inc b/dl-swin-gan_amd/csrc/conv3d_thin_f16x3.inc
--- a/dl-swin-gan_amd/csrc/conv3d_thin_f16x3.inc
+++ b/dl-swin-gan_amd/csrc/conv3d_thin_f16x3.inc
@@ -227,7 +227,7 @@
 #pragma unroll
                 for (int r = 0; r < 4; ++r) acc[i][j][r] *= ((rsgn >> (4 * (lane >> 4) + r)) & 1) ? -inv : inv;
         if constexpr (EPI == kEpiMask)
-            conv_epilogue_h3<kEpiMask, 5, false>(a, acc, Es, pw, nh * 80, lane, b, pt, tyy * 2, txx * 2, nT, nY, nX, op, opmax,
+            conv_epilogue_h3<kEpiMask, 5, false, false>(a, acc, Es, pw, nh * 80, lane, b, pt, tyy * 2, txx * 2, nT, nY, nX, op, opmax,
                                           cpart ? cpart + (long)tile * 160 : nullptr);
         else
             conv_epilogue_f32<EPI, 5>(a, acc, Es, pw, nh * 80, lane, b, pt, tyy * 2, txx * 2, nT, nY, nX);
@@ -673,10 +673,11 @@
     const dim3 g(256);
     if (thin_in) {
         int epi;
-        if (!v.res && !v.mask && !v.mplanes && !v.accumulate) epi = 0;
-        else if (!v.res && (v.mask || v.mplanes) && !v.accumulate) epi = kEpiMask;
+        const bool masked = v.mask || v.mbits;
+        if (!v.res && !masked && !v.accumulate) epi = 0;
+        else if (!v.res && masked && !v.accumulate) epi = kEpiMask;
         else epi = kEpiGeneric;
-        if ((op || cpart || v.mplanes) && epi != kEpiMask) return DLCS_ERR_UNSUPPORTED_SIZE;
+        if ((op || cpart || v.mbits) && epi != kEpiMask) return DLCS_ERR_UNSUPPORTED_SIZE;
         if (epi == 0)
             hipLaunchKernelGGL(conv3d_thin_in_f16x3_kernel<0>, g, dim3(512), 0, st, v, wimg, xmax, cin, ntiles, op, opmax,
                                cpart);
diff --git a/dl-swin-gan_amd/dl_cs/_lib.py b/dl-swin-gan_amd/dl_cs/_lib.py
--- a/dl-swin-gan_amd/dl_cs/_lib.py
+++ b/dl-swin-gan_amd/dl_cs/_lib.py
@@ -58,11 +58,12 @@
     "dlcs_conv3d_pack_weights": [_INT, _P, _P, _I64, _I64, _I64, _I64, _INT, _P],
     "dlcs_conv3d_unpack_wgrad": [_P, _P, _I64, _I64, _I64, _I64, _INT, _P],
     "dlcs_split2_f16_bytes": [_I64],
+    "dlcs_relu_bits_bytes": [_I64],
     "dlcs_split2_f16": [_P, _I64, _I64, _P, _INT, _P, _P],
     "dlcs_conv3d_pack_weights_f16x3_bytes": [],
     "dlcs_conv3d_pack_weights_f16x3": [_P, _INT, _P, _P],
     "dlcs_gemm_k160_f16x3": [_P, _I64, _P, _I64, _P, _I64, _P, _INT, _F, _P, _I64, _F, _P, _I64, _F, _INT, _P, _P, _P,
-                             _P, _P, _P],
+                             _P, _P, _P, _P],
     "dlcs_planes_bound": [_P, _I64, _P, _P, _F, _P, _P, _F, _P, _I64, _F, _P],
     "dlcs_abs_row_sum_max": [_P, _I64, _I64, _I64, _I64, _I64, _P, _P],
     "dlcs_h3r_pack_bytes": [_I64, _I64],
@@ -75,12 +76,12 @@
     "dlcs_gemm_f32_splitk_det_workspace_bytes": [_I64, _I64],
     "dlcs_conv3d_k3_wgrad_f16x3": [_P, _P, _P, _I64, _I64, _I64, _I64, _P],
     "dlcs_conv3d_k3_f16x3": [_P, _P, _P, _P, _I64, _I64, _I64, _I64, _I64, _P, _I64, _P, _I64, _F, _INT, _INT, _P, _P, _P,
-                             _P, _P],
+                             _P, _P, _P, _P],
     "dlcs_conv3d_thin_pack_f16x3_bytes": [_INT],
     "dlcs_conv3d_thin_pack_f16x3": [_P, _I64, _I64, _I64, _I64, _INT, _P, _P],
     "dlcs_absmax_f32": [_P, _I64, _P, _P],
     "dlcs_conv3d_thin_f16x3": [_P, _I64, _I64, _P, _P, _P, _P, _I64, _I64, _I64, _I64, _I64, _I64, _P, _I64, _P,
-                               _I64, _F, _INT, _INT, _P, _P, _P, _P, _P],
+                               _I64, _F, _INT, _INT, _P, _P, _P, _P, _P, _P],
     "dlcs_conv3d_thin_out_planes_f16x3": [_P, _P, _P, _P, _I64, _I64, _I64, _I64, _I64, _I64, _INT, _INT, _P],
     "dlcs_conv3d_thin_wgrad_planes_f16x3": [_P, _P, _I64, _I64, _P, _INT, _P, _I64, _I64, _I64, _I64, _I64, _I64,
                                             _P],
@@ -123,7 +124,7 @@
 }
 _RESTYPE = {"dlcs_status_string": ctypes.c_char_p, "dlcs_scratch_bytes": _SZ, "dlcs_sense_workspace_bytes": _SZ,
             "dlcs_sense_cg_workspace_bytes": _SZ, "dlcs_sense_rowtab_bytes": _SZ,
-            "dlcs_sense_rows_workspace_bytes": _SZ, "dlcs_split2_f16_bytes": _SZ,
+            "dlcs_sense_rows_workspace_bytes": _SZ, "dlcs_split2_f16_bytes": _SZ, "dlcs_relu_bits_bytes": _SZ,
             "dlcs_conv3d_pack_weights_f16x3_bytes": _SZ, "dlcs_conv3d_thin_pack_f16x3_bytes": _SZ,
             "dlcs_gemm_dw_workspace_bytes": _SZ, "dlcs_layernorm_bwd_workspace_bytes": _SZ,
             "dlcs_gemm_f32_splitk_det_workspace_bytes": _SZ, "dlcs_gemm_nt_x6_workspace_bytes": _SZ,
diff --git a/dl-swin-gan_amd/dl_cs/models/_ops.py b/dl-swin-gan_amd/dl_cs/models/_ops.py
--- a/dl-swin-gan_amd/dl_cs/models/_ops.py
+++ b/dl-swin-gan_amd/dl_cs/models/_ops.py
@@ -368,6 +368,10 @@
     return out
 
 
+def bits_alloc(rows, device):
+    return empty((int(_lib.lib().dlcs_relu_bits_bytes(rows)),), torch.uint8, device)
+
+
 def planes_max(planes, rows):
     return ctypes.c_void_p(planes.data_ptr() + rows * 640)
 
@@ -379,24 +383,26 @@
 
 
 def conv3d_f16x3(planes, packed, grid, bias=None, out=None, mask=None, res=None, res_scale=1.0, accumulate=0,
-                 relu_out=0, out_max=None, out_planes=None, colsum=None, planes_only=False, mask_planes=None):
+                 relu_out=0, out_max=None, out_planes=None, colsum=None, planes_only=False, mask_planes=None,
+                 out_bits=None, mask_bits=None):
     B, D, H, W = grid
     rows = B * D * H * W
     if out is None and not planes_only:
         out = empty((rows, 160), torch.float32, planes.device)
     call("dlcs_conv3d_k3_f16x3", p(planes), p(packed), p(bias), p(out), out.shape[-1] if out is not None else 160,
          B, D, H, W, p(mask), mask.shape[-1] if mask is not None else 0, p(res), res.shape[-1] if res is not None else 0,
-         float(res_scale), int(accumulate), int(relu_out), out_max, p(out_planes), p(colsum), p(mask_planes), S())
+         float(res_scale), int(accumulate), int(relu_out), out_max, p(out_planes), p(colsum), p(mask_planes),
+         p(out_bits), p(mask_bits), S())
     return out
 
 
 def gemm_k160_f16x3(a_planes, M, b_planes, N, C, bias=None, act=0, alpha=1.0, res=None, res_scale=1.0,
                     res2=None, res2_scale=1.0, accumulate=0, out_max=None, out_planes=None, colsum=None,
-                    res_planes=None, res2_planes=None):
+                    res_planes=None, res2_planes=None, out_bits=None):
     call("dlcs_gemm_k160_f16x3", p(a_planes), M, p(b_planes), N, p(C), C.shape[-1] if C is not None else N,
          p(bias), int(act), float(alpha), p(res), res.shape[-1] if res is not None else 0, float(res_scale),
          p(res2), res2.shape[-1] if res2 is not None else 0, float(res2_scale), int(accumulate), out_max,
-         p(out_planes), p(colsum), p(res_planes), p(res2_planes), S())
+         p(out_planes), p(colsum), p(res_planes), p(res2_planes), p(out_bits), S())
     return C
 
 
@@ -453,7 +459,7 @@
 
 def conv3d_thin_f16x3(x, cin, x_max, wthin, cout, out_ld, grid, bias=None, out=None, mask=None, res=None,
                       res_scale=1.0, accumulate=0, relu_out=0, out_max=None, out_planes=None, colsum=None,
-                      planes_only=False, mask_planes=None):
+                      planes_only=False, mask_planes=None, mask_bits=None):
     B, D, H, W = grid
     rows = B * D * H * W
     if out is None and not planes_only:
@@ -461,7 +467,8 @@
     call("dlcs_conv3d_thin_f16x3", p(x), cin, x.shape[-1], _word(x_max), p(wthin), p(bias), p(out), cout,
          out.shape[-1] if out is not None else 160, B, D, H, W, p(mask), mask.shape[-1] if mask is not None else 0,
          p(res), res.shape[-1] if res is not None else 0, float(res_scale), int(accumulate), int(relu_out),
-         _word(out_max) if out_max is not None else None, p(out_planes), p(colsum), p(mask_planes), S())
+         _word(out_max) if out_max is not None else None, p(out_planes), p(colsum), p(mask_planes),
+         p(mask_bits), S())
     return out
 
 
diff --git a/dl-swin-gan_amd/dl_cs/models/engine.py b/dl-swin-gan_amd/dl_cs/models/engine.py
--- a/dl-swin-gan_amd/dl_cs/models/engine.py
+++ b/dl-swin-gan_amd/dl_cs/models/engine.py
@@ -356,7 +356,7 @@
     geos = [SwinGeometry(B, nT, nY, nX, window, i % 2 == 1, dev) for i in range(depth)]
     nst = len(W.stages)
     stages = []
-    inp, pout = s, None
+    inp, pout, bout, bh = s, None, None, None
     inp_max = word(0) if W.split else None
     fwd_po = (W.split and not K160_F32 and W.thin_h3 and THIN_PLANES and CAPTURE is None and
               DGRAD_CAPTURE is None and FWD_PLANES_ONLY)
@@ -365,7 +365,7 @@
         tok_t, bsaved = _stage_swin_forward(W, st, inp, geos, ntok, heads,
                                             drop_scales[k] if drop_scales is not None else None)
         a = None if fwd_po else K.empty((rows, C), dtype, dev)
-        ss = dict(inp=inp, tok_t=tok_t, bsaved=bsaved, a=a)
+        ss = dict(inp=inp, tok_t=tok_t, bsaved=bsaved, a=a, bits=K.bits_alloc(rows, dev) if fwd_po else None)
         tb = P[st.pre + "swin_tail.bias"]
         if W.split:
             pa = K.planes_alloc(rows, dev)
@@ -378,13 +378,14 @@
                 tp = K.split2(tok_t)
                 K.planes_bound(pa, rows, m0=K.planes_max(tp, ntok), n0=st.unemb_norm, vec=st.unemb_bias)
                 K.gemm_k160_f16x3(tp, ntok, st.unemb_h3, 64 * C, a.view(ntok, 64 * C) if a is not None else None,
-                                  bias=st.unemb_bias, act=3, out_max=amax, out_planes=pa)
+                                  bias=st.unemb_bias, act=3, out_max=amax, out_planes=pa, out_bits=ss["bits"])
             ss["planes"] = pa
             if last:
                 pb = K.planes_alloc(rows, dev)
+                bout = K.bits_alloc(rows, dev) if fwd_po else None
                 K.planes_bound(pb, rows, m0=amax, n0=st.tail_norm, m1=inp_max, vec=tb)
                 out = _timed("conv_fwd", flops, K.conv3d_f16x3, ss["planes"], st.tail, grid, bias=tb, res=inp,
-                             relu_out=1, out_max=omax, out_planes=pb, planes_only=fwd_po)
+                             relu_out=1, out_max=omax, out_planes=pb, planes_only=fwd_po, out_bits=bout)
                 pout = pb
             else:
                 out = _timed("conv_fwd", flops, K.conv3d_f16x3, ss["planes"], st.tail, grid, bias=tb, res=inp,
@@ -403,8 +404,9 @@
         if W.thin_h3 and THIN_PLANES:
             ph = K.planes_alloc(rows, dev)
             K.planes_bound(ph, rows, m0=inp_max, n0=W.dfe_norm, m1=word(0), c1=2.0, vec=P["dfe_tail.bias"])
+            bh = K.bits_alloc(rows, dev) if fwd_po else None
         h = _timed("conv_fwd", flops, K.conv3d_f16x3, pout, W.dfe, grid, bias=P["dfe_tail.bias"], res=s,
-                   res_scale=2.0, relu_out=1, out_max=K.p(hmax), out_planes=ph, planes_only=fwd_po)
+                   res_scale=2.0, relu_out=1, out_max=K.p(hmax), out_planes=ph, planes_only=fwd_po, out_bits=bh)
         if ph is not None:
             o = K.conv3d_thin_out_planes(ph, W.fin_h3, cin, PAD_CIN, grid, bias=P["final_layer.layers.2.conv.bias"])
         elif W.thin_h3:
@@ -419,7 +421,7 @@
         o = K.conv3d(h, C, W.fin, cin, PAD_CIN, grid, bias=P["final_layer.layers.2.conv.bias"],
                      out_dtype=torch.float32)
     out = K.swin_post(o, (B, E, T, Y, X), pad)
-    saved = dict(u=u, s=s, b=b, pout=pout, h=h, ph=ph, stages=stages, geos=geos, shape=(B, E, T, Y, X), grid=grid,
+    saved = dict(u=u, s=s, b=b, pout=pout, bout=bout, h=h, ph=ph, bh=bh, stages=stages, geos=geos, shape=(B, E, T, Y, X), grid=grid,
                  pad=pad, heads=heads, cin=cin, C=C, ntok=ntok, umax=umax, hmax=hmax)
     if CAPTURE is not None:
         CAPTURE.append(dict(relu_inputs=[ss["a"] for ss in stages] + [b, h], grid=grid, C=C))
@@ -458,7 +460,7 @@
                 ghm = K.zeros((1,), torch.int32, dev)
                 K.planes_bound(pg, rows, m0=gomax, n0=_conv_norm(P["final_layer.layers.2.conv.weight"], C, dgrad=True))
                 K.conv3d_thin_f16x3(go, cin, gomax, K.thin_pack_f16x3(wf, C, cin, 0), C, C, grid, mask=sv["h"],
-                                    mask_planes=sv["ph"] if sv["h"] is None else None, out_max=K.p(ghm),
+                                    mask_bits=sv["bh"], out_max=K.p(ghm),
                                     out_planes=pg, planes_only=True, colsum=grads["dfe_tail.bias"])
                 g_h = None
             else:
@@ -486,7 +488,7 @@
             gom = K.zeros((1,), torch.int32, dev)
             K.planes_bound(pg, rows, m0=ghmax, n0=_conv_norm(P["dfe_tail.weight"], C, dgrad=True))
             _timed("conv_dgrad", flops, K.conv3d_f16x3, gp, K.conv_pack_f16x3(P["dfe_tail.weight"], 1), grid,
-                   mask=sv["b"], mask_planes=sv["pout"] if sv["b"] is None else None, out_max=K.p(gom),
+                   mask=sv["b"], mask_bits=sv["bout"], out_max=K.p(gom),
                    out_planes=pg, planes_only=True,
                    colsum=grads[W.stages[-1].pre + "swin_tail.bias"])
             g_out = None
@@ -518,7 +520,7 @@
                 gp = K.split2(g_out, out=pg, have_max=True, colsum=grads[pre + "swin_tail.bias"])
                 gomax = gp[rows * 640:rows * 640 + 4].view(torch.int32).clone()
             g_a = _timed("conv_dgrad", flops, K.conv3d_f16x3, gp, K.conv_pack_f16x3(P[pre + "swin_tail.weight"], 1),
-                         grid, mask=ss["a"], mask_planes=ss["planes"] if ss["a"] is None else None)
+                         grid, mask=ss["a"], mask_bits=ss["bits"])
             split_wgrad(ss["planes"], gp, pre + "swin_tail.weight")
             del gp
             if DGRAD_CAPTURE is not None:
diff --git a/include/dlcs.h b/include/dlcs.h
--- a/include/dlcs.h
+++ b/include/dlcs.h
@@ -141,6 +141,7 @@
 #endif
 
 size_t dlcs_split2_f16_bytes(int64_t rows);
+size_t dlcs_relu_bits_bytes(int64_t rows);
 int dlcs_split2_f16(const float* x, int64_t rows, int64_t ld, void* planes, int have_max, float* colsum,
                     dlcs_stream_t stream);
 size_t dlcs_conv3d_pack_weights_f16x3_bytes(void);
@@ -149,12 +150,12 @@
                          int64_t B, int64_t D, int64_t H, int64_t W, const float* mask, int64_t mask_ld,
                          const float* residual, int64_t res_ld, float res_scale, int accumulate, int relu_out,
                          unsigned* out_max, void* out_planes, float* colsum, const void* mask_planes,
-                         dlcs_stream_t stream);
+                         void* out_bits, const void* mask_bits, dlcs_stream_t stream);
 int dlcs_gemm_k160_f16x3(const void* aplanes, int64_t M, const void* bplanes, int64_t N, float* C, int64_t ldc,
                          const float* bias, int act, float alpha, const float* residual, int64_t ldr, float res_scale,
                          const float* residual2, int64_t ldr2, float res2_scale, int accumulate, unsigned* out_max,
                          void* out_planes, float* colsum, const void* res_planes, const void* res2_planes,
-                         dlcs_stream_t stream);
+                         void* out_bits, dlcs_stream_t stream);
 int dlcs_planes_bound(void* planes, int64_t rows, const unsigned* m0, const unsigned* n0, float c0,
                       const unsigned* m1, const unsigned* n1, float c1, const float* vec, int64_t nvec, float cvec,
                       dlcs_stream_t stream);
@@ -196,7 +197,8 @@
                            const float* bias, float* out, int64_t cout, int64_t cout_ld, int64_t B, int64_t D,
                            int64_t H, int64_t W, const float* mask, int64_t mask_ld, const float* residual,
                            int64_t res_ld, float res_scale, int accumulate, int relu_out, unsigned* out_max,
-                           void* out_planes, float* colsum, const void* mask_planes, dlcs_stream_t stream);
+                           void* out_planes, float* colsum, const void* mask_planes, const void* mask_bits,
+                           dlcs_stream_t stream);
 int dlcs_conv3d_thin_wgrad_f16x3(const float* in, int64_t cin, int64_t cin_ld, const unsigned* in_max,
                                  const float* g, int64_t cout, int64_t g_ld, const unsigned* g_max, float* dw_packed,
                                  int64_t cout_pad, int64_t cin_pad, float* colsum, int64_t B, int64_t D, int64_t H,
```
